# amirkdv/biseqt

Measured on AMD Instinct MI355X. Metric: GCUPS (DP cell updates/s) banded local align, higher is better.
Workload: dtype i16

## Files before the change

biseqt_amd/batch.py:

```python
import ctypes as C

import numpy as np

from . import _pwlib as W
from .sequence import Sequence

RESULT_DTYPE = np.dtype([('score', '<f8'), ('opt_i', '<i4'), ('opt_j', '<i4'),
                         ('origin_idx', '<i4'), ('mutant_idx', '<i4'),
                         ('tx_len', '<i4'), ('status', '<i4')])
assert RESULT_DTYPE.itemsize == 32
SUMMARY_DTYPE = np.dtype([(f, '<i4') for f in ('n_match', 'n_subst', 'n_ins', 'n_del', 'n_gaps', 'first_match', 'last_match',
                                               'head_origin', 'head_mutant', 'tail_origin', 'tail_mutant', 'flags')])
assert SUMMARY_DTYPE.itemsize == 48
CIGAR_EXTENDED, CIGAR_CLASSIC = W.PW_CIGAR_EXTENDED, W.PW_CIGAR_CLASSIC
CIGAR_OPS = 'MIDNSHP=X'
_CIGAR_FORMS = {'extended': CIGAR_EXTENDED, 'classic': CIGAR_CLASSIC}
SITE_DTYPE = np.dtype([('depth', '<u4'), ('call', 'u1'), ('ref', 'u1'), ('flags', '<u2')])
assert SITE_DTYPE.itemsize == 8
POLISH_STATS_DTYPE = np.dtype([(f, '<u4') for f in ('kept', 'substituted', 'deleted', 'inserted')])
assert POLISH_STATS_DTYPE.itemsize == 16
_SIDES = {'origin': W.PW_SIDE_ORIGIN, 'mutant': W.PW_SIDE_MUTANT, 'both': W.PW_SIDE_BOTH}
_CIGAR_LETTERS = ({'M': '=', 'S': 'X', 'I': 'I', 'D': 'D'}, {'M': 'M', 'S': 'M', 'I': 'I', 'D': 'D'})


# ... 604 lines not shown
        if sides not in _SIDES:
            raise ValueError("sides is 'origin', 'mutant' or 'both', not %r" % (sides,))

        def per_pair(a, dtype, what):
            if a is None:
                return None
            a = np.ascontiguousarray(a, dtype).reshape(-1)
            if len(a) != self.n:
                raise ValueError('%s has %d entries for %d pairs' % (what, len(a), self.n))
            return a
        c, mc = per_pair(col0, np.int64, 'col0'), per_pair(mutant_col0, np.int64, 'mutant_col0')
        rv = per_pair(None if reverse is None else np.asarray(reverse) != 0, np.uint8, 'reverse')
        comp = None
        if rv is not None and rv.any():
            if sides == 'origin':
                raise ValueError("reverse applies to the mutant side: sides is 'mutant' or 'both'")
            if complement is None:
                raise ValueError('reversed pairs need a complement table')
            comp = np.ascontiguousarray(complement, np.uint8).reshape(-1)
        if not isinstance(pileup, Pileup) or not pileup.handle:
            raise ValueError('pileup must be an open Pileup')
        if sides == 'origin' and mc is None and rv is None and complement is None and not pileup.ins_slots:
            self._ck(self.lib.pw_batch_pileup_add(self.handle, pileup.handle, None if c is None else c.ctypes.data, int(arena_first), stream),
                     'pw_batch_pileup_add')
            return

        def ptr(a):
            return None if a is None else a.ctypes.data
        self._ck(self.lib.pw_batch_pileup_add_sides(self.handle, pileup.handle, _SIDES[sides], ptr(c), ptr(mc), ptr(rv), ptr(comp),
                                                    0 if comp is None else len(comp), int(arena_first), stream),
                 'pw_batch_pileup_add_sides')

    def scores_plane(self, k):
        X, Y = self.lens[k]
        dmin, dmax, _ = self.band(k)
        nd, pitch = dmax - dmin + 1, min(X, Y) + 1
        out = np.zeros(nd * pitch, np.float64)
        self._ck(self.lib.pw_batch_scores(self.handle, k, out.ctypes.data_as(C.POINTER(C.c_double)), out.size),
                 'pw_batch_scores')
        return out.reshape(nd, pitch)

    def masks(self, k):
        out = np.zeros(max(int(self.lib.pw_batch_pair_cells(self.handle, k)), 1), np.uint8)
        self._ck(self.lib.pw_batch_masks(self.handle, k, out.ctypes.data_as(C.POINTER(C.c_uint8)), out.size),
                 'pw_batch_masks')
        return out

    def results_device(self):
        return DeviceBuffer(self.lib.pw_batch_results_device(self.handle), 32 * self.n, self)

    def transcripts_device(self):
        return DeviceBuffer(self.lib.pw_batch_transcripts_device(self.handle),
                            self.lib.pw_batch_transcripts_bytes(self.handle), self)

    def fill_ms(self):
        return float(self.lib.pw_batch_fill_ms(self.handle))

    def trace_ms(self):
        return float(self.lib.pw_batch_trace_ms(self.handle))


def align_batch(pairs, **kw):
    with BatchAligner(pairs, **kw) as b:
        res = b.run()
        return res, b.transcripts(res)


def summary_dict(rec):
    return {f: int(rec[f]) for f in SUMMARY_DTYPE.names}


def summarize_transcripts(transcripts, device=0):
    if isinstance(transcripts, tuple) and len(transcripts) == 2 and isinstance(transcripts[0], np.ndarray):
        buf = np.ascontiguousarray(transcripts[0], np.uint8)
        off = np.ascontiguousarray(transcripts[1], np.uint64)
        assert off.ndim == 1 and off.size >= 1 and int(off[-1]) <= buf.size
    else:
        raw = [(t or '').encode('ascii') for t in transcripts]
        off = np.zeros(len(raw) + 1, np.uint64)
        if raw:
            off[1:] = np.cumsum([len(r) for r in raw])
        buf = np.frombuffer(b''.join(raw), np.uint8)
    n = off.size - 1
    out = np.zeros(max(n, 1), SUMMARY_DTYPE)
    if W.load().pw_tx_summarize_packed(device, buf.ctypes.data if buf.size else None, off.ctypes.data, n, out.ctypes.data) != 0:
        raise RuntimeError('pw_tx_summarize_packed failed: ' + W.last_error())
    return out[:n]


def _packed_transcripts(transcripts):
    if isinstance(transcripts, tuple) and len(transcripts) == 2 and isinstance(transcripts[0], np.ndarray):
        buf = np.ascontiguousarray(transcripts[0], np.uint8)
        off = np.ascontiguousarray(transcripts[1], np.uint64)
        assert off.ndim == 1 and off.size >= 1 and int(off[-1]) <= buf.size
        return buf, off
    raw = [(t or '').encode('ascii') for t in transcripts]
    off = np.zeros(len(raw) + 1, np.uint64)
    if raw:
        off[1:] = np.cumsum([len(r) for r in raw])
    return np.frombuffer(b''.join(raw), np.uint8), off


def cigars_of_transcripts(transcripts, form='extended', device=0):
    f = _cigar_form(form)
    buf, off = _packed_transcripts(transcripts)
    n = off.size - 1
    lib = W.load()
    roff = np.zeros(n + 1, np.uint64)
    ops = buf.ctypes.data if buf.size else None
    runs = np.zeros(max(int(off[-1]) - int(off[0]), 1), np.uint32)
    if lib.pw_tx_cigar_packed(device, ops, off.ctypes.data, n, f, runs.ctypes.data, runs.size, roff.ctypes.data) != 0:
        raise RuntimeError('pw_tx_cigar_packed failed: ' + W.last_error())
    return runs[:int(roff[-1])].copy(), roff


def cigar_strings(runs, offsets):
    runs, offsets = np.asarray(runs, np.uint32), np.asarray(offsets, np.int64)
    lens, ops = (runs >> 4).tolist(), (runs & 15).tolist()
    return [''.join('%d%s' % (lens[r], CIGAR_OPS[ops[r]]) for r in range(int(offsets[k]), int(offsets[k + 1])))
            for k in range(len(offsets) - 1)]


def cigar_of_transcript(tx, form='extended'):
    letters = _CIGAR_LETTERS[_cigar_form(form)]
    out, cur, n = [], None, 0
    for op in tx or '':
        if op not in letters:
            raise ValueError('transcript op %r is none of M, S, I, D' % (op,))
        if letters[op] == cur:
            n += 1
            continue
        if cur is not None:
            out.append('%d%s' % (n, cur))
        cur, n = letters[op], 1
    if cur is not None:
        out.append('%d%s' % (n, cur))
    return ''.join(out)


def transcript_of_cigar(s):
    import re
    if not re.fullmatch(r'(?:[0-9]+[A-Za-z=])*', s):
        raise ValueError('not a CIGAR string: %r' % (s,))
    back = {'=': 'M', 'X': 'S', 'I': 'I', 'D': 'D'}
    out = []
    for n, op in re.findall(r'([0-9]+)([A-Za-z=])', s):
        if op not in back:
            raise ValueError('CIGAR op %r has no transcript letter (only the extended form =, X, I, D has)' % (op,))
        out.append(back[op] * int(n))
    return ''.join(out)


def plan_only(shapes, alnmode=W.STD_MODE, alntype=W.GLOBAL, alphabet_len=4, subst_scores=None, match_score=1, mismatch_score=0,
              go_score=0, ge_score=0, flags=0, ramp_free=False, stamp_group=False):
    lib = W.load()
    L = alphabet_len
    if subst_scores is None:
        subst_scores = [[match_score if i == j else mismatch_score for i in range(L)] for j in range(L)]
    S = np.ascontiguousarray(np.asarray(subst_scores, dtype=np.float64).reshape(L, L))
    sc = W.pw_scoring(alnmode, alntype, L, S.ctypes.data_as(C.POINTER(C.c_double)), float(go_score), float(ge_score))
    pairs = (W.pw_pair * max(len(shapes), 1))()
    off = 0
    for k, sh in enumerate(shapes):
        X, Y = int(sh[0]), int(sh[1])
        dmin, dmax = (int(sh[2]), int(sh[3])) if len(sh) > 2 else (0, 0)
        oo = off
        off += (X + 15) // 16 * 16 + 16
        mo = off
        off += (Y + 15) // 16 * 16 + 16
        pairs[k] = W.pw_pair(oo, mo, X, Y, dmin, dmax)
    name = C.create_string_buffer(128)
    info = (C.c_int32 * 8)()
    if lib.pw_plan_only(C.byref(sc), len(shapes), pairs, max(off, 16), flags, name, 128, info) != 0:
        raise RuntimeError('pw_plan_only failed: ' + W.last_error())
    out = dict(kernel=name.value.decode(), score_dtype='f64' if info[0] else 'i32', scale_shift=info[1], one_wavefront=info[2],
                workgroup=info[3], tiled=info[4], strips=info[5], packed_rule=info[6], matrix=bool(info[7] & 1))
    if ramp_free:
        out['ramp_free'] = bool(info[7] & 2)
    if stamp_group:
        out['stamp_group'] = 4 if info[7] & 4 else 1
    return out
```

biseqt_amd/csrc/build.py:

```python
import concurrent.futures
import os
import shutil
import subprocess
import sys

HERE = os.path.dirname(os.path.abspath(__file__))
ROOT = os.path.dirname(os.path.dirname(HERE))
OUT_DIR = os.path.join(os.path.dirname(HERE), 'pwlib')
OBJ_DIR = os.path.join(HERE, os.environ.get('PW_OBJ_DIR', '_build'))
SO = os.path.join(OUT_DIR, os.environ.get('PW_SO_NAME', 'pwlib.so'))
HIPCC = os.environ.get('HIPCC', '/opt/rocm/bin/hipcc')
ARCH = 'gfx950'
COMMON = ['--offload-arch=' + ARCH, '-O3', '-std=c++17', '-fPIC', '-ffp-contract=off', '-Wall',
          '-Wno-unused-function'] + os.environ.get('PW_EXTRA_CXXFLAGS', '').split()
BKS = (2, 4, 8, 16, 32)
PACKED_BKS = (4, 8, 12, 16, 20, 24, 28, 32)
PACKED_RULES = (0, 1, 2, 3, 4, 5)
PACKED_MAT_RULES = (0, 1, 2, 3)
FILL16_WAVES = {
    (8, 0, 0): (5, 0), (8, 3, 0): (5, 0),
    (16, 0, 0): (3, 0), (16, 3, 0): (3, 0),
    (8, 0, 1): (3, 0), (8, 3, 1): (3, 0),
}
for _e in filter(None, os.environ.get('PW_FILL16_WAVES_OVERRIDE', '').split(';')):
    _k, _v = _e.split('=')
    FILL16_WAVES[tuple(int(x) for x in _k.split(','))] = tuple(int(x) for x in _v.split(','))
FILL16_UNR = {}
for _e in filter(None, os.environ.get('PW_FILL16_UNR_OVERRIDE', '').split(';')):
    _k, _v = _e.split('=')
    FILL16_UNR[tuple(int(x) for x in _k.split(','))] = int(_v)
TYPES = (('i32', 'int32_t'), ('f64', 'double'))
F64_FLAGS = {'f64': ['-fno-honor-nans'] + os.environ.get('PW_F64_EXTRA_CXXFLAGS', '').split()}
FILL_EXTRA = {('f64', 8): ['-mllvm', '-amdgpu-sched-strategy=max-ilp']}
HASHED_OBJECTS = ('pw_fill16_bk8_r3_mat.o', 'pw_fill16g_bk8_r3_mat.o', 'pw_fill16_bk8_r3.o', 'pw_fill16_bk8_r0.o', 'pw_fill_i32_bk8.o', 'pw_fill_f64_bk8.o', 'pw_strip.o')
HEADERS = ['pw_types.h', 'pw_wave.h', 'pw_strip.h', 'pw_plan.h', 'pw_model.h', 'pw_launch.h', 'pw_device.h', 'pw_hip_host.h']


def _jobs():
    jobs = []
    for tn, t in TYPES:
        for bk in BKS:
            obj = os.path.join(OBJ_DIR, 'pw_fill_%s_bk%d.o' % (tn, bk))
            cmd = [HIPCC] + COMMON + F64_FLAGS.get(tn, []) + FILL_EXTRA.get((tn, bk), []) + ['-DPW_T=' + t, '-DPW_TNAME=' + tn, '-DPW_BK=%d' % bk, '-c',
                                      os.path.join(HERE, 'pw_fill_tu.hip'), '-o', obj]
            jobs.append((obj, cmd, [os.path.join(HERE, 'pw_fill_tu.hip')]))
    for tn, t in TYPES:
        obj = os.path.join(OBJ_DIR, 'pw_fill_mw_%s.o' % tn)
        cmd = [HIPCC] + COMMON + F64_FLAGS.get(tn, []) + ['-DPW_T=' + t, '-DPW_TNAME=' + tn, '-c', os.path.join(HERE, 'pw_fill_mw_tu.hip'), '-o', obj]
        jobs.append((obj, cmd, [os.path.join(HERE, 'pw_fill_mw_tu.hip')]))
    for tn, t in TYPES:
        obj = os.path.join(OBJ_DIR, 'pw_fill_tile_%s.o' % tn)
        cmd = [HIPCC] + COMMON + F64_FLAGS.get(tn, []) + ['-DPW_T=' + t, '-DPW_TNAME=' + tn, '-c', os.path.join(HERE, 'pw_fill_tile_tu.hip'), '-o', obj]
        jobs.append((obj, cmd, [os.path.join(HERE, 'pw_fill_tile_tu.hip')]))
    for bk, rule, mat in [(bk, r, 0) for r in PACKED_RULES for bk in PACKED_BKS] + [(bk, r, 1) for r in PACKED_MAT_RULES for bk in PACKED_BKS]:
        obj = os.path.join(OBJ_DIR, 'pw_fill16_bk%d_r%d%s.o' % (bk, rule, '_mat' if mat else ''))
        occ, occ_seg = FILL16_WAVES.get((bk, rule, mat), (0, 0)) if os.environ.get('PW_FILL16_OCCUPANCY', '1') != '0' else (0, 0)
        cmd = [HIPCC] + COMMON + ['-mllvm', '-amdgpu-sched-strategy=max-ilp', '-DPW_BK=%d' % bk, '-DPW_RULE=%d' % rule, '-DPW_MAT=%d' % mat,
                                  '-DPW_FILL16_WAVES=%d' % occ, '-DPW_FILL16_WAVES_SEG=%d' % occ_seg] + \
              (['-DPW_FILL16_UNR=%d' % FILL16_UNR[(bk, rule, mat)]] if (bk, rule, mat) in FILL16_UNR else []) + ['-c',
               os.path.join(HERE, 'pw_fill16_tu.hip'), '-o', obj]
        jobs.append((obj, cmd, [os.path.join(HERE, 'pw_fill16_tu.hip')]))
    obj = os.path.join(OBJ_DIR, 'pw_fill16g_bk8_r3_mat.o')
    occ, occ_seg = FILL16_WAVES.get((8, 3, 1), (0, 0)) if os.environ.get('PW_FILL16_OCCUPANCY', '1') != '0' else (0, 0)
    jobs.append((obj, [HIPCC] + COMMON + ['-mllvm', '-amdgpu-sched-strategy=max-ilp', '-DPW_FILL16_WAVES=%d' % occ,
                                          '-DPW_FILL16_WAVES_SEG=%d' % occ_seg, '-c', os.path.join(HERE, 'pw_fill16g_tu.hip'), '-o', obj],
                 [os.path.join(HERE, 'pw_fill16g_tu.hip')]))
    obj = os.path.join(OBJ_DIR, 'pw_trace.o')
    jobs.append((obj, [HIPCC] + COMMON + ['-c', os.path.join(HERE, 'pw_trace.hip'), '-o', obj],
                 [os.path.join(HERE, 'pw_trace.hip')]))
    obj = os.path.join(OBJ_DIR, 'pw_txsum.o')
    jobs.append((obj, [HIPCC] + COMMON + ['-c', os.path.join(HERE, 'pw_txsum.hip'), '-o', obj],
                 [os.path.join(HERE, 'pw_txsum.hip'), os.path.join(ROOT, 'include', 'pw_txsum.h'), os.path.join(ROOT, 'include', 'pw_batch.h')]))
    obj = os.path.join(OBJ_DIR, 'pw_cigar.o')
    jobs.append((obj, [HIPCC] + COMMON + ['-c', os.path.join(HERE, 'pw_cigar.hip'), '-o', obj],
                 [os.path.join(HERE, 'pw_cigar.hip'), os.path.join(ROOT, 'include', 'pw_cigar.h'), os.path.join(ROOT, 'include', 'pw_batch.h')]))
    obj = os.path.join(OBJ_DIR, 'pw_pileup.o')
    jobs.append((obj, [HIPCC] + COMMON + ['-c', os.path.join(HERE, 'pw_pileup.hip'), '-o', obj],
                 [os.path.join(HERE, 'pw_pileup.hip'), os.path.join(ROOT, 'include', 'pw_pileup.h'), os.path.join(ROOT, 'include', 'pw_batch.h')]))
    obj = os.path.join(OBJ_DIR, 'pw_polish.o')
    jobs.append((obj, [HIPCC] + COMMON + ['-Wno-unused-parameter', '-c', os.path.join(HERE, 'pw_polish.hip'), '-o', obj],
                 [os.path.join(HERE, 'pw_polish.hip'), os.path.join(ROOT, 'include', 'pw_polish.h'), os.path.join(ROOT, 'include', 'pw_pileup.h'),
                  os.path.join(ROOT, 'include', 'pw_batch.h')]))
    obj = os.path.join(OBJ_DIR, 'pw_graph.o')
    jobs.append((obj, [HIPCC] + COMMON + ['-Wno-unused-parameter', '-c', os.path.join(HERE, 'pw_graph.hip'), '-o', obj],
                 [os.path.join(HERE, 'pw_graph.hip'), os.path.join(HERE, 'pw_graph_launch.h'), os.path.join(ROOT, 'include', 'pw_graph.h'),
                  os.path.join(ROOT, 'include', 'pw_txsum.h'), os.path.join(ROOT, 'include', 'pw_batch.h')]))
    obj = os.path.join(OBJ_DIR, 'pw_consensus.o')
    jobs.append((obj, [HIPCC] + COMMON + ['-Wno-unused-parameter', '-c', os.path.join(HERE, 'pw_consensus.hip'), '-o', obj],
                 [os.path.join(HERE, 'pw_consensus.hip'), os.path.join(HERE, 'pw_consensus_launch.h'), os.path.join(HERE, 'pw_graph_launch.h'),
                  os.path.join(ROOT, 'include', 'pw_consensus.h'), os.path.join(ROOT, 'include', 'pw_graph.h'),
                  os.path.join(ROOT, 'include', 'pw_batch.h')]))
    obj = os.path.join(OBJ_DIR, 'pw_strip.o')
    jobs.append((obj, [HIPCC] + COMMON + os.environ.get('PW_STRIP_CXXFLAGS', '').split() + ['-c', os.path.join(HERE, 'pw_strip.hip'), '-o', obj],
                 [os.path.join(HERE, 'pw_strip.hip')]))
    obj = os.path.join(OBJ_DIR, 'pw_seeds.o')
    jobs.append((obj, [HIPCC] + COMMON + ['-Wno-unused-parameter', '-c', os.path.join(HERE, 'pw_seeds.hip'), '-o', obj],
                 [os.path.join(HERE, 'pw_seeds.hip'), os.path.join(HERE, 'pw_seed_kernels.h'), os.path.join(HERE, 'pw_seed_host.h'), os.path.join(ROOT, 'include', 'pw_seeds.h')]))
    obj = os.path.join(OBJ_DIR, 'pw_mseeds.o')
    jobs.append((obj, [HIPCC] + COMMON + ['-Wno-unused-parameter', '-c', os.path.join(HERE, 'pw_mseeds.hip'), '-o', obj],
                 [os.path.join(HERE, 'pw_mseeds.hip'), os.path.join(HERE, 'pw_seed_kernels.h'), os.path.join(HERE, 'pw_seed_host.h'), os.path.join(ROOT, 'include', 'pw_mseeds.h')]))
    obj = os.path.join(OBJ_DIR, 'pw_qseeds.o')
    jobs.append((obj, [HIPCC] + COMMON + ['-Wno-unused-parameter', '-c', os.path.join(HERE, 'pw_qseeds.hip'), '-o', obj],
                 [os.path.join(HERE, 'pw_qseeds.hip'), os.path.join(HERE, 'pw_seed_kernels.h'), os.path.join(HERE, 'pw_seed_host.h'), os.path.join(HERE, 'pw_complement.h'),
                  os.path.join(ROOT, 'include', 'pw_qseeds.h')]))
    obj = os.path.join(OBJ_DIR, 'pw_overlap.o')
    jobs.append((obj, [HIPCC] + COMMON + ['-Wno-unused-parameter', '-c', os.path.join(HERE, 'pw_overlap.hip'), '-o', obj],
                 [os.path.join(HERE, 'pw_overlap.hip'), os.path.join(HERE, 'pw_complement.h'), os.path.join(HERE, 'pw_kmer_encode.h'), os.path.join(HERE, 'pw_minimizer.h'),
                  os.path.join(ROOT, 'include', 'pw_overlap.h')]))
    obj = os.path.join(OBJ_DIR, 'pw_kmers.o')
    jobs.append((obj, [HIPCC] + COMMON + ['-Wno-unused-parameter', '-c', os.path.join(HERE, 'pw_kmers.hip'), '-o', obj],
                 [os.path.join(HERE, 'pw_kmers.hip'), os.path.join(HERE, 'pw_complement.h'), os.path.join(HERE, 'pw_kmer_encode.h'), os.path.join(HERE, 'pw_minimizer.h'),
                  os.path.join(ROOT, 'include', 'pw_kmers.h'), os.path.join(ROOT, 'include', 'pw_overlap.h')]))
    obj = os.path.join(OBJ_DIR, 'pwlib_api.o')
    jobs.append((obj, [HIPCC] + COMMON + ['-x', 'hip', '-c', os.path.join(HERE, 'pwlib_api.cpp'), '-o', obj],
                 [os.path.join(HERE, 'pwlib_api.cpp'), os.path.join(HERE, 'pw_model.h'), os.path.join(ROOT, 'include', 'pwlib.h'),
                  os.path.join(ROOT, 'include', 'pw_batch.h'), os.path.join(ROOT, 'include', 'pw_txsum.h'),
                  os.path.join(ROOT, 'include', 'pw_cigar.h'), os.path.join(ROOT, 'include', 'pw_pileup.h'),
                  os.path.join(ROOT, 'include', 'pw_polish.h'), os.path.join(ROOT, 'include', 'pw_graph.h'),
                  os.path.join(HERE, 'pw_graph_launch.h'), os.path.join(HERE, 'pw_complement.h'),
                  os.path.join(ROOT, 'include', 'pw_consensus.h'), os.path.join(HERE, 'pw_consensus_launch.h')]))
    return jobs


def _cmd_text(cmd):
    return ' '.join(cmd) + '\n'


def _stale(target, deps, cmd=None):
    if not os.path.exists(target):
        return True
    t = os.path.getmtime(target)
    if any(os.path.getmtime(d) > t for d in deps):
        return True
    if cmd is not None:
        try:
            with open(target + '.cmd') as f:
                return f.read() != _cmd_text(cmd)
        except OSError:
            return True
    return False


def build(force=False, verbose=True):
    os.makedirs(OBJ_DIR, exist_ok=True)
    os.makedirs(OUT_DIR, exist_ok=True)
    hdrs = [os.path.join(HERE, h) for h in HEADERS]
    jobs = _jobs()
    todo = [(o, c) for (o, c, deps) in jobs if force or _stale(o, deps + hdrs, c)]

    def run(job):
        obj, cmd = job
        if os.path.exists(obj + '.cmd'):
            os.remove(obj + '.cmd')
        r = subprocess.run(cmd, stdout=subprocess.PIPE, stderr=subprocess.STDOUT, universal_newlines=True)
        if r.returncode == 0:
            with open(obj + '.cmd', 'w') as f:
                f.write(_cmd_text(cmd))
        return obj, r.returncode, r.stdout

    workers = max(1, min(len(todo), (os.cpu_count() or 4)))
    if todo:
        if verbose:
            print('[build] compiling %d objects for %s with %d workers' % (len(todo), ARCH, workers))
        with concurrent.futures.ThreadPoolExecutor(workers) as ex:
            for obj, rc, out in ex.map(run, todo):
                if rc != 0:
                    raise RuntimeError('hipcc failed for %s:\n%s' % (obj, out))
                if verbose and out.strip():
                    print(out)
    objs = [o for (o, _, _) in jobs]
    strip_obj = os.path.join(OBJ_DIR, 'pw_strip.o')
    if force or any(o == strip_obj for o, _ in todo) or not os.path.exists(SO):
        from . import codeobj
        bad = codeobj.strip_kernel_violations(strip_obj)
        if bad:
            os.remove(strip_obj)
            raise RuntimeError('pw_strip.o breaks the invariants its inline asm relies on:\n  ' + '\n  '.join(bad))
    if force or todo or _stale(SO, objs):
        cmd = [HIPCC, '--offload-arch=' + ARCH, '-shared', '-fPIC'] + objs + ['-o', SO]
        r = subprocess.run(cmd, stdout=subprocess.PIPE, stderr=subprocess.STDOUT, universal_newlines=True)
        if r.returncode != 0:
            raise RuntimeError('link failed:\n' + r.stdout)
        if verbose:
            print('[build] linked', SO)
    shutil.copyfile(os.path.join(ROOT, 'include', 'pwlib.h'), os.path.join(OUT_DIR, 'pwlib.h'))
    hashes = os.path.join(OUT_DIR, 'kernel_hashes.json' if os.path.basename(SO) == 'pwlib.so' else os.path.basename(SO) + '.hashes.json')
    if force or todo or not os.path.exists(hashes):
        from . import codeobj
        import json
        fp = {}
        for obj in HASHED_OBJECTS:
            fp.update(codeobj.kernel_fingerprints(os.path.join(OBJ_DIR, obj)))
        with open(hashes, 'w') as f:
            json.dump(fp, f, indent=1, sort_keys=True)
    return SO


if __name__ == '__main__':
    build(force='--force' in sys.argv)
```

biseqt_amd/csrc/pw_device.h:

```cpp
#ifndef PW_DEVICE_H
#define PW_DEVICE_H

#include <hip/hip_runtime.h>
#include <stdint.h>

#define PW_FN __device__ __forceinline__
#include "pw_wave.h"
#include "pw_launch.h"

namespace pw {

PW_FN uint32_t dev_shl1_in(uint32_t m, bool flag) {
  const uint64_t mask = __builtin_amdgcn_ballot_w64(flag);
  uint32_t r;
  uint64_t cout;
  asm("v_addc_co_u32 %0, %1, %2, %2, %3" : "=v"(r), "=s"(cout) : "v"(m), "s"(mask));
  return r;
}

template <typename T, bool ALWAYS_LDS> PW_FN T dev_tab_read(const T* tab, uint32_t handle, uint32_t off, bool in_lds) {
  typedef __attribute__((address_space(3))) const T lds_T;
  if (ALWAYS_LDS || in_lds) return *(lds_T*)(uintptr_t)(handle + off);
  return *(const T*)((const char*)tab + off);
}
PW_FN uint32_t dev_lds_handle(const void* p) {
  return (uint32_t)(uintptr_t)(__attribute__((address_space(3))) const char*)p;
}

PW_FN uint32_t dev_const_dword(const uint8_t* base, int idx) {
  typedef const __attribute__((address_space(4))) uint32_t c_u32;
  return ((c_u32*)base)[idx];
}

typedef uint64_t FeedDwords __attribute__((aligned(4)));
PW_FN uint64_t dev_const_dword2(const uint8_t* base, uint32_t byte_off) {
  typedef const __attribute__((address_space(4))) uint8_t c_u8;
  typedef const __attribute__((address_space(4))) FeedDwords c_fd;
  return *(c_fd*)((c_u8*)base + byte_off + 4u);
}

struct DevFeed {
  PW_FN static uint64_t const_dword2(const uint8_t* base, uint32_t byte_off) { return dev_const_dword2(base, byte_off); }
};

struct DevP : DevFeed {
  PW_FN static uint32_t const_dword(const uint8_t* base, int idx) { return dev_const_dword(base, idx); }
  template <typename T, bool A> PW_FN static T tab_read(const T* tab, uint32_t h, uint32_t off, bool in_lds) { return dev_tab_read<T, A>(tab, h, off, in_lds); }
  PW_FN static uint32_t shl1_in(uint32_t m, bool flag) { return dev_shl1_in(m, flag); }
  PW_FN static int lane() { return (int)(threadIdx.x & 63u); }
  PW_FN static int32_t shr1(int32_t v, int32_t old) {
    return __builtin_amdgcn_update_dpp(old, v, 0x138 , 0xf, 0xf, false);
  }
  PW_FN static int32_t shl1(int32_t v, int32_t old) {
    return __builtin_amdgcn_update_dpp(old, v, 0x130 , 0xf, 0xf, false);
  }
  PW_FN static int32_t shr1z(int32_t v) { return __builtin_amdgcn_update_dpp(0, v, 0x138 , 0xf, 0xf, true); }
  PW_FN static int32_t shl1z(int32_t v) { return __builtin_amdgcn_update_dpp(0, v, 0x130 , 0xf, 0xf, true); }
  PW_FN static int32_t shfl_xor(int32_t v, int m) { return __shfl_xor(v, m, 64); }
  PW_FN static int32_t uniform(int32_t v) { return __builtin_amdgcn_readfirstlane(v); }
  PW_FN static int nlanes() { return 64; }
  PW_FN static int nwaves() { return 1; }
  PW_FN static int32_t wave_bcast(int32_t v, int) { return v; }
  PW_FN static int lane0() { return 0; }
  PW_FN static bool central() { return true; }
  static constexpr bool kVirtualLanes = false;
  static constexpr bool kBatchedShifts = false;
};

template <int N, int MAXW> PW_FN void wg_shift_right(int32_t* v, const int32_t* old, int phase) {
  __shared__ int32_t edge[2][MAXW][N];
  const int w = (int)(threadIdx.x >> 6), l = (int)(threadIdx.x & 63u);
  int32_t r[N];
#pragma unroll
  for (int i = 0; i < N; i++) r[i] = __builtin_amdgcn_update_dpp(old[i], v[i], 0x138 , 0xf, 0xf, false);
  if (l == 63) {
#pragma unroll
    for (int i = 0; i < N; i++) edge[phase][w][i] = v[i];
  }
  asm volatile("s_waitcnt lgkmcnt(0)\n\ts_barrier" ::: "memory");
  if (l == 0 && w > 0) {
#pragma unroll
    for (int i = 0; i < N; i++) r[i] = edge[phase][w - 1][i];
  }
#pragma unroll
  for (int i = 0; i < N; i++) v[i] = r[i];
}
template <int N, int MAXW> PW_FN void wg_shift_left(int32_t* v, const int32_t* old, int phase) {
  __shared__ int32_t edge[2][MAXW][N];
  const int w = (int)(threadIdx.x >> 6), l = (int)(threadIdx.x & 63u), nw = (int)(blockDim.x >> 6);
  int32_t r[N];
#pragma unroll
  for (int i = 0; i < N; i++) r[i] = __builtin_amdgcn_update_dpp(old[i], v[i], 0x130 , 0xf, 0xf, false);
  if (l == 0) {
#pragma unroll
    for (int i = 0; i < N; i++) edge[phase][w][i] = v[i];
  }
  asm volatile("s_waitcnt lgkmcnt(0)\n\ts_barrier" ::: "memory");
  if (l == 63 && w + 1 < nw) {
#pragma unroll
    for (int i = 0; i < N; i++) r[i] = edge[phase][w + 1][i];
  }
#pragma unroll
  for (int i = 0; i < N; i++) v[i] = r[i];
}

struct DevPM : DevFeed {
  PW_FN static uint32_t const_dword(const uint8_t* base, int idx) { return dev_const_dword(base, idx); }
  template <typename T, bool A> PW_FN static T tab_read(const T* tab, uint32_t h, uint32_t off, bool in_lds) { return dev_tab_read<T, A>(tab, h, off, in_lds); }
  PW_FN static uint32_t shl1_in(uint32_t m, bool flag) { return dev_shl1_in(m, flag); }
  PW_FN static int lane() { return (int)threadIdx.x; }
  PW_FN static int lane0() { return 0; }
  PW_FN static bool central() { return true; }
  static constexpr bool kVirtualLanes = false;
  static constexpr bool kBatchedShifts = true;
  template <int N> PW_FN static void shrv(int32_t* v, const int32_t* old, int phase) { wg_shift_right<N, 16>(v, old, phase); }
  template <int N> PW_FN static void shlv(int32_t* v, const int32_t* old, int phase) { wg_shift_left<N, 16>(v, old, phase); }
  PW_FN static int nlanes() { return (int)blockDim.x; }
  PW_FN static int nwaves() { return (int)(blockDim.x >> 6); }
  PW_FN static int32_t shr1(int32_t v, int32_t old) {
    __shared__ int32_t edge[16];
    const int w = (int)(threadIdx.x >> 6), l = (int)(threadIdx.x & 63u);
    int32_t r = __builtin_amdgcn_update_dpp(old, v, 0x138 , 0xf, 0xf, false);
    if (l == 63) edge[w] = v;
    __syncthreads();
    if (l == 0 && w > 0) r = edge[w - 1];
    __syncthreads();
    return r;
  }
  PW_FN static int32_t shl1(int32_t v, int32_t old) {
    __shared__ int32_t edge[16];
    const int w = (int)(threadIdx.x >> 6), l = (int)(threadIdx.x & 63u);
    int32_t r = __builtin_amdgcn_update_dpp(old, v, 0x130 , 0xf, 0xf, false);
    if (l == 0) edge[w] = v;
    __syncthreads();
    if (l == 63 && w + 1 < (int)(blockDim.x >> 6)) r = edge[w + 1];
    __syncthreads();
    return r;
  }
  PW_FN static int32_t shfl_xor(int32_t v, int m) { return __shfl_xor(v, m, 64); }
  PW_FN static int32_t uniform(int32_t v) { return __builtin_amdgcn_readfirstlane(v); }
  PW_FN static int32_t wave_bcast(int32_t v, int w) {
    __shared__ int32_t slot[16];
    if ((threadIdx.x & 63u) == 0) slot[threadIdx.x >> 6] = v;
    __syncthreads();
    const int32_t r = slot[w];
    __syncthreads();
    return r;
  }
};

constexpr int kMaxLdsL = 32;

#ifndef PW_FILL_ATTR
#define PW_FILL_ATTR
#endif
template <typename T, int BK, bool BANY, bool TRACK, bool GENERIC>
__global__ __launch_bounds__(64) PW_FILL_ATTR void k_fill(const FillParams<T> a) {
  constexpr bool TAB = true;
  __shared__ T sub_lds[TAB ? kMaxLdsL * kMaxLdsL : 1];
  const T* tab = a.subst;
  if (TAB) {
    if (a.L <= kMaxLdsL) {
      for (int i = (int)threadIdx.x; i < a.L * a.L; i += 64) sub_lds[i] = a.subst[i];
      __syncthreads();
      tab = sub_lds;
    }
  }
  const int slot = (int)blockIdx.x;
  const int pair = a.order ? a.order[slot] : slot;
  const PairDesc pd = a.pairs[pair];
  WaveFill<DevP, T, BK, BANY, TRACK, GENERIC> w(a, pd, tab);
  w.tab_handle = dev_lds_handle(sub_lds); w.tab_in_lds = tab == sub_lds;
  w.pair_slot = pair;
  w.run();
}

#ifndef PW_FILL16_WAVES
#define PW_FILL16_WAVES 0
#endif
#ifndef PW_FILL16_WAVES_SEG
#define PW_FILL16_WAVES_SEG 0
#endif
template <int BK, bool SEG, int RULE> struct Fill16Occupancy {
  static constexpr unsigned w = SEG ? PW_FILL16_WAVES_SEG : PW_FILL16_WAVES;
  static constexpr unsigned lo = w ? w : 1, hi = w ? w : 8;
};
template <int BK, bool SEG, int RULE, bool MAT = false>
__global__ __launch_bounds__(64) PW_FILL_ATTR
__attribute__((amdgpu_waves_per_eu(Fill16Occupancy<BK, SEG, RULE>::lo, Fill16Occupancy<BK, SEG, RULE>::hi)))
void k_fill16(const FillParams<int32_t> a) {
  const WaveDesc wd = a.waves[blockIdx.x];
  WaveFill16<DevP, BK, SEG, RULE, MAT> w(a, wd);
  w.run();
}

template <int BK, bool SEG, int RULE, bool MAT = false>
__global__ __launch_bounds__(64) PW_FILL_ATTR
__attribute__((amdgpu_waves_per_eu(Fill16Occupancy<BK, SEG, RULE>::lo, Fill16Occupancy<BK, SEG, RULE>::hi)))
void k_fill16g(const FillParams<int32_t> a) {
  const WaveDesc wd = a.waves[blockIdx.x];
  WaveFill16<DevP, BK, SEG, RULE, MAT, 4> w(a, wd);
  w.run();
}

template <int BK, int RULE, bool MAT = false>
__global__ __launch_bounds__(512) void k_fill16_mw(const FillParams<int32_t> a) {
  const WaveDesc wd = a.waves[blockIdx.x];
  WaveFill16<DevPM, BK, false, RULE, MAT> w(a, wd);
  w.run();
}

constexpr int kTileLanes = PW_TILE_LANES, kTileGhost = PW_TILE_GHOST, kTileCentral = kTileLanes - 2 * kTileGhost;
struct DevPT : DevFeed {
  PW_FN static uint32_t const_dword(const uint8_t* base, int idx) { return dev_const_dword(base, idx); }
  template <typename T, bool A> PW_FN static T tab_read(const T* tab, uint32_t h, uint32_t off, bool in_lds) { return dev_tab_read<T, A>(tab, h, off, in_lds); }
  PW_FN static uint32_t shl1_in(uint32_t m, bool flag) { return dev_shl1_in(m, flag); }
  PW_FN static int tile() {
#ifdef PW_TILE_NO_XCD_REMAP
    return (int)blockIdx.x;
#else
    return (int)(blockIdx.x & 7u) * (int)(gridDim.x >> 3) + (int)(blockIdx.x >> 3);
#endif
  }
  PW_FN static int lane0() { return tile() * kTileCentral - kTileGhost; }
  PW_FN static int lane() { return lane0() + (int)threadIdx.x; }
  PW_FN static int nlanes() { return lane0() + kTileLanes; }
  PW_FN static int nwaves() { return kTileLanes / 64; }
  PW_FN static bool central() { return (int)threadIdx.x >= kTileGhost && (int)threadIdx.x < kTileLanes - kTileGhost; }
  static constexpr bool kVirtualLanes = true;
  static constexpr bool kBatchedShifts = true;
  template <int N> PW_FN static void shrv(int32_t* v, const int32_t* old, int phase) { wg_shift_right<N, kTileLanes / 64>(v, old, phase); }
  template <int N> PW_FN static void shlv(int32_t* v, const int32_t* old, int phase) { wg_shift_left<N, kTileLanes / 64>(v, old, phase); }
  PW_FN static void wg_max4(int (&v)[4]) {
    __shared__ int red[4];
    if (threadIdx.x < 4) red[threadIdx.x] = -0x7fffffff;
    __syncthreads();
#pragma unroll
    for (int i = 0; i < 4; i++) atomicMax(&red[i], v[i]);
    __syncthreads();
#pragma unroll
    for (int i = 0; i < 4; i++) v[i] = red[i];
  }
  PW_FN static int32_t shr1(int32_t v, int32_t old) {
    __shared__ int32_t edge[kTileLanes / 64];
    const int w = (int)(threadIdx.x >> 6), l = (int)(threadIdx.x & 63u);
    int32_t r = __builtin_amdgcn_update_dpp(old, v, 0x138 , 0xf, 0xf, false);
    if (l == 63) edge[w] = v;
    __syncthreads();
    if (l == 0 && w > 0) r = edge[w - 1];
    __syncthreads();
    return r;
  }
  PW_FN static int32_t shl1(int32_t v, int32_t old) {
    __shared__ int32_t edge[kTileLanes / 64];
    const int w = (int)(threadIdx.x >> 6), l = (int)(threadIdx.x & 63u);
    int32_t r = __builtin_amdgcn_update_dpp(old, v, 0x130 , 0xf, 0xf, false);
    if (l == 0) edge[w] = v;
    __syncthreads();
    if (l == 63 && w + 1 < kTileLanes / 64) r = edge[w + 1];
    __syncthreads();
    return r;
  }
  PW_FN static int32_t shfl_xor(int32_t v, int m) { return __shfl_xor(v, m, 64); }
  PW_FN static int32_t uniform(int32_t v) { return __builtin_amdgcn_readfirstlane(v); }
  PW_FN static int32_t wave_bcast(int32_t v, int) { return v; }
};

constexpr int kTileBK = PW_TILE_BK;
static_assert(kTileBK == kTileBKHost && kTileCentral == kTileCentralLanes && kTileBlocks * 16 <= kTileGhost * kTileBK,
              "tile geometry: host and device must agree, and a time block must fit the ghost zone");

template <typename T, bool BANY, bool TRACK, bool GENERIC>
__global__ __launch_bounds__(kTileLanes) void k_fill_tile(const FillParams<T> a, const int pair) {
  constexpr bool TAB = true;
  __shared__ T sub_lds[TAB ? kMaxLdsL * kMaxLdsL : 1];
  const T* tab = a.subst;
  if (TAB) {
    if (a.L <= kMaxLdsL) {
      for (int i = (int)threadIdx.x; i < a.L * a.L; i += (int)blockDim.x) sub_lds[i] = a.subst[i];
      __syncthreads();
      tab = sub_lds;
    }
  }
  const PairDesc pd = a.pairs[pair];
  WaveFill<DevPT, T, kTileBK, BANY, TRACK, GENERIC> w(a, pd, tab);
  w.tab_handle = dev_lds_handle(sub_lds); w.tab_in_lds = tab == sub_lds;
  w.pair_slot = pair;
  w.run_tile();
}

template <typename T>
__global__ __launch_bounds__(256) void k_tile_finish(const FillParams<T> a, const int pair) {
  using Tr = ScoreTraits<T>;
  __shared__ T s_s[256]; __shared__ unsigned long long s_k[256]; __shared__ int s_x[256], s_y[256], s_h[256];
  const PairDesc pd = a.pairs[pair];
  const int X = pd.X, Y = pd.Y, endrule = a.endrule, pitch = a.st_pitch;
  T cs = Tr::neg(); unsigned long long ck = ~0ull; int cx = -1, cy = -1, have = 0;
  for (int dd = (int)threadIdx.x; dd < pd.ndiag; dd += 256) {
    const int d = pd.dmin + dd;
    const bool ends_right = d < X - Y;
    const int lx = ends_right ? d + Y : X, ly = ends_right ? Y : X - d;
    T s; unsigned long long k; int x, y; bool ok = true;
    if (endrule == END_CORNER) { ok = d == X - Y; s = a.st_in[dd]; k = 0; x = X; y = Y; }
    else if (endrule == END_STD_OVERLAP) { s = a.st_in[dd]; x = lx; y = ly; k = ends_right ? (unsigned)lx : (unsigned)(X + ly); }
    else if (endrule == END_BANDED_OVERLAP) { s = a.st_in[dd]; x = lx; y = ly; k = (unsigned)dd; }
    else {
      const int tfirst = (d < 0 ? -d : d) - pd.s0;
      const int aa = ((int)a.st_in[4 * pitch + dd] - tfirst) >> 1;
      s = a.st_in[3 * pitch + dd]; x = aa + (d > 0 ? d : 0); y = aa - (d < 0 ? d : 0);
      if (endrule == END_STD_LOCAL) k = (unsigned long long)(unsigned)x * (unsigned long long)(unsigned)(Y + 1) + (unsigned)y;
      else k = ((unsigned long long)(unsigned)dd << 32) | (unsigned)aa;
    }
    if (ok && (!have || s > cs || (s == cs && k < ck))) { cs = s; ck = k; cx = x; cy = y; have = 1; }
  }
  s_s[threadIdx.x] = cs; s_k[threadIdx.x] = ck; s_x[threadIdx.x] = cx; s_y[threadIdx.x] = cy; s_h[threadIdx.x] = have;
  __syncthreads();
  for (int off = 128; off >= 1; off >>= 1) {
    if ((int)threadIdx.x < off) {
      const int o = (int)threadIdx.x + off;
      if (s_h[o] && (!s_h[threadIdx.x] || s_s[o] > s_s[threadIdx.x] || (s_s[o] == s_s[threadIdx.x] && s_k[o] < s_k[threadIdx.x]))) {
        s_s[threadIdx.x] = s_s[o]; s_k[threadIdx.x] = s_k[o]; s_x[threadIdx.x] = s_x[o]; s_y[threadIdx.x] = s_y[o]; s_h[threadIdx.x] = 1;
      }
    }
    __syncthreads();
  }
  if (threadIdx.x == 0) {
    Result r;
    r.score = (double)s_s[0] * a.score_mul;
    r.opt_i = a.banded ? s_x[0] - s_y[0] - pd.dmin : s_x[0];
    r.opt_j = a.banded ? (s_x[0] < s_y[0] ? s_x[0] : s_y[0]) : s_y[0];
    r.origin_idx = 0; r.mutant_idx = 0; r.tx_len = 0; r.status = 0;
    if (!s_h[0] || (endrule == END_STD_LOCAL && !(s_s[0] > T(0)))) { r.opt_i = -1; r.opt_j = -1; r.score = 0.0; }
    a.results[pair] = r;
  }
}

template <typename T>
hipError_t launch_tile_T(const FillParams<T>& a, int variant, int pair, int ntiles, hipStream_t st) {
  const dim3 grid((unsigned)((ntiles + 7) / 8 * 8)), block(kTileLanes);
  switch (variant) {
    case VAR_FAST_ANY_TRACK: hipLaunchKernelGGL((k_fill_tile<T, true, true, false>), grid, block, 0, st, a, pair); break;
    case VAR_FAST_TRACK: hipLaunchKernelGGL((k_fill_tile<T, false, true, false>), grid, block, 0, st, a, pair); break;
    case VAR_FAST: hipLaunchKernelGGL((k_fill_tile<T, false, false, false>), grid, block, 0, st, a, pair); break;
    case VAR_GENERIC: hipLaunchKernelGGL((k_fill_tile<T, false, true, true>), grid, block, 0, st, a, pair); break;
    default: return hipErrorInvalidValue;
  }
  return hipGetLastError();
}
template <typename T>
hipError_t launch_tile_finish_T(const FillParams<T>& a, int pair, hipStream_t st) {
  hipLaunchKernelGGL((k_tile_finish<T>), dim3(1), dim3(256), 0, st, a, pair);
  return hipGetLastError();
}

// ... 50 lines not shown
```

biseqt_amd/csrc/pw_launch.h:

```cpp
#ifndef PW_LAUNCH_H
#define PW_LAUNCH_H

#include <hip/hip_runtime_api.h>

#include "pw_plan.h"
#include "pw_types.h"

namespace pw {

hipError_t launch_fill(const FillParams<int32_t>& a, int variant, int bk, int nblocks, hipStream_t st);
hipError_t launch_fill(const FillParams<double>& a, int variant, int bk, int nblocks, hipStream_t st);
hipError_t launch_fill16(const FillParams<int32_t>& a, int bk, int seg, int rule, int mat, int nwaves, hipStream_t st);
hipError_t launch_fill16_mw(const FillParams<int32_t>& a, int bk, int rule, int mat, int nw, int npairs, hipStream_t st);
hipError_t launch_fill16g(const FillParams<int32_t>& a, int nwaves, hipStream_t st);
hipError_t launch_fill_mw(const FillParams<int32_t>& a, int variant, int bk, int nw, int nblocks, hipStream_t st);
hipError_t launch_fill_mw(const FillParams<double>& a, int variant, int bk, int nw, int nblocks, hipStream_t st);
hipError_t launch_tile(const FillParams<int32_t>& a, int variant, int pair, int ntiles, hipStream_t st);
hipError_t launch_tile(const FillParams<double>& a, int variant, int pair, int ntiles, hipStream_t st);
hipError_t launch_tile_finish(const FillParams<int32_t>& a, int pair, hipStream_t st);
hipError_t launch_tile_finish(const FillParams<double>& a, int pair, hipStream_t st);
hipError_t launch_trace(const TraceParams& p, hipStream_t st);
hipError_t launch_tx_pack(const PairDesc* pairs, const Result* results, const uint8_t* slots, int n, uint64_t* offsets,
                          uint8_t* packed, hipStream_t st);
hipError_t launch_tx_summary(const PairDesc* pairs, const Result* results, const uint8_t* slots, int n, void* out, hipStream_t st);
hipError_t launch_tx_summary_packed(const uint8_t* ops, const uint64_t* offsets, int n, void* out, hipStream_t st);
hipError_t launch_cigar_count(const PairDesc* pairs, const Result* results, const uint8_t* slots, int n, int form, uint64_t* offsets,
                              hipStream_t st);
hipError_t launch_cigar_write(const PairDesc* pairs, const Result* results, const uint8_t* slots, int n, int form, const uint64_t* offsets,
                              uint32_t* runs, hipStream_t st);
hipError_t launch_cigar_count_packed(const uint8_t* ops, const uint64_t* offsets, int n, int form, uint64_t* run_offsets, hipStream_t st);
hipError_t launch_cigar_write_packed(const uint8_t* ops, const uint64_t* offsets, int n, int form, const uint64_t* run_offsets, uint32_t* runs,
                                     hipStream_t st);
hipError_t launch_pileup_add(const PairDesc* pairs, const Result* results, const uint8_t* slots, const uint8_t* arena, int n,
                             const int64_t* col0, int64_t arena_first, uint32_t* counts, int64_t n_cols, int L, hipStream_t st);
hipError_t launch_pileup_call(const uint32_t* counts, const uint8_t* ref, int64_t n_cols, int L, uint32_t min_depth, void* sites,
                              hipStream_t st);
struct PolishComplement { uint32_t w[8]; };
}
struct DeviceBuffer;
namespace pw {
hipError_t launch_polish_add(const PairDesc* pairs, const Result* results, const uint8_t* slots, const uint8_t* arena, int n, int sides,
                             const int64_t* ocol0, const int64_t* mcol0, const uint8_t* reversed, const PolishComplement& comp,
                             int64_t arena_first, uint32_t* counts, uint32_t* ins, int64_t n_cols, int L, int J, hipStream_t st);
hipError_t launch_polish_letters(uint32_t* counts, const uint8_t* letters, int64_t lo, int64_t hi, int L, uint32_t weight, hipStream_t st);
hipError_t launch_polish_count(const uint32_t* counts, const uint32_t* ins, const uint8_t* letters, const int64_t* roff, const int32_t* rlen,
                               int64_t n, int L, int J, uint32_t min_depth, uint64_t* lens, uint64_t* offsets, void* stats, DeviceBuffer& tmp,
                               hipStream_t st);
hipError_t launch_polish_write(const uint32_t* counts, const uint32_t* ins, const uint8_t* letters, const int64_t* roff, const int32_t* rlen,
                               int64_t n, int L, int J, uint32_t min_depth, const uint64_t* offsets, uint8_t* out, hipStream_t st);
struct StripParams;
struct StripTraceParams;
hipError_t launch_strip_fill(const StripParams& a, bool track, bool byte_rows, const uint32_t* ctl_init, int nworkers, int lds_bytes,
                             hipStream_t st);
hipError_t launch_strip_trace(const StripTraceParams& p, hipStream_t st);
hipError_t launch_xcc_census(uint32_t* d_seen8, hipStream_t st);
hipError_t launch_table_rowmajor(const void* plane, bool f64, int X, int Y, int pitch, double mul, double* out, hipStream_t st);

}
#endif
```

biseqt_amd/csrc/pw_plan.h:

```cpp
#ifndef PW_PLAN_H
#define PW_PLAN_H

#include <math.h>
#include <stdint.h>
#include <stdlib.h>

#include <algorithm>

#include "pw_model.h"
#include "pw_types.h"

namespace pw {

struct Plan {
  int rc;
  int clamped;
  int dmin, dmax;
  int num_rows;
  int64_t cells;
  int ndiag;
  int s0, nblocks, steady_b0, steady_b1;
  int brule, endrule;
};

// ... 18 lines not shown
  if (mode == STD_MODE) {
    *brule = (type == LOCAL || type == END_ANCHORED) ? BRULE_ANY
             : (type == OVERLAP || type == END_ANCHORED_OVERLAP) ? BRULE_EDGE : BRULE_ORIGIN;
    *endrule = (type == GLOBAL || type == END_ANCHORED || type == END_ANCHORED_OVERLAP) ? END_CORNER
               : (type == OVERLAP || type == START_ANCHORED_OVERLAP) ? END_STD_OVERLAP : END_STD_LOCAL;
  } else {
    *brule = type == B_LOCAL ? BRULE_ANY : type == B_OVERLAP ? BRULE_EDGE : BRULE_ORIGIN;
    *endrule = type == B_GLOBAL ? END_CORNER : type == B_OVERLAP ? END_BANDED_OVERLAP : END_BANDED_LOCAL;
  }
}

static inline Plan plan_problem(int mode, int type, int X, int Y, int dmin_in, int dmax_in) {
  Plan p;
  p.rc = 0; p.clamped = 0; p.cells = 0; p.ndiag = 0;
  p.s0 = 0; p.nblocks = 0; p.steady_b0 = 0; p.steady_b1 = 0;
  plan_rules(mode, type, &p.brule, &p.endrule);
  if (mode == STD_MODE) {
    p.dmin = -Y; p.dmax = X; p.num_rows = X + 1;
    p.cells = (int64_t)(X + 1) * (int64_t)(Y + 1);
  } else {
    int dmin = dmin_in, dmax = dmax_in;
    if (dmax > X || dmin < -Y) {
      dmax = dmax > X ? X : dmax;
      dmin = dmin < -Y ? -Y : dmin;
      p.clamped = 1;
    }
    p.dmin = dmin; p.dmax = dmax;
    const int dend = X - Y;
    if (type == B_GLOBAL && (dend > dmax || dend < dmin || (int64_t)dmax * dmin > 0)) { p.rc = -1; return p; }
    p.num_rows = 1 + dmax - dmin;
    if (p.num_rows < 0) { p.rc = -1; return p; }
    if (p.num_rows == 0) { p.ndiag = 0; return p; }
    p.cells = plan_band_cells(X, Y, dmin, dmax);
  }
  p.ndiag = 1 + p.dmax - p.dmin;
  const int amin = p.dmin > 0 ? p.dmin : (p.dmax < 0 ? -p.dmax : 0);
  int s_last = 0, tf_max = 0, tl_min = 0x7fffffff;
  p.s0 = amin - (((amin - p.dmin) % 2 + 2) % 2);
  const int cand[4] = {p.dmin, p.dmax, 0, X - Y};
  for (int k = 0; k < 4; k++) {
    const int d = cand[k];
    if (d < p.dmin || d > p.dmax) continue;
    const int ad = d < 0 ? -d : d;
    const int tl = ad + 2 * (plan_len(X, Y, d) - 1);
    if (tl > s_last) s_last = tl;
    if (ad - p.s0 > tf_max) tf_max = ad - p.s0;
    if (tl - p.s0 < tl_min) tl_min = tl - p.s0;
  }
  const int nsteps = s_last - p.s0 + 1;
  p.nblocks = (nsteps + 15) / 16;
  p.steady_b0 = tf_max / 16 + 1;
  p.steady_b1 = (tl_min + 1) / 16;
  if (p.steady_b1 > p.nblocks) p.steady_b1 = p.nblocks;
  if (p.steady_b1 < p.steady_b0) p.steady_b1 = p.steady_b0;
  return p;
}


enum { VAR_FAST_ANY_TRACK = 0,
       VAR_FAST_TRACK = 1,
       VAR_FAST = 2,
       VAR_GENERIC = 3,
       VAR_FAST16 = 4 };

static const int kSupportedBK[] = {2, 4, 8, 16, 32};
static const int kNumSupportedBK = 5;
static const int kNarrowMwBK[] = {4, 8, 16}, kWideMwBK[] = {8, 16, 32};
static const int kPackedBK[] = {4, 8, 12, 16, 20, 24, 28, 32};
static const int kNumPackedBK = 8;
static const int kMaxWavesPerPair = 8;
#ifndef PW_TILE_LANES
#define PW_TILE_LANES 256
#endif
#ifndef PW_TILE_BK
#define PW_TILE_BK 2
#endif
#ifndef PW_TILE_GHOST
#define PW_TILE_GHOST 64
#endif
#ifndef PW_TILE_BLOCKS
#define PW_TILE_BLOCKS (PW_TILE_GHOST * PW_TILE_BK / 16)
#endif
static const int kTileBKHost = PW_TILE_BK, kTileCentralLanes = PW_TILE_LANES - 2 * PW_TILE_GHOST, kTileBlocks = PW_TILE_BLOCKS;

static inline int narrowest_bk(int ndiag, const int* bk, int n, int waves) {
  for (int i = 0; i < n; i++) if ((int64_t)64 * waves * bk[i] >= ndiag) return bk[i];
  return 0;
}

static inline bool plan_integral(double v) { return v == floor(v) && fabs(v) < 1e9; }

struct ScoreSummary {
  bool finite;
  bool integral;
  bool simple;
  int scale_shift;
  double mt, mm;
  double smin, smax;
  double maxabs;
};

static inline ScoreSummary summarise_scores(int L, const double* subst, double go, double ge, bool allow_dyadic) {
  ScoreSummary s{};
  s.finite = true; s.simple = true;
  s.integral = plan_integral(go) && plan_integral(ge);
  s.maxabs = std::max(fabs(go), std::max(fabs(ge), fabs(go + ge)));
  const double mt0 = subst[0], mm0 = L > 1 ? subst[1] : subst[0];
  for (int i = 0; i < L * L; i++) {
    const double v = subst[i];
    if (!(v == v) || fabs(v) > 1e300) { s.finite = false; return s; }
    s.integral = s.integral && plan_integral(v);
    s.maxabs = std::max(s.maxabs, fabs(v));
    if (v != (i / L == i % L ? mt0 : mm0)) s.simple = false;
  }
  if (!s.integral && allow_dyadic && s.maxabs < 1e6) {
    for (int sh = 1; sh <= 10 && !s.scale_shift; sh++) {
      const double f = (double)(1 << sh);
      bool ok = plan_integral(go * f) && plan_integral(ge * f);
      for (int i = 0; ok && i < L * L; i++) ok = plan_integral(subst[i] * f);
      if (ok) s.scale_shift = sh;
    }
    if (s.scale_shift) { s.integral = true; s.maxabs *= (double)(1 << s.scale_shift); }
  }
  const double f = (double)(1 << s.scale_shift);
  s.mt = mt0 * f; s.mm = mm0 * f;
  s.smin = s.smax = s.mt;
  for (int i = 0; i < L * L; i++) { s.smax = std::max(s.smax, subst[i] * f); s.smin = std::min(s.smin, subst[i] * f); }
  if (s.simple) { s.smax = std::max(s.mt, s.mm); s.smin = std::min(s.mt, s.mm); }
  return s;
}

static inline double floor_gap_step(double go, double ge) { return std::max(0.0, -(ge + std::min(go, 0.0))); }
static inline bool reaches_reference_floor(int brule, bool one_diagonal, double gap_step, double smin, int64_t maxspan) {
  const double h = one_diagonal ? std::max(gap_step, -smin) : gap_step;
  return brule != BRULE_ANY && (double)maxspan * h >= 2147483647.0;
}

struct PlanKnobs {
  bool no_dyadic = false;
  int latency_mode = -1;
  bool no_packed_mat = false;
  bool no_packed_anchored = false;
  bool no_packed_overlap = false;
  bool no_packed_mw = false;
  bool no_strip = false;
  bool no_small_strip = false;
  bool strip_no_byte_rows = false;
  bool no_small_tiled = false;
  bool mw_wide_lanes = false;
  int simple_as_matrix = -1;
  bool no_scaled16 = false;
  bool ramp_blocks = false;
  bool stamp_group1 = false;
  bool packed_bk_forced = false;
  int packed_bk = 0;
  bool packed_bk_seg = false;
};

static inline int packed_rule(int brule, int endrule) {
  const bool local_end = endrule == END_STD_LOCAL || endrule == END_BANDED_LOCAL;
  const bool overlap_end = endrule == END_BANDED_OVERLAP || endrule == END_STD_OVERLAP;
  if (brule == BRULE_ANY) return local_end ? 0 : endrule == END_CORNER ? 4 : -1;
  if (brule == BRULE_ORIGIN) return endrule == END_STD_LOCAL ? 5 : endrule == END_STD_OVERLAP ? 1 : endrule == END_CORNER ? 2 : -1;
  if (brule == BRULE_EDGE) return overlap_end || endrule == END_CORNER ? 1 : -1;
  return -1;
}

static inline bool packed_matrix_bytes_ok(const ScoreSummary& s, int L, bool x4) {
  return L >= 2 && L <= 4 && s.integral && s.smin <= 0 && (x4 ? 4 : 1) * (s.smax - s.smin) <= 127;
}

static inline void packed_matrix_rows(const double* subst, int L, bool x4, uint32_t rows[4], int32_t* bias) {
  const int scale = x4 ? 4 : 1;
  double smin = subst[0];
  for (int i = 0; i < L * L; i++) smin = std::min(smin, subst[i]);
  for (int o = 0; o < 4; o++) {
    uint32_t row = 0;
    for (int m = 0; m < 4; m++)
      if (o < L && m < L) row |= (uint32_t)(scale * (int)(subst[(size_t)o * L + m] - smin)) << (8 * m);
    rows[o] = row;
  }
  *bias = scale * (int)(-smin);
}

struct PackedAdmission {
  int rule = -1;
  bool force_matrix = false;
  bool matrix_ok = false;
  bool x4 = false;
  bool x4_matrix = false;
};

static inline PackedAdmission admit_packed(int rule, const ScoreSummary& s, int L, double go, double ge, int64_t maxmin,
                                           int maxnd, int64_t maxspan, const PlanKnobs& kn) {
  PackedAdmission a;
  const bool bytes = !kn.no_packed_mat && packed_matrix_bytes_ok(s, L, false);
  if (rule < 0 || (!s.simple && (rule > 2 || !bytes))) return a;
  if (s.simple && s.mm > 0) {
    if (rule > 2 || !bytes) return a;
    a.force_matrix = true;
  }
  if (rule >= 4 && kn.no_packed_anchored) return a;
  const double best = (double)maxmin * std::max(0.0, s.smax);
  bool fits;
  if (rule == 0 || rule == 4) fits = best <= 8000;
  else {
    const double lowest = (double)maxmin * std::max(0.0, -s.smin) + fabs(go) + fabs(ge) * (maxnd + 2);
    fits = lowest <= 23000 && !kn.no_packed_overlap;
    fits = fits && best <= (rule == 5 ? 8000 : 30000);
  }
  if (!fits || s.maxabs > 100 || maxspan >= 32000 || go > 0 || ge > 0) return a;
  a.rule = rule;
  a.matrix_ok = s.simple && rule <= 2 && bytes;
  a.x4 = rule == 0 && best <= 2047 && !kn.no_scaled16;
  a.x4_matrix = packed_matrix_bytes_ok(s, L, true);
  return a;
}

static inline bool ramp_free(int rule, bool matrix, double go, double ge, double smin, const PlanKnobs& kn) {
  return (rule == 0 || rule == 3) && matrix && !kn.ramp_blocks && ge < 0 && ge + go < 0 && smin < 0;
}

static inline int stamp_group(int rule, bool matrix, int bk, bool seg, int nw, bool ramp_free_on, const PlanKnobs& kn) {
  return (rule == 3 && matrix && bk == 8 && !seg && nw == 1 && ramp_free_on && !kn.stamp_group1) ? 4 : 1;
}

struct PackedLayout { int bk = 0, nl = 0, seg = 0, nw = 1; };

static inline PackedLayout packed_workgroup_layout(int maxnd) {
  PackedLayout l;
  l.bk = narrowest_bk(maxnd, kPackedBK, kNumPackedBK, kMaxWavesPerPair);
  if (l.bk) { l.nw = (maxnd + 64 * l.bk - 1) / (64 * l.bk); l.nl = 64 * l.nw; }
  return l;
}

static inline PackedLayout packed_lane_layout(int maxnd, int64_t sumnd, int nsolv, bool latency_mode, bool strips_win,
                                              const PlanKnobs& kn, const PlanModel& model) {
  const bool forced = kn.packed_bk_forced;
  const double meannd = (double)sumnd / nsolv;
  double cost1 = 1e300, costp = 1e300; int bk1 = 0, bkp = 0, nlp = 0;
  for (int i = 0; i < kNumPackedBK; i++) {
    const int bk = kPackedBK[i];
    if (forced && kn.packed_bk != bk) continue;
    const int nl = (maxnd + bk - 1) / bk;
    if (nl > 64) continue;
    if (!bk1) {
      bk1 = bk;
      cost1 = model.one_pair_discount * model.seg_slot_cost[i] * last_round_factor((double)nsolv) / (meannd / (64.0 * bk));
    }
    const int ppw = 64 / nl;
    const int64_t nwv = ((int64_t)nsolv + ppw - 1) / ppw;
    const bool enough = forced || nwv >= 1024;
    const double cp = model.seg_slot_cost[i] * last_round_factor((double)nwv) / ((double)ppw * meannd / (64.0 * bk));
    if (ppw >= 2 && enough && cp < costp - 1e-9) { costp = cp; bkp = bk; nlp = nl; }
  }
  const bool want_seg = bkp && (!bk1 || costp < 0.95 * cost1 || (forced && kn.packed_bk_seg));
  const int ppw1 = bk1 ? std::max(1, 64 / ((maxnd + bk1 - 1) / bk1)) : 1;
  PackedLayout l;
  if ((latency_mode || nsolv < 1024 * ppw1) && bk1 && !forced) {
    l.bk = bk1; l.nl = (maxnd + bk1 - 1) / bk1; l.seg = 64 / l.nl >= 2 ? 1 : 0;
  }
  else if (want_seg) { l.bk = bkp; l.nl = nlp; l.seg = 1; }
  else if (bk1) { l.bk = bk1; l.nl = (maxnd + bk1 - 1) / bk1; }
  if (latency_mode && l.bk >= 16 && !l.seg) {
    l = PackedLayout();
    if (!strips_win && !forced && !kn.no_packed_mw) l = packed_workgroup_layout(maxnd);
    if (l.nw <= 1) l = PackedLayout();
  }
  return l;
}

static inline bool packed_matrix_form(const PackedAdmission& adm, const PackedLayout& l, bool simple, const PlanKnobs& kn) {
  const bool measured = !l.seg && l.nw <= 1 && (((l.bk == 8 || l.bk == 16) && adm.rule == 0) || (l.bk == 32 && adm.rule == 2));
  return !simple || adm.force_matrix || (adm.matrix_ok && (kn.simple_as_matrix > 0 || (kn.simple_as_matrix < 0 && measured)));
}

enum { PAIR_WAVES = 0, PAIR_TILED, PAIR_STRIPS };
struct PairLayout { int kind = PAIR_WAVES, bk = 0, nl = 64, nw = 1; };
struct PairRules {
  bool strips;
  bool all_strips;
  bool few_strips;
  bool all_tiled;
  bool few_tiled;
  bool latency_mode, f64, wide_lanes;
  int packed_bk, packed_nl;
};

static inline PairLayout pair_layout(int ndiag, int X, const PairRules& r) {
  PairLayout l;
  if (r.strips && (r.all_strips || ndiag > 2048 * kMaxWavesPerPair || (r.few_strips && X >= 127))) { l.kind = PAIR_STRIPS; return l; }
  if (r.packed_bk) { l.bk = r.packed_bk; l.nl = r.packed_nl; return l; }
  if (r.all_tiled || ndiag > 2048 * kMaxWavesPerPair || (r.few_tiled && ndiag > 1024)) {
    l.kind = PAIR_TILED; l.bk = kTileBKHost; l.nl = (ndiag + l.bk - 1) / l.bk;
    return l;
  }
  l.bk = narrowest_bk(ndiag, kSupportedBK, kNumSupportedBK, 1);
  if (l.bk == 0) {
    if (r.latency_mode || !r.wide_lanes) l.bk = narrowest_bk(ndiag, kWideMwBK, 3, kMaxWavesPerPair);
    if (l.bk == 0) l.bk = 32;
  } else if ((r.latency_mode && l.bk >= 16) || (r.f64 && l.bk >= 32)) {
    if (const int bk = narrowest_bk(ndiag, kNarrowMwBK, 3, kMaxWavesPerPair)) l.bk = bk;
  } else {
    return l;
  }
  l.nw = (ndiag + 64 * l.bk - 1) / (64 * l.bk);
  l.nl = 64 * l.nw;
  return l;
}

}
#endif
```

biseqt_amd/csrc/pw_trace.hip:

```cpp
#include "pw_device.h"

#include <stdlib.h>

namespace pw {

__global__ __launch_bounds__(64) void k_trace(const TraceParams p, const int walkers) {
  __shared__ uint32_t win[64][WIN_WORDS + 1];
  const int pair = (int)blockIdx.x * walkers + (int)threadIdx.x;
  if ((int)threadIdx.x < walkers && pair < p.npairs) trace_walk(p, pair, win[threadIdx.x]);
}

__device__ inline uint32_t bytes_equal(uint32_t w, uint32_t c4) {
  const uint32_t v = w ^ c4;
  const uint32_t t = (v & 0x7f7f7f7fu) + 0x7f7f7f7fu;
  return ~(t | v | 0x7f7f7f7fu);
}
__global__ __launch_bounds__(64) void k_trace_fixup(const TraceParams p) {
  const int pair = (int)blockIdx.x;
  const PairDesc& pd = p.pairs[pair];
  if (!pd.solvable) return;
  const Result r = p.results[pair];
  if (!(r.status & ST_TRACED) || r.tx_len <= 0) return;
  const uint8_t* oseq = p.arena + pd.o_off;
  const uint8_t* mseq = p.arena + pd.m_off;
// ... 18 lines not shown
    }
    const int tail0 = head + 4 * nwords;
    if (tail0 + lane < s0) { nI += tx[tail0 + lane] == 'I'; nD += tx[tail0 + lane] == 'D'; }
#pragma unroll
    for (int off = 32; off >= 1; off >>= 1) { nI += __shfl_xor(nI, off, 64); nD += __shfl_xor(nD, off, 64); }
    x += s0 - nI; y += s0 - nD;
  }
  for (int k0 = s0; k0 < s1; k0 += 64) {
    const int k = k0 + lane;
    const uint8_t ch = k < s1 ? tx[k] : (uint8_t)0;
    const bool isx = ch == 'X';
    const unsigned long long bo = __ballot(isx || ch == 'D'), bm = __ballot(isx || ch == 'I');
    if (isx) {
      const int mx = x + __popcll(bo & below), my = y + __popcll(bm & below);
      tx[k] = (oseq[mx] == mseq[my]) ? 'M' : 'S';
    }
    x += __popcll(bo); y += __popcll(bm);
  }
}

__global__ __launch_bounds__(1024) void k_tx_offsets(const Result* __restrict__ results, int n, unsigned long long* __restrict__ offsets) {
  __shared__ unsigned long long part[1024];
  const int t = (int)threadIdx.x;
  const int per = (n + 1023) / 1024;
  const int k0 = t * per, k1 = k0 + per < n ? k0 + per : n;
  unsigned long long s = 0;
  for (int k = k0; k < k1; k++) { const int len = results[k].tx_len; s += len > 0 ? (unsigned long long)len : 0ull; }
  part[t] = s;
  __syncthreads();
  for (int off = 1; off < 1024; off <<= 1) {
    const unsigned long long v = t >= off ? part[t - off] : 0ull;
    __syncthreads();
    part[t] += v;
    __syncthreads();
  }
  unsigned long long run = t > 0 ? part[t - 1] : 0ull;
  for (int k = k0; k < k1; k++) {
    offsets[k] = run;
    const int len = results[k].tx_len;
    run += len > 0 ? (unsigned long long)len : 0ull;
  }
  if (t == 1023) offsets[n] = part[1023];
}
__global__ __launch_bounds__(64) void k_tx_pack(const PairDesc* __restrict__ pairs, const Result* __restrict__ results,
                                                const uint8_t* __restrict__ slots, const unsigned long long* __restrict__ offsets,
                                                uint8_t* __restrict__ packed) {
  const int pair = (int)blockIdx.x;
  const int len = results[pair].tx_len;
  if (len <= 0) return;
  const PairDesc& pd = pairs[pair];
  const uint8_t* src = slots + pd.tx_off + pd.tx_cap - len;
  uint8_t* dst = packed + offsets[pair];
  const int lane = (int)threadIdx.x;
  const int head = (int)((4u - (uint32_t)((uintptr_t)dst & 3u)) & 3u);
  if (lane < head && lane < len) dst[lane] = src[lane];
  const int nwords = len > head ? (len - head) >> 2 : 0;
  for (int q = lane; q < nwords; q += 64) {
    const uint8_t* sp = src + head + 4 * q;
    PackedU32 v = *(const PackedU32*)sp;
    *(uint32_t*)(dst + head + 4 * q) = v.v;
  }
  const int tail0 = head + 4 * nwords;
  if (tail0 + lane < len) dst[tail0 + lane] = src[tail0 + lane];
}
hipError_t launch_tx_pack(const PairDesc* pairs, const Result* results, const uint8_t* slots, int n, uint64_t* offsets,
                          uint8_t* packed, hipStream_t st) {
  hipLaunchKernelGGL(k_tx_offsets, dim3(1), dim3(1024), 0, st, results, n, (unsigned long long*)offsets);
  hipError_t e = hipGetLastError();
  if (e != hipSuccess || n <= 0) return e;
  hipLaunchKernelGGL(k_tx_pack, dim3((unsigned)n), dim3(64), 0, st, pairs, results, slots, (const unsigned long long*)offsets, packed);
  return hipGetLastError();
}

template <typename T>
__global__ __launch_bounds__(256) void k_table_rowmajor(const T* __restrict__ plane, int X, int Y, int pitch, double mul, double* __restrict__ out) {
  const int64_t c = (int64_t)blockIdx.x * 256 + threadIdx.x;
  if (c >= (int64_t)(X + 1) * (Y + 1)) return;
  const int x = (int)(c / (Y + 1)), y = (int)(c - (int64_t)x * (Y + 1));
  out[c] = (double)plane[(int64_t)(x - y + Y) * pitch + (x < y ? x : y)] * mul;
}
hipError_t launch_table_rowmajor(const void* plane, bool f64, int X, int Y, int pitch, double mul, double* out, hipStream_t st) {
  const int64_t n = (int64_t)(X + 1) * (Y + 1);
  const dim3 grid((unsigned)((n + 255) / 256)), blk(256);
  if (f64) hipLaunchKernelGGL((k_table_rowmajor<double>), grid, blk, 0, st, (const double*)plane, X, Y, pitch, mul, out);
  else hipLaunchKernelGGL((k_table_rowmajor<int32_t>), grid, blk, 0, st, (const int32_t*)plane, X, Y, pitch, mul, out);
  return hipGetLastError();
}

hipError_t launch_trace(const TraceParams& p, hipStream_t st) {
  if (p.npairs <= 0) return hipSuccess;
  static int walkers = 0;
  if (walkers == 0) {
    const char* e = getenv("PWLIB_WALKERS_PER_WAVE");
    walkers = e ? atoi(e) : 64;
    if (walkers < 1 || walkers > 64) walkers = 64;
  }
  hipLaunchKernelGGL(k_trace, dim3((unsigned)((p.npairs + walkers - 1) / walkers)), dim3(64), 0, st, p, walkers);
  hipError_t e = hipGetLastError();
  if (e != hipSuccess) return e;
  hipLaunchKernelGGL(k_trace_fixup, dim3((unsigned)p.npairs, (unsigned)(p.fix_segments > 0 ? p.fix_segments : 1)), dim3(64), 0, st, p);
  return hipGetLastError();
}

#define PW_DECL(TN, T) \
  hipError_t launch_fill_##TN##_bk2(const FillParams<T>&, int, int, hipStream_t);  \
  hipError_t launch_fill_##TN##_bk4(const FillParams<T>&, int, int, hipStream_t);  \
  hipError_t launch_fill_##TN##_bk8(const FillParams<T>&, int, int, hipStream_t);  \
  hipError_t launch_fill_##TN##_bk16(const FillParams<T>&, int, int, hipStream_t); \
  hipError_t launch_fill_##TN##_bk32(const FillParams<T>&, int, int, hipStream_t);
PW_DECL(i32, int32_t)
PW_DECL(f64, double)
#undef PW_DECL
#define PW_BKS(M, R, MT) M(4, R, MT) M(8, R, MT) M(12, R, MT) M(16, R, MT) M(20, R, MT) M(24, R, MT) M(28, R, MT) M(32, R, MT)
#define PW_ALL16(M) PW_BKS(M, 0, 0) PW_BKS(M, 1, 0) PW_BKS(M, 2, 0) PW_BKS(M, 3, 0) PW_BKS(M, 4, 0) PW_BKS(M, 5, 0) \
                    PW_BKS(M, 0, 1) PW_BKS(M, 1, 1) PW_BKS(M, 2, 1) PW_BKS(M, 3, 1)
#define PW_DECL16(BK, R, MT) hipError_t launch_fill16_bk##BK##_r##R##_m##MT(const FillParams<int32_t>&, int, int, hipStream_t); \
  hipError_t launch_fill16mw_bk##BK##_r##R##_m##MT(const FillParams<int32_t>&, int, int, hipStream_t);
PW_ALL16(PW_DECL16)
#undef PW_DECL16

hipError_t launch_tile_i32(const FillParams<int32_t>&, int, int, int, hipStream_t);
hipError_t launch_tile_f64(const FillParams<double>&, int, int, int, hipStream_t);
hipError_t launch_tile_finish_i32(const FillParams<int32_t>&, int, hipStream_t);
hipError_t launch_tile_finish_f64(const FillParams<double>&, int, hipStream_t);
hipError_t launch_tile(const FillParams<int32_t>& a, int variant, int pair, int ntiles, hipStream_t st) { return launch_tile_i32(a, variant, pair, ntiles, st); }
hipError_t launch_tile(const FillParams<double>& a, int variant, int pair, int ntiles, hipStream_t st) { return launch_tile_f64(a, variant, pair, ntiles, st); }
hipError_t launch_tile_finish(const FillParams<int32_t>& a, int pair, hipStream_t st) { return launch_tile_finish_i32(a, pair, st); }
hipError_t launch_tile_finish(const FillParams<double>& a, int pair, hipStream_t st) { return launch_tile_finish_f64(a, pair, st); }

hipError_t launch_fill_mw_i32(const FillParams<int32_t>&, int, int, int, int, hipStream_t);
hipError_t launch_fill_mw_f64(const FillParams<double>&, int, int, int, int, hipStream_t);
hipError_t launch_fill_mw(const FillParams<int32_t>& a, int variant, int bk, int nw, int nblocks, hipStream_t st) {
  return launch_fill_mw_i32(a, variant, bk, nw, nblocks, st);
}
hipError_t launch_fill_mw(const FillParams<double>& a, int variant, int bk, int nw, int nblocks, hipStream_t st) {
  return launch_fill_mw_f64(a, variant, bk, nw, nblocks, st);
}

hipError_t launch_fill16(const FillParams<int32_t>& a, int bk, int seg, int rule, int mat, int nwaves, hipStream_t st) {
#define PW_CASE16(BK, R, MT) case ((BK) * 8 + (R)) * 2 + (MT): return launch_fill16_bk##BK##_r##R##_m##MT(a, seg, nwaves, st);
  switch ((bk * 8 + rule) * 2 + (mat ? 1 : 0)) {
    PW_ALL16(PW_CASE16)
    default: return hipErrorInvalidValue;
  }
#undef PW_CASE16
}

hipError_t launch_fill16g_bk8_r3_m1(const FillParams<int32_t>&, int, hipStream_t);
hipError_t launch_fill16g(const FillParams<int32_t>& a, int nwaves, hipStream_t st) {
  if (!a.ramp_free) return hipErrorInvalidValue;
  return launch_fill16g_bk8_r3_m1(a, nwaves, st);
}

hipError_t launch_fill16_mw(const FillParams<int32_t>& a, int bk, int rule, int mat, int nw, int npairs, hipStream_t st) {
#define PW_CASE16(BK, R, MT) case ((BK) * 8 + (R)) * 2 + (MT): return launch_fill16mw_bk##BK##_r##R##_m##MT(a, nw, npairs, st);
  switch ((bk * 8 + rule) * 2 + (mat ? 1 : 0)) {
    PW_ALL16(PW_CASE16)
    default: return hipErrorInvalidValue;
  }
#undef PW_CASE16
}

hipError_t launch_fill(const FillParams<int32_t>& a, int variant, int bk, int nblocks, hipStream_t st) {
  switch (bk) {
    case 2: return launch_fill_i32_bk2(a, variant, nblocks, st);
    case 4: return launch_fill_i32_bk4(a, variant, nblocks, st);
    case 8: return launch_fill_i32_bk8(a, variant, nblocks, st);
    case 16: return launch_fill_i32_bk16(a, variant, nblocks, st);
    case 32: return launch_fill_i32_bk32(a, variant, nblocks, st);
    default: return hipErrorInvalidValue;
  }
}
hipError_t launch_fill(const FillParams<double>& a, int variant, int bk, int nblocks, hipStream_t st) {
  switch (bk) {
    case 2: return launch_fill_f64_bk2(a, variant, nblocks, st);
    case 4: return launch_fill_f64_bk4(a, variant, nblocks, st);
    case 8: return launch_fill_f64_bk8(a, variant, nblocks, st);
    case 16: return launch_fill_f64_bk16(a, variant, nblocks, st);
    case 32: return launch_fill_f64_bk32(a, variant, nblocks, st);
    default: return hipErrorInvalidValue;
  }
}

}
```

biseqt_amd/csrc/pw_wave.h:

```cpp
#ifndef PW_WAVE_H
#define PW_WAVE_H

#ifndef PW_FN
#error "PW_FN must be defined by the includer"
#endif

#include "pw_types.h"
#if !defined(__HIPCC__)
#include <stdlib.h>
#endif

namespace pw {

template <typename T> struct ScoreTraits;
template <> struct ScoreTraits<int32_t> {
  static constexpr bool is_int = true;
  PW_FN static int32_t neg() { return -(1 << 28); }
  PW_FN static int32_t zero_blk() { return 0; }
  PW_FN static int32_t max2(int32_t a, int32_t b) { return a > b ? a : b; }
  PW_FN static int32_t gap_offer(bool kept, int32_t go, int32_t A) { return kept ? A : A + go; }
};
template <> struct ScoreTraits<double> {
  static constexpr bool is_int = false;
  PW_FN static double neg() { return -1.0e300; }
// ... 448 lines not shown
#pragma unroll
    for (int off = 32; off >= 1; off >>= 1) {
      const T os = xshfl_xor<P>(cs, off);
      const uint64_t ok_ = xshfl_xor<P>(ck, off);
      const int ox = P::shfl_xor(cx, off), oy = P::shfl_xor(cy, off), oh = P::shfl_xor(hv, off);
      const bool take = oh && (!hv || os > cs || (os == cs && ok_ < ck));
      if (take) { cs = os; ck = ok_; cx = ox; cy = oy; hv = 1; }
    }
    if (P::nwaves() > 1) {
      T bs = cs; uint64_t bk_ = ck; int bx = cx, by = cy, bh = 0;
      for (int wv = 0; wv < P::nwaves(); wv++) {
        const T os = xwave_bcast<P>(cs, wv);
        const uint64_t ok_ = xwave_bcast<P>(ck, wv);
        const int ox = P::wave_bcast(cx, wv), oy = P::wave_bcast(cy, wv), oh = P::wave_bcast(hv, wv);
        const bool take = oh && (!bh || os > bs || (os == bs && ok_ < bk_));
        if (take) { bs = os; bk_ = ok_; bx = ox; by = oy; bh = 1; }
      }
      cs = bs; ck = bk_; cx = bx; cy = by; hv = bh;
    }
    if (lane == 0) {
      Result r;
      r.score = (double)cs * a.score_mul;
      r.opt_i = a.banded ? cx - cy - pd.dmin : cx;
      r.opt_j = a.banded ? (cx < cy ? cx : cy) : cy;
      r.origin_idx = 0; r.mutant_idx = 0; r.tx_len = 0; r.status = 0;
      if (!hv || (endrule == END_STD_LOCAL && !(cs > T(0)))) { r.opt_i = -1; r.opt_j = -1; r.score = 0.0; }
      a.results[pair_slot] = r;
    }
  }
  int pair_slot;
};

struct __attribute__((aligned(8))) U4 { uint32_t x, y, z, w; };
struct __attribute__((packed)) PackedU64 { uint64_t v; };
struct __attribute__((packed)) PackedU32 { uint32_t v; };

namespace pk {
#if defined(__HIP_DEVICE_COMPILE__)
typedef short s2_t __attribute__((ext_vector_type(2)));
typedef unsigned short u2_t __attribute__((ext_vector_type(2)));
PW_FN s2_t as_s2(uint32_t v) { return __builtin_bit_cast(s2_t, v); }
PW_FN u2_t as_u2(uint32_t v) { return __builtin_bit_cast(u2_t, v); }
PW_FN uint32_t add(uint32_t a, uint32_t b) { return __builtin_bit_cast(uint32_t, (u2_t)(as_u2(a) + as_u2(b))); }
PW_FN uint32_t sub(uint32_t a, uint32_t b) { return __builtin_bit_cast(uint32_t, (u2_t)(as_u2(a) - as_u2(b))); }
PW_FN uint32_t add32(uint32_t a, uint32_t b) { return a + b; }
PW_FN uint32_t subsat(uint32_t a, uint32_t b) { return __builtin_bit_cast(uint32_t, __builtin_elementwise_sub_sat(as_u2(a), as_u2(b))); }
PW_FN uint32_t max(uint32_t a, uint32_t b) { return __builtin_bit_cast(uint32_t, __builtin_elementwise_max(as_s2(a), as_s2(b))); }
PW_FN uint32_t minu(uint32_t a, uint32_t b) { return __builtin_bit_cast(uint32_t, __builtin_elementwise_min(as_u2(a), as_u2(b))); }
PW_FN uint32_t maxu(uint32_t a, uint32_t b) { return __builtin_bit_cast(uint32_t, __builtin_elementwise_max(as_u2(a), as_u2(b))); }
PW_FN uint32_t shru(uint32_t a, uint32_t sh) { return __builtin_bit_cast(uint32_t, (u2_t)(as_u2(a) >> as_u2(sh))); }
PW_FN uint32_t mad(uint32_t a, uint32_t b, uint32_t c) { return __builtin_bit_cast(uint32_t, (u2_t)(as_u2(a) * as_u2(b) + as_u2(c))); }
PW_FN uint32_t mins(uint32_t a, uint32_t b) { return __builtin_bit_cast(uint32_t, __builtin_elementwise_min(as_s2(a), as_s2(b))); }
PW_FN uint32_t align16(uint32_t hi, uint32_t lo) { return __builtin_amdgcn_alignbit(hi, lo, 16); }
PW_FN uint32_t sign(uint32_t a, uint32_t sh15) { return __builtin_bit_cast(uint32_t, (s2_t)(as_s2(a) >> as_s2(sh15))); }
PW_FN uint32_t opaque(uint32_t v) { asm volatile("" : "+v"(v)); return v; }
PW_FN uint32_t opaque_su(uint32_t v) { asm volatile("" : "+s"(v)); return v; }
PW_FN uint8_t* opaque_s(uint8_t* v) { asm volatile("" : "+s"(v)); return v; }
PW_FN uint32_t copy_su(uint32_t src, uint32_t& pass) {
  uint32_t d;
  asm volatile("s_mov_b32 %0, %2" : "=&s"(d), "+s"(pass) : "s"(src));
  return d;
}
PW_FN void store_global(uint8_t* base, uint32_t off, const U4& v) {
  typedef __attribute__((address_space(1))) uint8_t gbyte_t;
  typedef __attribute__((address_space(1))) U4 gu4_t;
  *(gu4_t*)((gbyte_t*)base + off) = v;
}
PW_FN uint32_t perm(uint32_t a, uint32_t b, uint32_t sel) { return __builtin_amdgcn_perm(a, b, sel); }
#else
PW_FN uint32_t mk(uint32_t lo, uint32_t hi) { return (lo & 0xffffu) | (hi << 16); }
PW_FN int32_t sl(uint32_t v) { return (int16_t)(v & 0xffffu); }
PW_FN int32_t sh(uint32_t v) { return (int16_t)(v >> 16); }
PW_FN uint32_t add(uint32_t a, uint32_t b) { return mk((a & 0xffffu) + (b & 0xffffu), (a >> 16) + (b >> 16)); }
PW_FN uint32_t sub(uint32_t a, uint32_t b) { return mk((a & 0xffffu) - (b & 0xffffu), (a >> 16) - (b >> 16)); }
#if !defined(__HIPCC__)
inline unsigned& add32_breaches() { static unsigned n = 0; return n; }
PW_FN uint32_t add32(uint32_t a, uint32_t b) {
  if ((a & 0xffffu) >= 0xff80u || (a >> 16) >= 0xff80u) add32_breaches()++;
  return a + b;
}
#else
PW_FN uint32_t add32(uint32_t a, uint32_t b) { return a + b; }
#endif
PW_FN uint32_t subsat(uint32_t a, uint32_t b) {
  const uint32_t al = a & 0xffffu, bl = b & 0xffffu, ah = a >> 16, bh = b >> 16;
  return mk(al > bl ? al - bl : 0u, ah > bh ? ah - bh : 0u);
}
PW_FN uint32_t max(uint32_t a, uint32_t b) { return mk((uint32_t)(sl(a) > sl(b) ? sl(a) : sl(b)), (uint32_t)(sh(a) > sh(b) ? sh(a) : sh(b))); }
PW_FN uint32_t minu(uint32_t a, uint32_t b) {
  const uint32_t al = a & 0xffffu, bl = b & 0xffffu, ah = a >> 16, bh = b >> 16;
  return mk(al < bl ? al : bl, ah < bh ? ah : bh);
}
PW_FN uint32_t mad(uint32_t a, uint32_t b, uint32_t c) {
  return mk((uint32_t)(sl(a) * sl(b) + sl(c)), (uint32_t)(sh(a) * sh(b) + sh(c)));
}
PW_FN uint32_t maxu(uint32_t a, uint32_t b) {
  const uint32_t al = a & 0xffffu, bl = b & 0xffffu, ah = a >> 16, bh = b >> 16;
  return mk(al > bl ? al : bl, ah > bh ? ah : bh);
}
PW_FN uint32_t shru(uint32_t a, uint32_t sh) { return mk((a & 0xffffu) >> (sh & 0xfu), (a >> 16) >> ((sh >> 16) & 0xfu)); }
PW_FN uint32_t mins(uint32_t a, uint32_t b) { return mk((uint32_t)(sl(a) < sl(b) ? sl(a) : sl(b)), (uint32_t)(sh(a) < sh(b) ? sh(a) : sh(b))); }
PW_FN uint32_t align16(uint32_t hi, uint32_t lo) { return (lo >> 16) | (hi << 16); }
PW_FN uint32_t sign(uint32_t a, uint32_t) { return mk(sl(a) < 0 ? 0xffffu : 0u, sh(a) < 0 ? 0xffffu : 0u); }
PW_FN uint32_t opaque(uint32_t v) { return v; }
PW_FN uint32_t opaque_su(uint32_t v) { return v; }
PW_FN uint8_t* opaque_s(uint8_t* v) { return v; }
PW_FN uint32_t copy_su(uint32_t src, uint32_t&) { return src; }
PW_FN void store_global(uint8_t* base, uint32_t off, const U4& v) { *(U4*)(base + off) = v; }
PW_FN uint32_t perm(uint32_t a, uint32_t b, uint32_t sel) {
  const uint64_t in = ((uint64_t)a << 32) | b;
  uint32_t r = 0;
  for (int i = 0; i < 4; i++) {
    const uint32_t c = (sel >> (8 * i)) & 0xffu;
    uint32_t v;
    if (c >= 13) v = 0xffu;
    else if (c == 12) v = 0u;
    else if (c >= 8) v = ((in >> (8 * (2 * (c - 8) + 1) + 7)) & 1u) ? 0xffu : 0u;
    else v = (uint32_t)(in >> (8 * c)) & 0xffu;
    r |= v << (8 * i);
  }
  return r;
}
#endif
PW_FN uint32_t both(int32_t v) { return ((uint32_t)v & 0xffffu) | ((uint32_t)v << 16); }
PW_FN uint32_t pack(int32_t lo, int32_t hi) { return ((uint32_t)lo & 0xffffu) | ((uint32_t)hi << 16); }
PW_FN int32_t lo_s(uint32_t v) { return (int32_t)(int16_t)(v & 0xffffu); }
PW_FN int32_t hi_s(uint32_t v) { return (int32_t)(int16_t)(v >> 16); }
}
#if !defined(__HIPCC__)
extern "C" __attribute__((used, visibility("default"))) inline unsigned pw_pk_add32_breaches(int reset) {
  const unsigned n = pk::add32_breaches();
  if (reset) pk::add32_breaches() = 0;
  return n;
}
namespace pk {
inline unsigned* ramp_block_counts() { static unsigned n[4] = {0, 0, 0, 0}; return n; }
inline int& ramp_free_emu() { static int v = -1; return v; }
}
extern "C" __attribute__((used, visibility("default"))) inline void pw_ramp_block_counts(unsigned* out, int reset) {
  for (int i = 0; i < 4; i++) { out[i] = pk::ramp_block_counts()[i]; if (reset) pk::ramp_block_counts()[i] = 0; }
}
extern "C" __attribute__((used, visibility("default"))) inline void pw_emu_ramp_free(int v) { pk::ramp_free_emu() = v; }
namespace pk {
inline int& stamp_group_emu() { static int v = -1; return v; }
inline unsigned& group_stamps() { static unsigned n = 0; return n; }
}
extern "C" __attribute__((used, visibility("default"))) inline void pw_emu_stamp_group(int v) { pk::stamp_group_emu() = v; }
extern "C" __attribute__((used, visibility("default"))) inline unsigned pw_group_stamps(int reset) {
  const unsigned n = pk::group_stamps();
  if (reset) pk::group_stamps() = 0;
  return n;
}
namespace pk {
inline unsigned& feed_breaches() { static unsigned n = 0; return n; }
inline unsigned* feed_path_counts() { static unsigned n[4] = {0, 0, 0, 0}; return n; }
}
extern "C" __attribute__((used, visibility("default"))) inline unsigned pw_feed_breaches(int reset) {
  const unsigned n = pk::feed_breaches();
  if (reset) pk::feed_breaches() = 0;
  return n;
}
extern "C" __attribute__((used, visibility("default"))) inline void pw_feed_path_counts(unsigned* out, int reset) {
  for (int i = 0; i < 4; i++) { out[i] = pk::feed_path_counts()[i]; if (reset) pk::feed_path_counts()[i] = 0; }
}
#endif

template <class P, int BK, bool SEG, int RULE = 0, bool MAT = false, int GRP = 1>
struct WaveFill16 {
  static constexpr bool SC4 = RULE == 3;
  static constexpr int RL = SC4 ? 0 : RULE;
  static constexpr int SCL = SC4 ? 4 : 1;
  static constexpr bool ANYB = RL == 0 || RL == 4;
  static constexpr bool TRK = RL == 0 || RL == 5;
  static constexpr bool CAP = !TRK;
  static_assert(BK % 4 == 0, "packed layout needs an even number of cells per step");
  static constexpr int R = BK / 2;
  static constexpr int RH = R / 2;
#ifdef PW_FILL16_UNR
  static constexpr int UNR = PW_FILL16_UNR;
#else
  static constexpr int UNR = BK <= 8 ? 4 : (BK <= 16 ? 2 : 1);
#endif
  static constexpr int32_t NEG16 = ANYB ? -8192 : -24000;
  static constexpr uint32_t SENT_O = 0xfffeu, SENT_M = 0xffffu;
  static constexpr uint32_t MSEL = 0x0c00u, MOUT = 8u;
  static constexpr bool FIXSEL = MAT && RH == 2;
  PW_FN static uint32_t sel4_fed(int it) { return ((uint32_t)it >> 1) & 1u; }
  PW_FN static bool sel4_lo(int k, int p) { return (((k + 7 - p) >> 1) & 1) != 0; }
  using Base = WaveFill<P, int32_t, BK, true, true, false>;

  const FillParams<int32_t>& a;
  const WaveDesc wd;
  PairDesc pd;
  int li;
  bool valid, segfirst, seglast;
  int pair_slot;
  const uint8_t* oseq;
  const uint8_t* mseq;
  int X, Y, ndiag, owlast, mwlast, xfeed_o, yfeed_m;
  uint32_t fo_lo, fo_hi, fm_lo, fm_hi, fo_n0, fm_n0;
  uint64_t fo_n12, fm_n12;
  uint32_t fo_w, fm_w, fo_lim, fm_lim;

  uint32_t HE[RH], UE[RH], LE[RH], HO[RH], UO[RH], LO[RH];
  uint32_t bestE[RH], bestO[RH], btE[RH], btO[RH];
  uint32_t gebE[RH], gebO[RH];
  uint32_t clE[RH], clO[RH];
  uint32_t tfE[RH], tfO[RH], tlE[RH], tlO[RH];
  uint32_t accE[RH], accO[RH], acc2E[RH], acc2O[RH];
  uint32_t OW[RH], MW[RH];
  uint32_t ROW[MAT ? R : 1];
  uint32_t BIASV, MADJ;
  uint32_t MR0, MR1, MR2, MR3;
  uint32_t ONE, SH15, C2, C4, C16, NDELTA, MATCHV, GOV, GOVI, NEGV, LIMV;
  uint32_t kbE[RH], kbO[RH], C8, SEVEN;
  uint32_t up_prev;
  uint32_t left_next;
  int phase_l, phase_r;
  uint32_t mrow0, mrow_step, mspare, mgroup;
  static constexpr bool SPLIT = ANYB && MAT;
  static constexpr bool KEPT = SC4 && SPLIT;
  static constexpr bool SBASE = !SEG && SPLIT;
  static constexpr bool RAMPF = SPLIT && TRK;
  static constexpr bool GOK = SC4 && SPLIT && TRK && !SEG && BK == 8;
  static_assert(GRP == 1 || (GRP == 4 && GOK), "a stamp group of 4: rule 3, matrix form, one pair per wavefront, 8 per lane");
#if defined(__HIPCC__)
  PW_FN static constexpr bool grp4() { return GRP == 4; }
#else
  bool grp4_rt = false;
  PW_FN bool grp4() const { return grp4_rt; }
#endif
  uint32_t kgE[RH], kgO[RH];
  uint32_t POS[8];
  static constexpr bool FROWS = MAT && !SEG && UNR == 4 && BK <= 8;
  uint32_t frow[FROWS ? 8 : 1];
  bool rf;
  uint32_t flimx, flimy;
  uint32_t mrowb;
  uint8_t* mbase[BK / 4];

  PW_FN WaveFill16(const FillParams<int32_t>& a_, const WaveDesc& wd_) : a(a_), wd(wd_) {}

  template <int EK>
  PW_FN void cellpair(uint32_t& Hs, uint32_t& Us, uint32_t& Ls, uint32_t& bests, uint32_t& bts, uint32_t geb,
                      uint32_t tf, uint32_t tl, uint32_t& acc, uint32_t up, uint32_t left, uint32_t oc,
                      uint32_t mc, uint32_t tv, uint32_t clampL = 0, uint32_t och = 0, bool lo4 = false) {
    constexpr bool EDGE = EK != 0;
    uint32_t hM;
    constexpr bool FLOOR0 = MAT && ANYB && (EK & 1) == 0;
    if (MAT) {
      const uint32_t sub2 = lo4 ? pk::perm(oc, och, mc) : pk::perm(och, oc, mc);
      const uint32_t hb = ANYB ? pk::add32(Hs, sub2) : pk::add(Hs, sub2);
      hM = FLOOR0 ? pk::subsat(hb, BIASV) : pk::sub(hb, BIASV);
    } else {
      const uint32_t ne = pk::minu(oc ^ mc, ONE);
      hM = pk::add(Hs, pk::mad(ne, NDELTA, MATCHV));
    }
    uint32_t Hn = pk::max(pk::max(up, left), hM);
    uint32_t nB;
    if (ANYB) {
      if (EK & 1) Hn = pk::max(Hn, pk::sign(pk::sub(tv, tf), SH15) & NEGV);
      else if (!FLOOR0) Hn = pk::max(Hn, 0u);
      nB = KEPT ? pk::subsat(ONE, Hn) : pk::minu(Hn, ONE);
    } else {
      const uint32_t Bc = EDGE ? pk::mad(pk::minu(tv ^ tf, ONE), NEGV, 0u) : NEGV;
      Hn = pk::max(Hn, Bc);
      nB = pk::minu(Hn ^ Bc, ONE);
    }
    const uint32_t nD = KEPT ? pk::subsat(C2, Hn ^ up) : pk::minu(Hn ^ up, SC4 ? C2 : ONE);
    const uint32_t nI = KEPT ? pk::subsat(C4, Hn ^ left) : pk::minu(Hn ^ left, SC4 ? C4 : ONE);
    const uint32_t hg = pk::add(Hn, geb);
    Us = pk::mad(nD, GOV, hg);
    Ls = pk::mad(nI, GOVI, hg);
    if (!ANYB) Ls = pk::mins(Ls, clampL);
    if (SC4) acc = pk::mad(acc, C16, nB + nD + nI);
    else acc = pk::mad(acc, C16, pk::mad(nI, C4, pk::mad(nD, C2, nB)));
    if (TRK) {
    } else if (EK & 2) {
      const uint32_t e = pk::minu(tv ^ tl, ONE);
      bests = pk::mad(e, pk::sub(bests, Hn), Hn);
    }
    Hs = Hn;
  }

  PW_FN void stamp_best(uint32_t& bts, uint32_t kb, uint32_t kb0, uint32_t blk8) {
    const uint32_t ch = pk::minu((kb ^ kb0) & ~SEVEN, ONE);
    bts = pk::maxu(bts, pk::mad(ch, blk8, kb & SEVEN));
  }
  PW_FN void stamp_group(uint32_t g1) {
#if !defined(__HIPCC__)
    if (P::lane() == 0) pk::group_stamps()++;
#endif
    const uint32_t sv = pk::both((int32_t)(32u * g1));
#pragma unroll
    for (int p = 0; p < RH; p++) {
      const uint32_t chE = pk::minu((kbE[p] ^ kgE[p]) & 0xffe0ffe0u, ONE), chO = pk::minu((kbO[p] ^ kgO[p]) & 0xffe0ffe0u, ONE);
      btE[p] = pk::maxu(btE[p], pk::mad(chE, sv, kbE[p] & 0x001f001fu));
      btO[p] = pk::maxu(btO[p], pk::mad(chO, sv, kbO[p] & 0x001f001fu));
      kgE[p] = kbE[p]; kgO[p] = kbO[p];
    }
  }

  template <int EK>
  PW_FN void track_key(uint32_t& kb, uint32_t H, uint32_t tl, uint32_t tv, int k) {
    const uint32_t hk = (!ANYB || (EK & 1)) ? pk::max(H, 0u) : H;
    uint32_t key = grp4() ? pk::mad(hk, C8, POS[k]) : pk::mad(hk, SC4 ? C2 : C8, pk::both(7 - k));
    if (EK & 2) key &= ~pk::sign(pk::sub(tl, tv), SH15);
    kb = pk::maxu(kb, key);
  }

  template <int EK, int HALF>
  PW_FN void iteration16(int it, int k) {
    constexpr bool EDGE = EK != 0;
    const uint32_t tv0 = pk::both(2 * it), tv1 = pk::both(2 * it + 1);
    {
      uint32_t prev = up_prev;
      if (SEG) prev = segfirst ? NEGV : prev;
      const uint32_t up0 = pk::align16(UO[RH - 1], prev);
#pragma unroll
      for (int p = 0; p < RH; p++)
      {
        cellpair<EK>(HE[p], UE[p], LE[p], bestE[p], btE[p], gebE[p], tfE[p], tlE[p], HALF == 0 ? accE[p] : acc2E[p],
                     p == 0 ? up0 : UO[p == 0 ? 0 : p - 1], LO[p], MAT ? ROW[MAT ? p : 0] : OW[p], MW[p], tv0, clE[p],
                     MAT ? ROW[MAT ? p + RH : 0] : 0u, FIXSEL && sel4_lo(k, p));
        if (TRK) track_key<EK>(kbE[p], HE[p], tlE[p], tv0, k);
      }
    }
    {
      const int oi = xfeed_o + it;
      const uint32_t fb = Base::feed_byte(fo_lo, fo_hi, k);
      uint32_t feed = (!EDGE || (uint32_t)oi < (uint32_t)X) ? fb : SENT_O;
      if (MAT) feed = FROWS ? frow[FROWS ? k : 0] : row_of(fb);
      int32_t mv[2] = {(int32_t)(MAT ? ROW[0] : OW[0]), (int32_t)LE[0]};
      const int32_t mo[2] = {(int32_t)feed, (int32_t)left_next};
      xshlv<P, 2>(mv, mo, phase_l); phase_l ^= 1;
      uint32_t nxt = (uint32_t)mv[0];
      left_next = (uint32_t)mv[1];
      if (SEG) nxt = seglast ? feed : nxt;
      if (MAT) {
#pragma unroll
        for (int i = 0; i + 1 < (MAT ? R : 1); i++) ROW[i] = ROW[i + 1];
        ROW[MAT ? R - 1 : 0] = nxt;
      } else {
        const uint32_t last = pk::align16(nxt, OW[0]);
#pragma unroll
        for (int p = 0; p + 1 < RH; p++) OW[p] = OW[p + 1];
        OW[RH - 1] = last;
      }
    }
    {
      uint32_t nxt = left_next;
      if (SEG) nxt = seglast ? NEGV : nxt;
      const uint32_t leftl = pk::align16(nxt, LE[0]);
#pragma unroll
      for (int p = 0; p < RH; p++)
      {
        cellpair<EK>(HO[p], UO[p], LO[p], bestO[p], btO[p], gebO[p], tfO[p], tlO[p], HALF == 0 ? accO[p] : acc2O[p],
                     UE[p], p == RH - 1 ? leftl : LE[p == RH - 1 ? p : p + 1], MAT ? ROW[MAT ? p : 0] : OW[p], MW[p], tv1, clO[p],
                     MAT ? ROW[MAT ? p + RH : 0] : 0u, FIXSEL && sel4_lo(k, p));
        if (TRK) track_key<EK>(kbO[p], HO[p], tlO[p], tv1, k);
      }
    }
    {
      const int mi = yfeed_m + it;
      const uint32_t fbm = Base::feed_byte(fm_lo, fm_hi, k);
      const uint32_t feed = (MAT ? (MSEL | (fbm + 4u * (FIXSEL ? sel4_fed(k) : 1u)))
                                 : ((!EDGE || (uint32_t)mi < (uint32_t)Y) ? fbm : SENT_M)) << 16;
      int32_t mv[2] = {(int32_t)MW[RH - 1], (int32_t)UO[RH - 1]};
      const int32_t mo[2] = {(int32_t)feed, (int32_t)up_prev};
      xshrv<P, 2>(mv, mo, phase_r); phase_r ^= 1;
      uint32_t prv = (uint32_t)mv[0];
      up_prev = (uint32_t)mv[1];
      if (SEG) prv = segfirst ? feed : prv;
      uint32_t first = pk::align16(MW[RH - 1], prv);
      if (MAT && !FIXSEL) first += MADJ;
#pragma unroll
      for (int p = RH - 1; p > 0; p--) MW[p] = MW[p - 1];
      MW[0] = first;
    }
  }

  template <int EK>
  PW_FN void block16(int b) {
#if !defined(__HIPCC__)
    if (P::lane() == 0) pk::ramp_block_counts()[EK]++;
#endif
#pragma unroll
    for (int p = 0; p < RH; p++) { accE[p] = 0; accO[p] = 0; acc2E[p] = 0; acc2O[p] = 0; }
    uint32_t kb0E[RH], kb0O[RH];
    if (TRK && !grp4()) {
#pragma unroll
      for (int p = 0; p < RH; p++) { kb0E[p] = kbE[p]; kb0O[p] = kbO[p]; }
    }
#pragma clang loop unroll_count(UNR)
    for (int k = 0; k < 4; k++) iteration16<EK, 0>(8 * b + k, k);
#pragma clang loop unroll_count(UNR)
    for (int k = 4; k < 8; k++) iteration16<EK, 1>(8 * b + k, k);
    if (TRK && !grp4()) {
      const uint32_t blk8 = pk::both(8 * b + 8);
#pragma unroll
      for (int p = 0; p < RH; p++) {
        stamp_best(btE[p], kbE[p], kb0E[p], blk8);
        stamp_best(btO[p], kbO[p], kb0O[p], blk8);
      }
    }
    {
      uint32_t mwd[BK];
#pragma unroll
      for (int p = 0; p < RH; p++) {
        const uint32_t inv = KEPT ? 0u : 0x77777777u;
        const uint32_t kE = KEPT ? accE[p] : inv - accE[p], k2E = KEPT ? acc2E[p] : inv - acc2E[p];
        const uint32_t kO = KEPT ? accO[p] : inv - accO[p], k2O = KEPT ? acc2O[p] : inv - acc2O[p];
        mwd[2 * p] = pk::perm(kE, k2E, 0x05040100u);
        mwd[2 * p + R] = pk::perm(kE, k2E, 0x07060302u);
        mwd[2 * p + 1] = pk::perm(kO, k2O, 0x05040100u);
        mwd[2 * p + 1 + R] = pk::perm(kO, k2O, 0x07060302u);
      }
      if (!SBASE) {
        const uint32_t row = b < pd.nblocks ? mrow0 + (uint32_t)b * mrow_step : mspare;
        uint32_t* dst = a.masks + pd.mask_off;
#pragma unroll
        for (int g = 0; g < BK / 4; g++) {
          U4 v; v.x = mwd[4 * g]; v.y = mwd[4 * g + 1]; v.z = mwd[4 * g + 2]; v.w = mwd[4 * g + 3];
          *(U4*)(dst + (row + (uint32_t)g * mgroup)) = v;
        }
      } else {
#pragma unroll
        for (int g = 0; g < BK / 4; g++) {
          U4 v; v.x = mwd[4 * g]; v.y = mwd[4 * g + 1]; v.z = mwd[4 * g + 2]; v.w = mwd[4 * g + 3];
          pk::store_global(mbase[g], mrowb, v);
        }
        mrowb += 4u * mrow_step;
      }
    }
    if (TRK && grp4()) {
#pragma unroll
      for (int k = 0; k < 8; k++) POS[k] -= 0x00080008u;
      if ((b & 3) == 3) {
        stamp_group((uint32_t)(b >> 2) + 1u);
#pragma unroll
        for (int k = 0; k < 8; k++) POS[k] += 0x00200020u;
      }
    }
  }

  PW_FN static uint64_t dwords(uint32_t lo, uint32_t hi) { return ((uint64_t)hi << 32) | lo; }
  PW_FN static void feed_count(int which) {
#if !defined(__HIPCC__)
    if (P::lane() == 0) pk::feed_path_counts()[which]++;
#endif
  }
  PW_FN static uint32_t feed_dword(const uint8_t* base, int idx, int wlast) {
#if !defined(__HIPCC__)
    if (idx < 0 || idx > wlast) { pk::feed_breaches()++; return 0xa5a5a5a5u; }
#endif
    return P::const_dword(base, idx);
  }
  PW_FN static uint64_t feed_dword2(const uint8_t* base, uint32_t byte_off, int wlast) {
#if !defined(__HIPCC__)
    const int idx = (int)(byte_off + 4u) >> 2;
    if ((byte_off & 3u) != 0) pk::feed_breaches()++;
    return dwords(feed_dword(base, idx, wlast), feed_dword(base, idx + 1, wlast));
#else
    return P::const_dword2(base, byte_off);
#endif
  }
  PW_FN void feed_load3(const uint8_t* seq, int wlast, uint32_t fw, uint32_t& n0, uint64_t& n12) {
    const int w = (int)fw >> 2;
    n0 = feed_dword(seq, pw_clampi(w, 0, wlast), wlast);
    n12 = dwords(feed_dword(seq, pw_clampi(w + 1, 0, wlast), wlast), feed_dword(seq, pw_clampi(w + 2, 0, wlast), wlast));
  }
  PW_FN void feed_late(const uint8_t* seq, int wlast, uint32_t fw, uint32_t& n0, uint64_t& n12, int which) {
    const int w = (int)fw >> 2;
    feed_count(2 * which + 1);
    if (w >= wlast || w + 2 <= 0) { n0 = (uint32_t)(n12 >> 32); n12 = dwords(n0, n0); }
    else feed_load3(seq, wlast, fw, n0, n12);
  }
  PW_FN void feed_ahead(const uint8_t* seq, int wlast, uint32_t& fw, uint32_t flim, uint32_t& n0, uint64_t& n12, int which) {
    fw += 8u;
    if (fw < flim) {
      feed_count(2 * which);
      n0 = pk::copy_su((uint32_t)(n12 >> 32), fw);
      n12 = feed_dword2(seq, fw, wlast);
    }
  }
  template <bool FIRST = false>
  PW_FN void feed_issue(int b) {
    if (!SEG) {
      if (FIRST) {
        feed_load3(oseq, owlast, fo_w, fo_n0, fo_n12); feed_load3(mseq, mwlast, fm_w, fm_n0, fm_n12);
      } else {
        feed_ahead(oseq, owlast, fo_w, fo_lim, fo_n0, fo_n12, 0); feed_ahead(mseq, mwlast, fm_w, fm_lim, fm_n0, fm_n12, 1);
      }
      return;
    }
    const uint32_t* o32 = (const uint32_t*)oseq;
    const uint32_t* m32 = (const uint32_t*)mseq;
    const int wo = (xfeed_o + 8 * b) >> 2, wm = (yfeed_m + 8 * b) >> 2;
    fo_n0 = o32[pw_clampi(wo, 0, owlast)]; fo_n12 = dwords(o32[pw_clampi(wo + 1, 0, owlast)], o32[pw_clampi(wo + 2, 0, owlast)]);
    fm_n0 = m32[pw_clampi(wm, 0, mwlast)]; fm_n12 = dwords(m32[pw_clampi(wm + 1, 0, mwlast)], m32[pw_clampi(wm + 2, 0, mwlast)]);
  }
  PW_FN static int clamp08(int v) {
    if (SEG) return pw_clampi(v, 0, 8);
    const int r = (int)pk::opaque_su((uint32_t)(v > 0 ? v : 0));
    return r < 8 ? r : 8;
  }
  PW_FN static uint64_t inside_bytes(int i0, int n) {
    const int lo = clamp08(-i0), hi = clamp08(n - i0);
    const uint64_t below_hi = hi >= 8 ? ~(uint64_t)0 : (((uint64_t)1 << (8 * hi)) - 1);
    const uint64_t below_lo = lo >= 8 ? ~(uint64_t)0 : (((uint64_t)1 << (8 * lo)) - 1);
    return below_hi & ~below_lo;
  }
  template <bool RT = false>
  PW_FN void feed_commit(int b, bool edge) {
    const int ro = (xfeed_o + 8 * b) & 3, rm = (yfeed_m + 8 * b) & 3;
    if (!SEG) {
      const bool late_o = fo_w >= fo_lim, late_m = fm_w >= fm_lim;
      if (late_o | late_m) {
        if (late_o) feed_late(oseq, owlast, fo_w, fo_n0, fo_n12, 0);
        if (late_m) feed_late(mseq, mwlast, fm_w, fm_n0, fm_n12, 1);
      }
    }
    fo_lo = Base::funnel((uint32_t)fo_n12, fo_n0, ro); fo_hi = (uint32_t)(fo_n12 >> (8 * ro));
    fm_lo = Base::funnel((uint32_t)fm_n12, fm_n0, rm); fm_hi = (uint32_t)(fm_n12 >> (8 * rm));
    if (FROWS) {
#pragma unroll
      for (int k = 0; k < 8; k++) frow[k] = row_bits(fo_lo, fo_hi, k);
    }
    if (MAT && edge) {
      const uint64_t io = inside_bytes(xfeed_o + 8 * b, X), im = inside_bytes(yfeed_m + 8 * b, Y);
      const uint64_t m = (((((uint64_t)fm_hi) << 32) | fm_lo) & im) | ((0x0101010101010101ull * MOUT) & ~im);
      fm_lo = (uint32_t)m; fm_hi = (uint32_t)(m >> 32);
      if (FROWS) {
        const uint32_t io_lo = pk::opaque_su((uint32_t)io), io_hi = pk::opaque_su((uint32_t)(io >> 32));
#pragma unroll
        for (int k = 0; k < 8; k++) frow[k] = (((k < 4 ? io_lo : io_hi) >> (8 * (k & 3))) & 1u) ? frow[k] : 0u;
      } else {
        const uint64_t o = ((((uint64_t)fo_hi) << 32) | fo_lo) | ~io;
        fo_lo = (uint32_t)o; fo_hi = (uint32_t)(o >> 32);
      }
      if (!SEG && !RT) { if (!FROWS) fo_hi = pk::opaque_su(fo_hi); fm_hi = pk::opaque_su(fm_hi); }
    }
    if (MAT && !SEG && RT) { if (!FROWS) fo_hi = pk::opaque_su(fo_hi); fm_hi = pk::opaque_su(fm_hi); }
  }

  PW_FN int tfirst_of(int j) const {
    const int dd = li * BK + j, d = pd.dmin + dd;
    if (MAT && ANYB && valid && dd == ndiag) return 0;
    return (valid && dd < ndiag) ? (d < 0 ? -d : d) - pd.s0 : 32767;
  }
  PW_FN int tlast_of(int j) const {
    const int dd = li * BK + j, d = pd.dmin + dd;
    if (!valid || dd >= ndiag) return -1;
    const int len = 1 + (d > 0 ? 0 : d) + (X - d > Y ? Y : X - d);
    return (d < 0 ? -d : d) - pd.s0 + 2 * (len - 1);
  }
  PW_FN int tbegin_of(int j) const {
    const int dd = li * BK + j, d = pd.dmin + dd;
    if (!valid || dd >= ndiag) return 32767;
    if ((RL == 2 || RL == 5 || a.brule == BRULE_ORIGIN) && d != 0) return 32767;
    return (d < 0 ? -d : d) - pd.s0;
  }
  PW_FN uint32_t row_of(uint32_t l) const {
    uint32_t r = l == 3u ? MR3 : 0u;
    r = l == 2u ? MR2 : r;
    r = l == 1u ? MR1 : r;
    return l == 0u ? MR0 : r;
  }
  PW_FN uint32_t row_bits(uint32_t lo, uint32_t hi, int k) const {
    const uint32_t w = k < 4 ? lo : hi;
    const bool b0 = (w & (1u << (8 * (k & 3)))) != 0, b1 = (w & (2u << (8 * (k & 3)))) != 0;
    const uint32_t r01 = b0 ? MR1 : MR0, r23 = b0 ? MR3 : MR2;
    return b1 ? r23 : r01;
  }
  PW_FN uint32_t row_at(int i) const { return (uint32_t)i < (uint32_t)X ? row_of((uint32_t)oseq[i]) : 0u; }
  PW_FN uint32_t msel(int i, uint32_t plus4) const { return MSEL | (((uint32_t)i < (uint32_t)Y ? (uint32_t)mseq[i] : MOUT) + 4u * plus4); }
  PW_FN uint32_t letter_o(int i) const { return (uint32_t)i < (uint32_t)X ? (uint32_t)oseq[i] : SENT_O; }
  PW_FN uint32_t letter_m(int i) const { return (uint32_t)i < (uint32_t)Y ? (uint32_t)mseq[i] : SENT_M; }
  PW_FN int blocked(int j) const { return li * BK + j == ndiag ? NEG16 : 0; }
  PW_FN int start_of(int j) const { return (valid && li * BK + j <= ndiag) ? 0 : NEG16; }
  PW_FN bool ramp_free_on() const {
#if !defined(__HIPCC__)
    if (pk::ramp_free_emu() >= 0) {
      const char* knob = getenv("PWLIB_RAMP_BLOCKS");
      return pk::ramp_free_emu() != 0 && !(knob && atoi(knob) != 0);
    }
#endif
    return a.ramp_free != 0;
  }

  PW_FN void run() {
    const int lane = P::lane();
    const int nl = wd.nl;
    const int seg = lane / nl;
    li = lane - seg * nl;
    valid = seg < wd.count;
    segfirst = li == 0; seglast = li == nl - 1;
    const int slot = wd.first + ((SEG && valid) ? seg : 0);
    pair_slot = a.order ? a.order[slot] : slot;
    if (!SEG) pair_slot = P::uniform(pair_slot);
    pd = a.pairs[pair_slot];
    X = pd.X; Y = pd.Y; ndiag = pd.ndiag;
    oseq = a.arena + pd.o_off; mseq = a.arena + pd.m_off;
    owlast = (X > 0 ? X - 1 : 0) >> 2; mwlast = (Y > 0 ? Y - 1 : 0) >> 2;
    const int e = (pd.s0 + pd.dmin) >> 1;
    const int f = (pd.s0 - pd.dmin) >> 1;
    const int xbase = e + li * R, ybase = f - li * R;
    xfeed_o = e + nl * R - 1;
    yfeed_m = f;
    fo_w = (uint32_t)xfeed_o & ~3u; fm_w = (uint32_t)yfeed_m & ~3u;
    fo_lim = 4u * (uint32_t)(owlast > 1 ? owlast - 1 : 0); fm_lim = 4u * (uint32_t)(mwlast > 1 ? mwlast - 1 : 0);
    rf = RAMPF && (GRP == 4 || ramp_free_on());
#if !defined(__HIPCC__)
    grp4_rt = GRP == 4 || (GOK && rf && P::nwaves() == 1 && pk::stamp_group_emu() == 4);
#endif
    if (grp4()) {
#pragma unroll
      for (int k = 0; k < 8; k++) POS[k] = pk::opaque_su(pk::both(31 - k));
    }
    ONE =pk::opaque(0x00010001u); SH15 = pk::opaque(0x000f000fu);
    C2 = pk::opaque(0x00020002u); C4 = pk::opaque(0x00040004u); C16 = pk::opaque(0x00100010u);
    C8 = pk::opaque(0x00080008u); SEVEN = pk::opaque(0x00070007u);
    NEGV = pk::both(NEG16); LIMV = pk::both(-32767);
    NDELTA = pk::both(SCL * (a.mismatch - a.match)); MATCHV = pk::both(SCL * a.match);
    GOV = pk::both(KEPT ? -2 * a.go : (SC4 ? 2 * a.go : a.go)); GOVI = pk::both(KEPT ? -a.go : a.go);
    BIASV = pk::both(a.mat_bias); MADJ = 0x0003fffcu;
    MR0 = a.mat_rows[0]; MR1 = a.mat_rows[1]; MR2 = a.mat_rows[2]; MR3 = a.mat_rows[3];
    if (MAT) {
#pragma unroll
      for (int i = 0; i < (MAT ? R : 1); i++) ROW[i] = row_at(xbase + i - 1);
    }
#pragma unroll
    for (int p = 0; p < RH; p++) {
      const int e0 = 2 * p, e1 = 2 * p + R, o0 = 2 * p + 1, o1 = 2 * p + 1 + R;
      if (ANYB) {
        const int geo = SCL * a.ge + (KEPT ? SCL * a.go : 0);
        gebE[p] = pk::pack(geo + blocked(e0), geo + blocked(e1));
        gebO[p] = pk::pack(geo + blocked(o0), geo + blocked(o1));
        tfE[p] = pk::pack(tfirst_of(e0), tfirst_of(e1)); tfO[p] = pk::pack(tfirst_of(o0), tfirst_of(o1));
        clE[p] = clO[p] = 0;
      } else {
        gebE[p] = gebO[p] = pk::both(a.ge);
        clE[p] = pk::pack(blocked(e0) ? NEG16 : 32767, blocked(e1) ? NEG16 : 32767);
        clO[p] = pk::pack(blocked(o0) ? NEG16 : 32767, blocked(o1) ? NEG16 : 32767);
        tfE[p] = pk::pack(tbegin_of(e0), tbegin_of(e1)); tfO[p] = pk::pack(tbegin_of(o0), tbegin_of(o1));
      }
      tlE[p] = pk::pack(tlast_of(e0), tlast_of(e1)); tlO[p] = pk::pack(tlast_of(o0), tlast_of(o1));
      HE[p] = UE[p] = LE[p] = HO[p] = UO[p] = LO[p] = NEGV;
      if (RAMPF && rf) {
        HE[p] = pk::pack(start_of(e0), start_of(e1)); HO[p] = pk::pack(start_of(o0), start_of(o1));
      }
      up_prev = left_next = NEGV; phase_l = 0; phase_r = 0;
      bestE[p] = bestO[p] = NEGV;
      kbE[p] = kbO[p] = 0u; btE[p] = btO[p] = 0u; kgE[p] = kgO[p] = 0u;
      OW[p] = pk::pack((int32_t)letter_o(xbase + p - 1), (int32_t)letter_o(xbase + p + RH - 1));
      if (MAT) {
        const int yl = ybase - p - 1, yh = ybase - p - RH - 1;
        MW[p] = pk::pack((int32_t)msel(yl, FIXSEL ? sel4_fed(yl - f) : 0u), (int32_t)msel(yh, FIXSEL ? sel4_fed(yh - f) : 1u));
      }
      else MW[p] = pk::pack((int32_t)letter_m(ybase - p - 1), (int32_t)letter_m(ybase - p - RH - 1));
    }
    const int sb1 = CAP ? wd.steady_b1 - 1 : wd.steady_b1;
    mgroup = 4u * (uint32_t)pd.nl;
    mspare = (uint32_t)mask_word_index(BK, pd.nl, pd.nblocks, 0, 0);
    const bool mrow_ok = valid && li < pd.nl;
    mrow0 = mrow_ok ? (uint32_t)mask_word_index(BK, pd.nl, 0, li, 0) : mspare;
    mrow_step = mrow_ok ? (uint32_t)mask_word_index(BK, pd.nl, 1, 0, 0) : 0u;
    mrowb = 4u * mrow0;
    if (SBASE) {
#pragma unroll
      for (int g = 0; g < BK / 4; g++)
        mbase[g] = pk::opaque_s((uint8_t*)(a.masks + pd.mask_off) + (uint64_t)(4u * (uint32_t)g * mgroup));
    }
    feed_issue<true>(0);
    if constexpr (SPLIT) {
      const int nb = nblocks_run();
      const int b0 = wd.steady_b0 < nb ? (wd.steady_b0 > 0 ? wd.steady_b0 : 0) : nb;
      const int b1 = sb1 < nb ? sb1 : nb;
      const int r0 = (RAMPF && rf) ? 0 : b0, r1 = (RAMPF && rf) ? nb : b1;
      flimx = (uint32_t)(X > 7 ? X - 7 : 0); flimy = (uint32_t)(Y > 7 ? Y - 7 : 0);
      int b = 0;
      if (GRP != 4) {
        if (sb1 > wd.steady_b0) for (; b < r0; b++) blocks_step<1>(b);
        else for (; b < r0; b++) blocks_step<3>(b);
      }
      for (; b < r1; b++) blocks_step<0>(b);
      if (GRP != 4) for (; b < nb; b++) blocks_step<2>(b);
      if (grp4() && (nb & 3) != 0 && nb > 0) stamp_group((uint32_t)(nb >> 2) + 1u);
    } else {
      for (int b = 0, nb = nblocks_run(); b < nb; b++) {
        const bool steady = b >= wd.steady_b0 && b < sb1;
        feed_commit(b, !steady);
        if (b + 1 < nb) feed_issue(b + 1);
        if (steady) block16<0>(b);
        else if (!ANYB) block16<3>(b);
        else if (b >= wd.steady_b0) block16<2>(b);
        else if (sb1 > wd.steady_b0) block16<1>(b);
        else block16<3>(b);
      }
    }
    finish();
  }
  PW_FN int nblocks_run() const { return SBASE ? (wd.nblocks < pd.nblocks ? wd.nblocks : pd.nblocks) : wd.nblocks; }
  template <int EK>
  PW_FN void blocks_step(int b) {
    if constexpr (RAMPF && EK == 0)
      feed_commit<true>(b, rf & (((uint32_t)(xfeed_o + 8 * b) >= flimx) | ((uint32_t)(yfeed_m + 8 * b) >= flimy)));
    else feed_commit(b, EK != 0);
    if (b + 1 < nblocks_run()) feed_issue(b + 1);
    block16<EK>(b);
  }

  PW_FN void finish() {
    const int endrule = a.endrule;
    int32_t cs = -32768; uint64_t ck = ~(uint64_t)0; int cx = -1, cy = -1; bool have = false;
    uint32_t parked[4 * RH];
#pragma unroll
    for (int p = 0; p < RH; p++) {
      parked[4 * p] = TRK ? pk::opaque(kbE[p]) : bestE[p]; parked[4 * p + 1] = TRK ? pk::opaque(btE[p]) : 0u;
      parked[4 * p + 2] = TRK ? pk::opaque(kbO[p]) : bestO[p]; parked[4 * p + 3] = TRK ? pk::opaque(btO[p]) : 0u;
    }
#pragma unroll 1
    for (int q = 0; q < 2 * RH; q++) {
      const int p = q >> 1, odd = q & 1;
      const uint32_t bq = parked[4 * p + 2 * odd], tq = parked[4 * p + 2 * odd + 1];
#pragma unroll 1
      for (int h = 0; h < 2; h++) {
        const int j = 2 * p + odd + h * R;
        const int dd = li * BK + j, d = pd.dmin + dd;
        const int tfirst = (d < 0 ? -d : d) - pd.s0;
        int32_t s; int bt;
        if (TRK) {
          const uint32_t key = h ? (bq >> 16) : (bq & 0xffffu), stamp = h ? (tq >> 16) : (tq & 0xffffu);
          if (!grp4()) {
            s = (int32_t)(key >> 3);
            if (stamp < 8u) bt = ANYB ? (int)((uint32_t)tfirst & 0xffffu) : 0;
            else bt = 16 * ((int)(stamp >> 3) - 1) + 2 * (7 - (int)(stamp & 7u)) + odd;
          } else {
            s = (int32_t)(key >> 5);
            if (stamp < 32u) bt = ANYB ? (int)((uint32_t)tfirst & 0xffffu) : 0;
            else bt = 64 * ((int)(stamp >> 5) - 1) + 2 * (31 - (int)(stamp & 31u)) + odd;
          }
        } else {
          s = (h ? pk::hi_s(bq) : pk::lo_s(bq)) / SCL;
          bt = 0;
        }
        const int aa = (bt - tfirst) >> 1;
        int x = aa + (d > 0 ? d : 0), y = aa - (d < 0 ? d : 0);
        uint64_t k;
        bool ok = true;
        if (CAP) {
          const bool ends_right = d < X - Y;
          x = ends_right ? d + Y : X; y = ends_right ? Y : X - d;
          k = endrule == END_STD_OVERLAP ? (uint64_t)(uint32_t)(x < X ? x : X + y) : (uint64_t)(uint32_t)dd;
          if (RL == 2 || RL == 4 || endrule == END_CORNER) ok = d == X - Y;
        } else if (endrule == END_STD_LOCAL) k = (uint64_t)(uint32_t)x * (uint64_t)(uint32_t)(Y + 1) + (uint64_t)(uint32_t)y;
        else k = ((uint64_t)(uint32_t)dd << 32) | (uint64_t)(uint32_t)aa;
        const bool better = ok && valid && dd < ndiag && (!have || s > cs || (s == cs && k < ck));
        if (better) { cs = s; ck = k; cx = x; cy = y; have = true; }
      }
    }
    const int lane = P::lane();
    const int seg = lane / wd.nl;
    for (int sidx = 0; sidx < wd.count; sidx++) {
      int hv = (have && seg == sidx) ? 1 : 0;
      int32_t rs = cs; uint64_t rk = ck; int rx = cx, ry = cy;
#pragma unroll
      for (int off = 32; off >= 1; off >>= 1) {
        const int32_t os = P::shfl_xor(rs, off);
        const uint64_t ok_ = xshfl_xor<P>(rk, off);
        const int ox = P::shfl_xor(rx, off), oy = P::shfl_xor(ry, off), oh = P::shfl_xor(hv, off);
        const bool take = oh && (!hv || os > rs || (os == rs && ok_ < rk));
        if (take) { rs = os; rk = ok_; rx = ox; ry = oy; hv = 1; }
      }
      if (P::nwaves() > 1) {
        int32_t bs = rs; uint64_t bk_ = rk; int bx = rx, by = ry, bh = 0;
        for (int wv = 0; wv < P::nwaves(); wv++) {
          const int32_t os = P::wave_bcast(rs, wv);
          const uint64_t ok_ = xwave_bcast<P>(rk, wv);
          const int ox = P::wave_bcast(rx, wv), oy = P::wave_bcast(ry, wv), oh = P::wave_bcast(hv, wv);
          const bool take = oh && (!bh || os > bs || (os == bs && ok_ < bk_));
          if (take) { bs = os; bk_ = ok_; bx = ox; by = oy; bh = 1; }
        }
        rs = bs; rk = bk_; rx = bx; ry = by; hv = bh;
      }
      if (seg == sidx && li == 0) {
        Result r;
        r.score = (double)rs * a.score_mul;
        r.opt_i = a.banded ? rx - ry - pd.dmin : rx;
        r.opt_j = a.banded ? (rx < ry ? rx : ry) : ry;
        r.origin_idx = 0; r.mutant_idx = 0; r.tx_len = 0; r.status = 0;
        if (!hv || (endrule == END_STD_LOCAL && !(rs > 0))) { r.opt_i = -1; r.opt_j = -1; r.score = 0.0; }
        a.results[pair_slot] = r;
      }
    }
  }
};

PW_FN int pw_first_op(uint32_t mask) {
  return (mask & 1u) ? 0 : (mask & 2u) ? 1 : (mask & 4u) ? 2 : 3;
}


enum { WIN_B = 4, WIN_WORDS = WIN_B * 2 * 4 };

PW_FN void trace_walk(const TraceParams& p, int pair, uint32_t* win ) {
  const PairDesc pdv = p.pairs[pair];
  if (!pdv.solvable || pdv.layout != 0) return;
  Result r = p.results[pair];
  const int ei = p.ends ? p.ends[2 * pair] : r.opt_i;
  const int ej = p.ends ? p.ends[2 * pair + 1] : r.opt_j;
  if (ei < 0 || ej < 0) { r.tx_len = 0; r.status = 0; p.results[pair] = r; return; }
  const int dmin = pdv.dmin, s0 = pdv.s0, ndiag = pdv.ndiag, bk = pdv.bk, nl = pdv.nl, gosign = p.gosign;
  int x = ei, y = ej;
  if (p.banded) {
    const int d = ei + dmin;
    x = ej + (d > 0 ? d : 0); y = ej - (d > 0 ? 0 : d);
  }
  const uint32_t* __restrict__ plane = p.masks + pdv.mask_off;
  uint8_t* __restrict__ tx = p.transcripts + pdv.tx_off;
  const int lgG = bk < 4 ? 1 : 2;
  const int G = 1 << lgG;
  const int njg = bk >> lgG;
  const int ngroups = (ndiag + G - 1) >> lgG;
  int pos = pdv.tx_cap;
  int nms = 0, bad = 0;
  int prev = 3;
  bool done = false;
  while (!done) {
    const int dd0 = x - y - dmin, t0 = x + y - s0;
    if (x < 0 || y < 0 || x > pdv.X || y > pdv.Y || dd0 < 0 || dd0 >= ndiag) { bad = 1; break; }
    const int cb = t0 >> 4;
    const int ga = dd0 >> lgG;
    int gb = ((dd0 & (G - 1)) >= (G >> 1)) ? ga + 1 : ga - 1;
    gb = gb < 0 ? ga + 1 : (gb >= ngroups ? ga - 1 : gb);
    if (gb < 0) gb = ga;
#pragma unroll
    for (int s2 = 0; s2 < 2; s2++) {
      const int gg = s2 ? gb : ga;
      const int ln = gg / njg, jg = gg - ln * njg;
#pragma unroll
      for (int k = 0; k < WIN_B; k++) {
        const int bb = cb - k > 0 ? cb - k : 0;
        const U4 v = *(const U4*)(plane + ((uint64_t)((uint64_t)bb * njg + jg) * nl + ln) * G);
        uint32_t* wslot = win + (k * 2 + s2) * 4;
        wslot[0] = v.x; wslot[1] = v.y; wslot[2] = v.z; wslot[3] = v.w;
      }
    }
    while (true) {
      const int dd = x - y - dmin, t = x + y - s0;
      if (x < 0 || y < 0 || x > pdv.X || y > pdv.Y || dd < 0 || dd >= ndiag) { bad = 1; done = true; break; }
      const int gg = dd >> lgG, b = t >> 4, kb = cb - b;
      if ((gg != ga && gg != gb) || kb < 0 || kb >= WIN_B) break;
      const uint32_t w = win[(kb * 2 + (gg == ga ? 0 : 1)) * 4 + (dd & (G - 1))];
      const uint32_t pm = (w >> (4 * (7 - ((t & 15) >> 1)))) & 15u;
      int op;
      if (prev == 3 || gosign == 0) op = pw_first_op(pm);
      else if (gosign < 0) op = (pm & (1u << prev)) ? prev : pw_first_op(pm);
      else { const uint32_t others = pm & ~(1u << prev); op = others ? pw_first_op(others) : prev; }
      if (op == 0 || pos <= 0) { done = true; break; }
      tx[--pos] = op == 3 ? 'X' : (op == 1 ? 'D' : 'I');
      nms += (op == 3);
      x -= (op != 2); y -= (op != 1);
      prev = op;
      if (op == 3) {
        const int n = ((t & 15) >> 1) - 1;
        if (n >= 0 && pos >= 16) {
          const uint64_t v = (uint64_t)((w & 0x77777777u) >> (4 * (7 - n))) | ((uint64_t)1 << (4 * (n + 1)));
          int k = (int)(__builtin_ctzll(v) >> 2);
          const int lim = x < y ? x : y;
          k = k < lim ? k : lim;
          if (k > 0) {
            PackedU64 xs; xs.v = 0x5858585858585858ull;
            *(PackedU64*)(tx + pos - 8) = xs;
            pos -= k; nms += k; x -= k; y -= k;
          }
        }
      }
    }
  }
  r.origin_idx = x; r.mutant_idx = y;
  r.tx_len = pdv.tx_cap - pos;
  r.status = ST_TRACED | (r.tx_len == 0 ? ST_EMPTY : 0) | ((x + y + nms <= 0) ? ST_PANICK : 0) | (bad ? ST_BADPATH : 0);
  p.results[pair] = r;
}

PW_FN void trace_fixup_serial(const TraceParams& p, int pair) {
  const PairDesc& pd = p.pairs[pair];
  if (!pd.solvable) return;
  const Result r = p.results[pair];
  if (!(r.status & ST_TRACED) || r.tx_len <= 0) return;
  const uint8_t* oseq = p.arena + pd.o_off;
  const uint8_t* mseq = p.arena + pd.m_off;
  uint8_t* tx = p.transcripts + pd.tx_off + pd.tx_cap - r.tx_len;
  int x = r.origin_idx, y = r.mutant_idx;
  for (int k = 0; k < r.tx_len; k++) {
    const uint8_t ch = tx[k];
    if (ch == 'X') { tx[k] = (oseq[x] == mseq[y]) ? 'M' : 'S'; x++; y++; }
    else if (ch == 'D') x++;
    else y++;
  }
}

}
#endif
```

biseqt_amd/csrc/pwlib_api.cpp:

```cpp
#include <hip/hip_runtime.h>
#include <math.h>
#include <cmath>
#include <stdint.h>
#include <stdio.h>
#include <stdlib.h>
#include <string.h>

#include <algorithm>
#include <string>
#include <chrono>
#include <memory>
#include <mutex>
#include <thread>
#include <vector>
#include <unordered_set>

#include "../../include/pw_batch.h"
#include "../../include/pw_txsum.h"
#include "../../include/pw_cigar.h"
#include "../../include/pw_pileup.h"
#include "../../include/pw_polish.h"
#include "../../include/pw_graph.h"
#include "../../include/pw_consensus.h"
#include "pw_launch.h"
// ... 20 lines not shown
struct PoolEntry { void* p; size_t bytes; int device; };
std::mutex g_pool_mutex;
std::vector<PoolEntry> g_pool;
constexpr int kMaxDevices = 64;
size_t g_pool_held[kMaxDevices] = {0};
size_t g_pool_cap[kMaxDevices] = {0};

size_t pool_cap(int device) {
  if (device < 0 || device >= kMaxDevices) return 0;
  if (g_pool_cap[device] == 0) {
    const char* v = getenv("PWLIB_POOL_GB");
    size_t cap;
    if (v && *v) cap = (size_t)atoi(v) << 30;
    else {
      size_t fr = 0, tot = 0;
      cap = (hipMemGetInfo(&fr, &tot) == hipSuccess) ? tot / 4 : ((size_t)16 << 30);
    }
    g_pool_cap[device] = cap + 1;
  }
  return g_pool_cap[device] - 1;
}
size_t pool_room_now(int device, size_t held) {
  static const bool fixed = [] { const char* v = getenv("PWLIB_POOL_GB"); return v && *v; }();
  const size_t cap = pool_cap(device);
  if (fixed) return cap;
  size_t fr = 0, tot = 0;
  if (hipMemGetInfo(&fr, &tot) != hipSuccess) return cap;
  return std::min(cap, (fr + held) / 2);
}

void* pool_take(int device, size_t bytes, size_t* got) {
  std::lock_guard<std::mutex> lk(g_pool_mutex);
  int best = -1;
  for (int i = 0; i < (int)g_pool.size(); i++)
    if (g_pool[i].device == device && g_pool[i].bytes >= bytes && g_pool[i].bytes <= bytes + bytes / 4 + (1u << 20) &&
        (best < 0 || g_pool[i].bytes < g_pool[best].bytes)) best = i;
  if (best < 0) return nullptr;
  void* p = g_pool[best].p; *got = g_pool[best].bytes;
  if (device >= 0 && device < kMaxDevices) g_pool_held[device] -= g_pool[best].bytes;
  g_pool.erase(g_pool.begin() + best);
  return p;
}
void pool_give(int device, void* p, size_t bytes) {
  if (!p) return;
  if (device >= 0 && device < kMaxDevices && bytes >= (1u << 20)) {
    size_t held_now;
    { std::lock_guard<std::mutex> lk(g_pool_mutex); held_now = g_pool_held[device]; }
    const size_t cap = pool_room_now(device, held_now);
    std::lock_guard<std::mutex> lk(g_pool_mutex);
    if (g_pool_held[device] + bytes <= cap && g_pool.size() < 64) {
      g_pool.push_back(PoolEntry{p, bytes, device});
      g_pool_held[device] += bytes;
      return;
    }
  }
  (void)hipFree(p);
}
void pool_drop(int device ) {
  std::vector<PoolEntry> drop;
  {
    std::lock_guard<std::mutex> lk(g_pool_mutex);
    std::vector<PoolEntry> keep;
    for (auto& e : g_pool) (device < 0 || e.device == device ? drop : keep).push_back(e);
    g_pool.swap(keep);
    for (int d = 0; d < kMaxDevices; d++) if (device < 0 || d == device) g_pool_held[d] = 0;
  }
  int cur = 0;
  (void)hipGetDevice(&cur);
  for (auto& d : drop) { (void)hipSetDevice(d.device); (void)hipFree(d.p); }
  (void)hipSetDevice(cur);
}
hipError_t pool_alloc(int device, void** p, size_t bytes, size_t* got) {
  if (bytes >= (1u << 20)) {
    int lg = 0; while ((bytes >> (lg + 1)) != 0) lg++;
    const size_t step = (size_t)1 << (lg - 3);
    bytes = (bytes + step - 1) / step * step;
  }
  *p = pool_take(device, bytes, got);
  if (*p) return hipSuccess;
  *got = bytes;
  hipError_t e = hipMalloc(p, bytes);
  if (e != hipSuccess) {
    (void)hipGetLastError();
    pool_drop(device);
    e = hipMalloc(p, bytes);
  }
  return e;
}

template <typename T>
struct PoolBuffer {
  int device = -1;
  T* p = nullptr;
  size_t bytes = 0;
  PoolBuffer() = default;
  PoolBuffer(PoolBuffer&& o) noexcept : device(o.device), p(std::exchange(o.p, nullptr)), bytes(std::exchange(o.bytes, 0)) {}
  PoolBuffer& operator=(PoolBuffer&& o) noexcept { std::swap(device, o.device); std::swap(p, o.p); std::swap(bytes, o.bytes); return *this; }
  ~PoolBuffer() { pool_give(device, p, bytes); }
  hipError_t alloc(int dev, size_t want) {
    pool_give(device, std::exchange(p, nullptr), bytes);
    device = dev;
    void* q = nullptr;
    const hipError_t e = pool_alloc(dev, &q, want, &bytes);
    if (e == hipSuccess) p = (T*)q;
    return e;
  }
};

thread_local std::string g_err;

int fail(const std::string& msg) { g_err = msg; return -1; }

#define HIP_TRY(expr) PW_HIP_CHECK(fail, expr)

struct BkClass {
  int bk = 0;
  int nw = 1;
  std::vector<int32_t> order;
  DeviceArray<int32_t> d_order;
};

}

struct pw_batch {
  int device = 0;
  int32_t n = 0;
  uint32_t flags = 0;
  int mode = 0, type = 0, L = 0;
  double go = 0, ge = 0;
  std::vector<double> subst;
  bool simple = false, use_f64 = false;
  double plan_ms = 0;
  pw::PlanKnobs knobs;
  int scale_shift = 0;
  double score_mul = 1.0;
  int variant = 0, brule = 0, endrule = 0, gosign = 0;
  std::vector<pw_pair> pairs;
  std::vector<pw::Plan> plans;
  std::vector<pw::PairDesc> descs;
  std::vector<BkClass> classes;
  std::vector<pw::WaveDesc> waves;
  std::vector<int32_t> strips;
  std::vector<uint32_t> strip_ctl_init;
  PoolBuffer<uint64_t> d_fifo; size_t fifo_bytes = 0;
  DeviceArray<pw::StripBest> d_sbest;
  DeviceArray<uint32_t> d_ctl;
  std::vector<int32_t> tiled;
  DeviceBuffer d_state[2];
  int32_t st_pitch = 0;
  int packed_seg = 0, packed_rule = 0, packed_nw = 1;
  int packed_mat = 0;
  int ramp_free = 0;
  int stamp_group = 1;
  DeviceArray<pw::WaveDesc> d_waves;
  int64_t cells = 0, alg_bytes = 0;
  bool on_device = false;
  PoolBuffer<uint8_t> arena; uint64_t arena_bytes = 0;
  uint8_t* d_arena = nullptr;
  bool arena_shared = false;
  PoolBuffer<pw::PairDesc> d_pairs;
  PoolBuffer<uint32_t> d_masks; uint64_t mask_words = 0;
  DeviceBuffer d_hdump; uint64_t h_elems = 0;
  PoolBuffer<pw::Result> d_results;
  PoolBuffer<uint8_t> d_tx; uint64_t tx_bytes = 0;
  DeviceBuffer d_subst;
  DeviceArray<int32_t> d_ends;
  PoolBuffer<uint8_t> d_txpacked;
  DeviceArray<uint64_t> d_txoffsets;
  PoolBuffer<pw_tx_summary> d_summaries;
  uint64_t trace_seq = 0, summary_seq = 0;
  DeviceArray<uint64_t> d_cigoffsets;
  PoolBuffer<uint32_t> d_cigruns;
  uint64_t cigar_room = 0, cigar_total = 0, cigar_seq = 0;
  int cigar_form = -1;
  hipStream_t cigar_stream = nullptr;
  DeviceArray<int64_t> d_col0;
  std::vector<int64_t> h_col0;
  DeviceArray<int64_t> d_sides_col0;
  DeviceArray<uint8_t> d_reversed;
  std::vector<int64_t> h_sides_col0;
  std::vector<uint8_t> h_reversed;
  DeviceEvent ev_fill0, ev_fill1, ev_tr0, ev_tr1;
  bool fill_timed = false, trace_timed = false;
  std::vector<double> subst_in; double go_in = 0, ge_in = 0;
  std::vector<std::pair<int32_t, std::unique_ptr<pw_batch>>> repaired;
  std::vector<std::pair<hipStream_t, DeviceEvent>> done_events;
  bool traced = false, traced_from = false;
  std::vector<int32_t> last_ends;
  ~pw_batch();
};

pw_batch::~pw_batch() {
  repaired.clear();
  if (!on_device) return;
  (void)hipSetDevice(device);
  for (auto& se : done_events) (void)hipEventSynchronize(se.second.e);
}

namespace {

pw::PlanKnobs plan_knobs() {
  auto on = [](const char* name) { return env_int(name, 0) != 0; };
  pw::PlanKnobs k;
  k.no_dyadic = on("PWLIB_NO_DYADIC");
  k.latency_mode = env_int("PWLIB_LATENCY_MODE", -1);
  k.no_packed_mat = on("PWLIB_NO_PACKED_MAT");
  k.no_packed_anchored = on("PWLIB_NO_PACKED_ANCHORED");
  k.no_packed_overlap = on("PWLIB_NO_PACKED_OVERLAP");
  k.no_packed_mw = on("PWLIB_NO_PACKED_MW");
  k.no_strip = on("PWLIB_NO_STRIP");
  k.no_small_strip = on("PWLIB_NO_SMALL_STRIP");
  k.strip_no_byte_rows = on("PWLIB_STRIP_NO_BYTE_ROWS");
  k.no_small_tiled = on("PWLIB_NO_SMALL_TILED");
  k.mw_wide_lanes = on("PWLIB_MW_WIDE_LANES");
  k.simple_as_matrix = env_int("PWLIB_SIMPLE_AS_MATRIX", -1);
  k.no_scaled16 = on("PWLIB_NO_SCALED16");
  k.ramp_blocks = on("PWLIB_RAMP_BLOCKS");
  k.stamp_group1 = env_int("PWLIB_STAMP_GROUP", 0) == 1;
  const char* bk = getenv("PWLIB_PACKED_BK");
  if (bk && *bk) { k.packed_bk_forced = true; k.packed_bk = atoi(bk); k.packed_bk_seg = strchr(bk, 's') != nullptr; }
  return k;
}

int batch_inputs(pw_batch* b, bool plan_only, const pw_scoring* sc, int32_t n_pairs, const pw_pair* pairs, uint64_t arena_bytes,
                 uint32_t flags) {
  if (!sc || n_pairs < 0 || (n_pairs > 0 && !pairs) || (plan_only && !sc->subst))
    return fail(plan_only ? "pw_plan_only: bad arguments" : "pw_batch_create: bad arguments");
  if (sc->mode != pw::STD_MODE && sc->mode != pw::BANDED_MODE) return fail("unknown alignment mode");
  if (sc->type < 0 || sc->type > (sc->mode == pw::STD_MODE ? 6 : 2)) return fail("unknown alignment type");
  if (sc->alphabet_len < 1 || sc->alphabet_len > 256 || !sc->subst) return fail("alphabet_len must be 1..256 with a score matrix");
  b->n = n_pairs; b->flags = flags;
  b->mode = sc->mode; b->type = sc->type; b->L = sc->alphabet_len; b->go = sc->go; b->ge = sc->ge;
  b->subst.assign(sc->subst, sc->subst + (size_t)b->L * b->L);
  b->subst_in = b->subst; b->go_in = b->go; b->ge_in = b->ge;
  b->pairs.assign(pairs, pairs + n_pairs);
  b->arena_bytes = arena_bytes;
  return 0;
}

void plan_waves(pw_batch* b, const pw::PackedLayout& p16) {
  const int ppw = p16.seg ? 64 / p16.nl : 1;
  BkClass& c = b->classes[0];
  for (size_t i = 0; i < c.order.size(); i += ppw) {
    pw::WaveDesc wd;
    memset(&wd, 0, sizeof wd);
    wd.first = (int32_t)i; wd.count = (int32_t)std::min<size_t>(ppw, c.order.size() - i);
    wd.nl = (p16.seg || p16.nw > 1) ? p16.nl : 64;
    wd.nblocks = 0; wd.steady_b0 = 0; wd.steady_b1 = 0x7fffffff;
    for (int q = 0; q < wd.count; q++) {
      const pw::PairDesc& d = b->descs[c.order[i + q]];
      wd.nblocks = std::max(wd.nblocks, d.nblocks);
      wd.steady_b0 = std::max(wd.steady_b0, d.steady_b0);
      wd.steady_b1 = std::min(wd.steady_b1, d.steady_b1);
    }
    if (wd.steady_b1 < wd.steady_b0) wd.steady_b1 = wd.steady_b0;
    b->waves.push_back(wd);
  }
}

int batch_plan(pw_batch* b) {
  const double t_build0 = std::chrono::duration<double, std::milli>(std::chrono::steady_clock::now().time_since_epoch()).count();
  const int L = b->L;
  const pw::PlanKnobs& kn = b->knobs = plan_knobs();
  const pw::ScoreSummary sc = pw::summarise_scores(L, b->subst.data(), b->go, b->ge, !(b->flags & PW_FLAG_FORCE_F64) && !kn.no_dyadic);
  if (!sc.finite) return fail("substitution scores must be finite");
  b->simple = sc.simple;
  if (sc.scale_shift) {
    const double f = (double)(1 << sc.scale_shift);
    for (auto& v : b->subst) v *= f;
    b->go *= f; b->ge *= f;
    b->scale_shift = sc.scale_shift; b->score_mul = 1.0 / f;
  }
  pw::plan_rules(b->mode, b->type, &b->brule, &b->endrule);
  b->gosign = b->go < 0 ? -1 : (b->go > 0 ? 1 : 0);
  int64_t maxspan = 0, maxmin = 0; int maxnd = 0; int64_t sumnd = 0; int nsolv = 0;
  const pw::PlanModel& model = pw::kPlanModel;
  pw::BatchEstimates est;
  int min_x = 0x7fffffff;
  b->plans.resize(b->n); b->descs.resize(b->n);
  uint64_t mask_words = 0, h_elems = 0, tx_bytes = 0;
  for (int32_t k = 0; k < b->n; k++) {
    const pw_pair& p = b->pairs[k];
    if (p.origin_len < 0 || p.mutant_len < 0) return fail("negative sequence length");
    if (p.origin_off + (uint64_t)p.origin_len > b->arena_bytes || p.mutant_off + (uint64_t)p.mutant_len > b->arena_bytes)
      return fail("pair frame outside the arena");
    if ((int64_t)p.origin_len + p.mutant_len > (1 << 30)) return fail("sequences too long");
    if ((p.origin_off & 3) || (p.mutant_off & 3)) return fail("frames must start on a 4-byte boundary of the arena");
    pw::Plan pl = pw::plan_problem(b->mode, b->type, p.origin_len, p.mutant_len, p.dmin, p.dmax);
    b->plans[k] = pl;
    pw::PairDesc d;
    memset(&d, 0, sizeof d);
    d.o_off = p.origin_off; d.m_off = p.mutant_off;
    d.X = p.origin_len; d.Y = p.mutant_len;
    d.solvable = (pl.rc == 0 && pl.ndiag > 0) ? 1 : 0;
    d.tx_off = tx_bytes;
    d.tx_cap = p.origin_len + p.mutant_len + 1;
    tx_bytes += ((uint64_t)d.tx_cap + 15) / 16 * 16;
    if (d.solvable) {
      d.dmin = pl.dmin; d.ndiag = pl.ndiag; d.s0 = pl.s0; d.nblocks = pl.nblocks;
      d.steady_b0 = pl.steady_b0; d.steady_b1 = pl.steady_b1;
      d.h_pitch = std::min(p.origin_len, p.mutant_len) + 1;
      b->cells += pl.cells;
      b->alg_bytes += pl.cells / 2 + p.origin_len + p.mutant_len + 32;
      maxspan = std::max<int64_t>(maxspan, (int64_t)p.origin_len + p.mutant_len + 2);
      maxmin = std::max<int64_t>(maxmin, std::min(p.origin_len, p.mutant_len));
      maxnd = std::max(maxnd, pl.ndiag); sumnd += pl.ndiag; nsolv++;
      est.add_pair(model, (double)pl.nblocks * 16.0 , pl.ndiag);
      min_x = std::min(min_x, (int)p.origin_len);
      if (b->mode == pw::STD_MODE) est.add_std_pair(model, p.origin_len, p.mutant_len, pl.ndiag);
    }
    b->descs[k] = d;
  }
  {
    const double f = (double)(1 << sc.scale_shift);
    const double gstep = pw::floor_gap_step(b->go, b->ge) / f, smin = sc.smin / f;
    for (int32_t k = 0; k < b->n; k++) {
      const pw::PairDesc& d = b->descs[k];
      if (d.solvable && pw::reaches_reference_floor(b->brule, d.ndiag == 1 && b->mode == pw::BANDED_MODE, gstep, smin,
                                                    (int64_t)d.X + d.Y + 2))
        return fail("scores too low for this alignment type: (X + Y + 2) * (the most a gap step, or on a one-diagonal band a "
                    "substitution, can lower a score) must stay below INT_MAX, where the reference floors gap candidates and "
                    "end cells at -INT_MAX (not reproduced)");
    }
  }
  b->use_f64 = (b->flags & PW_FLAG_FORCE_F64) || !sc.integral || (double)maxspan * sc.maxabs >= (double)(1 << 27);
  const bool bany = b->brule == pw::BRULE_ANY;
  const bool track = b->endrule == pw::END_STD_LOCAL || b->endrule == pw::END_BANDED_LOCAL;
  if ((b->flags & (PW_FLAG_FORCE_GENERIC | PW_FLAG_DUMP_SCORES)) || b->go > 0 || L > 32) b->variant = pw::VAR_GENERIC;
  else if (bany) b->variant = pw::VAR_FAST_ANY_TRACK;
  else if (track) b->variant = pw::VAR_FAST_TRACK;
  else b->variant = pw::VAR_FAST;
  const bool latency_mode = kn.latency_mode >= 0 ? kn.latency_mode != 0 : nsolv <= 256;
  const bool strips_serve = b->mode == pw::STD_MODE && !kn.no_strip && !(b->flags & (PW_FLAG_DUMP_SCORES | PW_FLAG_NO_STRIP)) &&
                            (double)maxspan * sc.maxabs < (double)(1 << 25) &&
                            (sc.simple || (sc.integral && L <= 4 && sc.smax <= 127 && sc.smin >= -128 && !kn.strip_no_byte_rows));
  const bool strips_win = latency_mode && strips_serve && min_x >= 127 && !kn.no_small_strip && est.strips_beat_packed_workgroups(model);
  const int rule = b->variant == pw::VAR_GENERIC ? -1 : pw::packed_rule(b->brule, b->endrule);
  const pw::PackedAdmission adm = pw::admit_packed(rule, sc, L, b->go, b->ge, maxmin, maxnd, maxspan, kn);
  pw::PackedLayout p16;
  if (adm.rule >= 0 && !b->use_f64 && nsolv > 0 && !(b->flags & (PW_FLAG_NO_PACKED16 | PW_FLAG_FORCE_TILED | PW_FLAG_FORCE_STRIP))) {
    if (maxnd > 2048) {
      if (maxnd <= 64 * pw::kMaxWavesPerPair * 32 && !kn.no_packed_mw && !strips_win) p16 = pw::packed_workgroup_layout(maxnd);
    } else {
      p16 = pw::packed_lane_layout(maxnd, sumnd, nsolv, latency_mode, strips_win, kn, model);
    }
  }
  if (p16.bk) {
    b->variant = pw::VAR_FAST16;
    b->packed_seg = p16.seg; b->packed_nw = p16.nw;
    b->packed_mat = pw::packed_matrix_form(adm, p16, sc.simple, kn);
    b->packed_rule = adm.x4 && (!b->packed_mat || adm.x4_matrix) ? 3 : adm.rule;
    b->ramp_free = pw::ramp_free(b->packed_rule, b->packed_mat != 0, b->go, b->ge, sc.smin, kn);
    b->stamp_group = pw::stamp_group(b->packed_rule, b->packed_mat != 0, p16.bk, p16.seg != 0, p16.nw, b->ramp_free != 0, kn);
  }
  pw::PairRules pr;
  pr.strips = strips_serve && !b->use_f64 && b->variant != pw::VAR_GENERIC && b->variant != pw::VAR_FAST16 &&
              !(b->flags & PW_FLAG_FORCE_TILED);
  pr.all_strips = (b->flags & PW_FLAG_FORCE_STRIP) != 0;
  pr.few_strips = latency_mode && !kn.no_small_strip && est.strips_beat_workgroups(model);
  pr.all_tiled = (b->flags & PW_FLAG_FORCE_TILED) != 0;
  pr.few_tiled = latency_mode && !(b->flags & PW_FLAG_DUMP_SCORES) && !kn.no_small_tiled && est.tiles_beat_workgroups(model, b->use_f64);
  pr.latency_mode = latency_mode; pr.f64 = b->use_f64; pr.wide_lanes = kn.mw_wide_lanes;
  pr.packed_bk = p16.bk; pr.packed_nl = p16.nl;
  for (int32_t k = 0; k < b->n; k++) {
    pw::PairDesc& d = b->descs[k];
    if (!d.solvable) continue;
    const pw::PairLayout lay = pw::pair_layout(d.ndiag, d.X, pr);
    d.bk = lay.bk; d.nl = lay.nl;
    d.mask_off = mask_words;
    d.h_off = h_elems;
    if (lay.kind == pw::PAIR_STRIPS) {
      const int nstrips = pw::strip_count(d.X), nkq = pw::strip_nkq(d.Y);
      d.layout = 1;
      mask_words += (uint64_t)nstrips * nkq * 64 * 4;
      b->strips.push_back(k);
      b->fifo_bytes = std::max<size_t>(b->fifo_bytes, (size_t)nstrips * (size_t)pw::strip_fifo_pitch(d.Y) * sizeof(uint64_t));
      continue;
    }
    if (lay.kind == pw::PAIR_TILED && (b->flags & PW_FLAG_DUMP_SCORES)) return fail("the score plane is not available for tiled (very wide) tables");
    mask_words += (uint64_t)(d.nblocks + 1) * lay.nl * lay.bk;
    if (b->flags & PW_FLAG_DUMP_SCORES) h_elems += (uint64_t)d.ndiag * d.h_pitch;
    if (lay.kind == pw::PAIR_TILED) { b->tiled.push_back(k); b->st_pitch = std::max(b->st_pitch, (d.ndiag + 63) / 64 * 64); continue; }
    size_t ci = 0;
    for (; ci < b->classes.size(); ci++) if (b->classes[ci].bk == lay.bk && b->classes[ci].nw == lay.nw) break;
    if (ci == b->classes.size()) { b->classes.emplace_back(); b->classes.back().bk = lay.bk; b->classes.back().nw = lay.nw; }
    b->classes[ci].order.push_back(k);
  }
  for (auto& c : b->classes)
    std::stable_sort(c.order.begin(), c.order.end(), [&](int32_t x, int32_t y) {
      return b->descs[x].nblocks > b->descs[y].nblocks;
    });
  if (b->variant == pw::VAR_FAST16) plan_waves(b, p16);
  b->mask_words = mask_words; b->h_elems = h_elems; b->tx_bytes = tx_bytes;
  b->arena_shared = (b->flags & PW_FLAG_SHARED_ARENA) != 0;
  b->plan_ms = std::chrono::duration<double, std::milli>(std::chrono::steady_clock::now().time_since_epoch()).count() - t_build0;
  return 0;
}

int batch_alloc(pw_batch* b) {
  const int L = b->L;
  const uint64_t mask_words = b->mask_words, h_elems = b->h_elems, tx_bytes = b->tx_bytes;
  const bool tim = env_int("PWLIB_TIMING", 0) != 0;
  auto tnow = []() { return std::chrono::duration<double, std::milli>(std::chrono::steady_clock::now().time_since_epoch()).count(); };
  const double t_plan = tnow();
  const int dev = b->device;
  b->on_device = true;
  HIP_TRY(hipSetDevice(dev));
  if (!b->arena_shared) {
    HIP_TRY(b->arena.alloc(dev, b->arena_bytes + 16));
    b->d_arena = b->arena.p;
  }
  HIP_TRY(b->d_pairs.alloc(dev, sizeof(pw::PairDesc) * std::max<int32_t>(b->n, 1)));
  HIP_TRY(b->d_masks.alloc(dev, 4 * mask_words + 64));
  HIP_TRY(b->d_results.alloc(dev, sizeof(pw::Result) * std::max<int32_t>(b->n, 1)));
  HIP_TRY(b->d_tx.alloc(dev, std::max<uint64_t>(tx_bytes, 16)));
  const size_t esz = b->use_f64 ? 8 : 4;
  if (h_elems) HIP_TRY(b->d_hdump.ensure(esz * h_elems));
  HIP_TRY(b->d_subst.ensure(esz * (size_t)L * L));
  if (b->use_f64) {
    HIP_TRY(hipMemcpy(b->d_subst.p, b->subst.data(), 8 * (size_t)L * L, hipMemcpyHostToDevice));
  } else {
    std::vector<int32_t> si((size_t)L * L);
    for (size_t i = 0; i < si.size(); i++) si[i] = (int32_t)b->subst[i];
    HIP_TRY(hipMemcpy(b->d_subst.p, si.data(), 4 * si.size(), hipMemcpyHostToDevice));
  }
  if (b->n) HIP_TRY(hipMemcpy(b->d_pairs.p, b->descs.data(), sizeof(pw::PairDesc) * b->n, hipMemcpyHostToDevice));
  if (!b->strips.empty()) {
    int maxs = 0;
    for (int32_t k : b->strips) maxs = std::max(maxs, pw::strip_count(b->descs[k].X));
    HIP_TRY(b->d_fifo.alloc(dev, b->fifo_bytes));
    HIP_TRY(hipMemset(b->d_fifo.p, 0, b->fifo_bytes));
    HIP_TRY(b->d_sbest.ensure((size_t)maxs));
    HIP_TRY(b->d_ctl.ensure(b->strips.size() * 16));
  }
  if (!b->tiled.empty())
    for (DeviceBuffer& st : b->d_state) HIP_TRY(st.ensure((size_t)5 * b->st_pitch * sizeof(double)));
  if (!b->waves.empty() && upload(fail, b->d_waves, b->waves.data(), b->waves.size()) != 0) return -1;
  for (auto& c : b->classes)
    if (upload(fail, c.d_order, c.order.data(), c.order.size()) != 0) return -1;
  {
    std::vector<pw::Result> init(std::max<int32_t>(b->n, 1));
    for (auto& r : init) { r.score = 0; r.opt_i = r.opt_j = -1; r.origin_idx = r.mutant_idx = 0; r.tx_len = 0; r.status = 0; }
    HIP_TRY(hipMemcpy(b->d_results.p, init.data(), sizeof(pw::Result) * init.size(), hipMemcpyHostToDevice));
  }
  if (b->flags & PW_FLAG_PROFILE)
    for (DeviceEvent* ev : {&b->ev_fill0, &b->ev_fill1, &b->ev_tr0, &b->ev_tr1}) HIP_TRY(ev->create());
  if (tim && b->n > 1000) fprintf(stderr, "pwlib timing: batch of %d pairs: planning %.1f ms, device buffers + descriptors %.1f ms\n", b->n, b->plan_ms, tnow() - t_plan);
  return 0;
}

int mark_done(pw_batch* b, hipStream_t st) {
  for (auto& se : b->done_events)
    if (se.first == st) { HIP_TRY(hipEventRecord(se.second.e, st)); return 0; }
  DeviceEvent ev;
  HIP_TRY(hipEventCreateWithFlags(&ev.e, hipEventDisableTiming));
  b->done_events.emplace_back(st, std::move(ev));
  HIP_TRY(hipEventRecord(b->done_events.back().second.e, st));
  return 0;
}

std::atomic<uint32_t> g_strip_epoch{1};

int xcc_queues(int device, int32_t* xcc_queue) {
  static std::mutex mu;
  static int cached_n[kMaxDevices] = {0};
  static int32_t cached_map[kMaxDevices][8];
  std::lock_guard<std::mutex> lk(mu);
  if (device < 0 || device >= kMaxDevices) return 0;
  if (cached_n[device] == 0) {
    DeviceArray<uint32_t> d; uint32_t h[8] = {0};
    if (d.ensure(8) != hipSuccess || hipMemset(d.p, 0, sizeof h) != hipSuccess ||
        pw::launch_xcc_census(d.p, nullptr) != hipSuccess || hipMemcpy(h, d.p, sizeof h, hipMemcpyDeviceToHost) != hipSuccess)
      return 0;
    int n = 0;
    for (int i = 0; i < 8; i++) cached_map[device][i] = h[i] ? n++ : -1;
    cached_n[device] = n;
  }
  memcpy(xcc_queue, cached_map[device], sizeof cached_map[device]);
  return cached_n[device];
}

bool strip_byte_rows_ok(const pw_batch* b) {
  if (b->L > 4 || b->knobs.strip_no_byte_rows) return false;
  for (double v : b->subst) if (v != std::floor(v) || v < -128 || v > 127) return false;
  return true;
}

int launch_strip_fills(pw_batch* b, hipStream_t st) {
  static const int workers = std::max(1, env_int("PWLIB_STRIP_WAVES", 1024));
  static const int lds_kb = std::max(0, env_int("PWLIB_STRIP_LDS_KB", 0));
  size_t q = 0;
  if (b->strip_ctl_init.size() != 16 * b->strips.size()) b->strip_ctl_init.assign(16 * b->strips.size(), 0u);
  for (int32_t k : b->strips) {
    const pw::PairDesc& d = b->descs[k];
    pw::StripParams a;
    memset(&a, 0, sizeof a);
    a.arena = b->d_arena; a.o_off = d.o_off; a.m_off = d.m_off;
    a.fifo = b->d_fifo.p; a.masks = b->d_masks.p + d.mask_off; a.sbest = b->d_sbest.p;
    a.ctl = b->d_ctl.p + 16 * q++;
    a.result = b->d_results.p + k;
    a.X = d.X; a.Y = d.Y;
    a.nstrips = pw::strip_count(d.X); a.nkq = pw::strip_nkq(d.Y);
    a.fifo_pitch = pw::strip_fifo_pitch(d.Y);
    uint32_t e = g_strip_epoch.fetch_add(1) & 0xffffffu;
    if (e == 0) e = g_strip_epoch.fetch_add(1) & 0xffffffu;
    a.epoch = e;
    a.brule = b->brule; a.endrule = b->endrule;
    a.match = (int32_t)b->subst[0]; a.mismatch = (int32_t)(b->L > 1 ? b->subst[1] : b->subst[0]);
    a.go = (int32_t)b->go; a.ge = (int32_t)b->ge;
    a.score_mul = b->score_mul;
    a.spin_limit = env_int("PWLIB_STRIP_SPIN_LIMIT", 1 << 21);
    a.nq = xcc_queues(b->device, a.xcc_queue);
    if (a.nq <= 0) return fail("could not determine the XCDs of the device");
    a.run_len = std::max(1, env_int("PWLIB_STRIP_RUN", std::max(1, workers / a.nq)));
    const bool track = b->endrule != pw::END_CORNER;
    const char* trace = getenv("PWLIB_STRIP_TRACE");
    DeviceArray<uint64_t> stamps;
    if (trace && *trace && q == 1) {
      HIP_TRY(stamps.ensure((size_t)a.nstrips * 16));
      HIP_TRY(hipMemset(stamps.p, 0, stamps.bytes((size_t)a.nstrips * 16)));
      a.stamps = stamps.p;
    }
    const bool byte_rows = strip_byte_rows_ok(b);
    if (!byte_rows && !b->simple) return fail("internal: a substitution matrix on the strips needs their byte rows");
    uint32_t* ci = b->strip_ctl_init.data() + 16 * (q - 1);
    uint32_t rows[4] = {0u, 0u, 0u, 0u};
    if (byte_rows)
      for (int o = 0; o < 4; o++)
        for (int m = 0; m < 4; m++)
          if (o < b->L && m < b->L) rows[o] |= ((uint32_t)(int32_t)b->subst[(size_t)o * b->L + m] & 0xffu) << (8 * m);
    for (int z = 0; z < 16; z++) ci[z] = (z >= pw::kStripRows && z < pw::kStripRows + 4) ? rows[z - pw::kStripRows] : 0u;
    HIP_TRY(pw::launch_strip_fill(a, track, byte_rows, ci, workers, lds_kb << 10, st));
    if (stamps.p) {
      std::vector<uint64_t> h((size_t)a.nstrips * 16);
      HIP_TRY(hipStreamSynchronize(st));
      HIP_TRY(hipMemcpy(h.data(), stamps.p, stamps.bytes(h.size()), hipMemcpyDeviceToHost));
      if (FILE* f = fopen(trace, "wb")) { fwrite(h.data(), 8, h.size(), f); fclose(f); }
    }
  }
  return 0;
}

template <typename T>
pw::FillParams<T> fill_params(const pw_batch* b) {
  pw::FillParams<T> a;
  memset(&a, 0, sizeof a);
  a.pairs = b->d_pairs.p; a.arena = b->d_arena; a.masks = b->d_masks.p; a.results = b->d_results.p;
  a.npairs = b->n; a.L = b->L; a.brule = b->brule; a.endrule = b->endrule;
  a.banded = b->mode == pw::BANDED_MODE;
  a.match = (T)b->subst[0]; a.mismatch = (T)(b->L > 1 ? b->subst[1] : b->subst[0]);
  a.go = (T)b->go; a.ge = (T)b->ge;
  a.score_mul = b->score_mul;
  return a;
}

template <typename T>
int launch_all_fills(pw_batch* b, hipStream_t st) {
  pw::FillParams<T> a = fill_params<T>(b);
  a.hdump = b->d_hdump.as<T>(); a.subst = b->d_subst.as<const T>();
  for (auto& c : b->classes) {
    a.order = c.d_order.p;
    if (c.nw > 1) HIP_TRY(pw::launch_fill_mw(a, b->variant, c.bk, c.nw, (int)c.order.size(), st));
    else HIP_TRY(pw::launch_fill(a, b->variant, c.bk, (int)c.order.size(), st));
  }
  a.order = nullptr;
  a.st_pitch = b->st_pitch;
  for (int32_t k : b->tiled) {
    const pw::PairDesc& d = b->descs[k];
    const int ntiles = (d.nl + pw::kTileCentralLanes - 1) / pw::kTileCentralLanes;
    int cur = 0;
    for (int tb = 0; tb < d.nblocks; tb += pw::kTileBlocks) {
      a.tile_b0 = tb; a.tile_nb = std::min(pw::kTileBlocks, d.nblocks - tb);
      a.st_in = b->d_state[cur].as<const T>(); a.st_out = b->d_state[cur ^ 1].as<T>();
      HIP_TRY(pw::launch_tile(a, b->variant, (int)k, ntiles, st));
      cur ^= 1;
    }
    a.st_in = b->d_state[cur].as<const T>();
    HIP_TRY(pw::launch_tile_finish(a, (int)k, st));
  }
  return 0;
}

int launch_packed_fill(pw_batch* b, hipStream_t st) {
  pw::FillParams<int32_t> a = fill_params<int32_t>(b);
  a.order = b->classes[0].d_order.p; a.waves = b->d_waves.p;
  if (b->packed_mat) pw::packed_matrix_rows(b->subst.data(), b->L, b->packed_rule == 3, a.mat_rows, &a.mat_bias);
  a.ramp_free = b->ramp_free;
  if (b->packed_nw > 1) HIP_TRY(pw::launch_fill16_mw(a, b->classes[0].bk, b->packed_rule, b->packed_mat, b->packed_nw, (int)b->waves.size(), st));
  else if (b->stamp_group == 4) HIP_TRY(pw::launch_fill16g(a, (int)b->waves.size(), st));
  else HIP_TRY(pw::launch_fill16(a, b->classes[0].bk, b->packed_seg, b->packed_rule, b->packed_mat, (int)b->waves.size(), st));
  return 0;
}

}

extern "C" {

const char* pw_last_error(void) { return g_err.c_str(); }

void pw_pool_trim(void) { pool_drop(-1); }

int pw_device_memory(int device, uint64_t* free_bytes, uint64_t* total_bytes) {
  size_t fr = 0, tot = 0;
  HIP_TRY(hipSetDevice(device));
  HIP_TRY(hipMemGetInfo(&fr, &tot));
  if (free_bytes) *free_bytes = fr;
  if (total_bytes) *total_bytes = tot;
  return 0;
}

int pw_device_count(void) {
  int n = 0;
  if (hipGetDeviceCount(&n) != hipSuccess) return 0;
  return n;
}

pw_batch* pw_batch_create(int device, const pw_scoring* sc, int32_t n_pairs, const pw_pair* pairs,
                          uint64_t arena_bytes, uint32_t flags) {
  std::unique_ptr<pw_batch> b(new pw_batch());
  b->device = device;
  if (batch_inputs(b.get(), false, sc, n_pairs, pairs, arena_bytes, flags) != 0 || batch_plan(b.get()) != 0 ||
      batch_alloc(b.get()) != 0)
    return nullptr;
  return b.release();
}

void pw_batch_destroy(pw_batch* b) { delete b; }

int pw_plan_only(const pw_scoring* sc, int32_t n_pairs, const pw_pair* pairs, uint64_t arena_bytes, uint32_t flags,
                 char* kernel, int32_t kernel_cap, int32_t* info) {
  pw_batch b;
  b.device = -1;
  if (batch_inputs(&b, true, sc, n_pairs, pairs, arena_bytes, flags) != 0 || batch_plan(&b) != 0) return -1;
  if (kernel && kernel_cap > 0) { strncpy(kernel, pw_batch_kernel_name(&b), (size_t)kernel_cap - 1); kernel[kernel_cap - 1] = 0; }
  if (info) {
    int64_t one = 0, wg = 0;
    for (const auto& c : b.classes) (c.nw > 1 || (b.variant == pw::VAR_FAST16 && b.packed_nw > 1) ? wg : one) += (int64_t)c.order.size();
    info[0] = b.use_f64 ? 1 : 0; info[1] = b.scale_shift; info[2] = (int32_t)one; info[3] = (int32_t)wg;
    info[4] = (int32_t)b.tiled.size(); info[5] = (int32_t)b.strips.size();
    info[6] = b.variant == pw::VAR_FAST16 ? b.packed_rule : -1; info[7] = (b.packed_mat ? 1 : 0) | (b.ramp_free ? 2 : 0) | (b.stamp_group == 4 ? 4 : 0);
  }
  return 0;
}

int pw_batch_init_rc(const pw_batch* b, int32_t k) { return (k < 0 || k >= b->n) ? -1 : b->plans[k].rc; }

int pw_batch_band(const pw_batch* b, int32_t k, int32_t* dmin, int32_t* dmax, int32_t* num_rows) {
  if (k < 0 || k >= b->n) return -1;
  if (dmin) *dmin = b->plans[k].dmin;
  if (dmax) *dmax = b->plans[k].dmax;
  if (num_rows) *num_rows = b->plans[k].num_rows;
  return b->plans[k].clamped;
}

int64_t pw_batch_pair_cells(const pw_batch* b, int32_t k) { return (k < 0 || k >= b->n) ? -1 : b->plans[k].cells; }
int64_t pw_batch_cells(const pw_batch* b) { return b->cells; }
int64_t pw_batch_algorithmic_bytes(const pw_batch* b) { return b->alg_bytes; }
int pw_batch_score_type(const pw_batch* b) { return b->use_f64 ? 1 : 0; }

const char* pw_batch_kernel_name(const pw_batch* b) {
  static thread_local char name[96];
  int bk = 0, nw = 1; size_t most = 0;
  for (const auto& c : b->classes) if (c.order.size() > most) { most = c.order.size(); bk = c.bk; nw = c.nw; }
  if (b->classes.empty() && b->tiled.empty() && !b->strips.empty()) {
    snprintf(name, sizeof name, "k_fill_strip<%s> x row strips", b->endrule != pw::END_CORNER ? "true" : "false");
    return name;
  }
  if (b->classes.empty() && !b->tiled.empty()) { snprintf(name, sizeof name, "k_fill_tile<%s> x time blocks", b->use_f64 ? "double" : "int"); return name; }
  const char* t = b->use_f64 ? "double" : "int";
  if (nw > 1) { snprintf(name, sizeof name, "k_fill_mw<%s, %d, ...> x %d wavefronts", t, bk, nw); return name; }
  switch (b->variant) {
    case pw::VAR_FAST16:
      if (b->packed_nw > 1) snprintf(name, sizeof name, "k_fill16_mw<%d, %d> x %d wavefronts", bk, b->packed_rule, b->packed_nw);
      else if (b->packed_rule == 3) snprintf(name, sizeof name, "k_fill16<%d, %s> x4", bk, b->packed_seg ? "true" : "false");
      else if (b->packed_rule) snprintf(name, sizeof name, "k_fill16<%d, %s, %d>", bk, b->packed_seg ? "true" : "false", b->packed_rule);
      else snprintf(name, sizeof name, "k_fill16<%d, %s>", bk, b->packed_seg ? "true" : "false");
      if (b->packed_mat) strncat(name, " matrix", sizeof name - strlen(name) - 1);
      break;
    case pw::VAR_FAST_ANY_TRACK: snprintf(name, sizeof name, "k_fill<%s, %d, true, true, false>", t, bk); break;
    case pw::VAR_FAST_TRACK: snprintf(name, sizeof name, "k_fill<%s, %d, false, true, false>", t, bk); break;
    case pw::VAR_FAST: snprintf(name, sizeof name, "k_fill<%s, %d, false, false, false>", t, bk); break;
    default: snprintf(name, sizeof name, "k_fill<%s, %d, false, true, true>", t, bk); break;
  }
  return name;
}

void* pw_arena_upload(int device, const uint8_t* host, uint64_t bytes) {
  void* p = nullptr;
  if (hipSetDevice(device) != hipSuccess || hipMalloc(&p, bytes + 16) != hipSuccess) { (void)hipGetLastError(); fail("pw_arena_upload: allocation failed"); return nullptr; }
  if (hipMemset((uint8_t*)p + bytes, 0, 16) != hipSuccess || (bytes && hipMemcpy(p, host, bytes, hipMemcpyHostToDevice) != hipSuccess)) {
    (void)hipGetLastError(); (void)hipFree(p); fail("pw_arena_upload: copy failed"); return nullptr;
  }
  return p;
}
void pw_arena_free(int device, void* p) { if (p) { (void)hipSetDevice(device); (void)hipFree(p); } }
int pw_batch_share_arena(pw_batch* b, void* dev) {
  if (!b->arena_shared) return fail("pw_batch_share_arena: the batch was not created with PW_FLAG_SHARED_ARENA");
  if (!dev) return fail("pw_batch_share_arena: null arena");
  b->d_arena = (uint8_t*)dev;
  return 0;
}

int pw_batch_upload_arena(pw_batch* b, const uint8_t* host, uint64_t bytes) {
  if (b->arena_shared) return fail("the batch shares a caller-owned arena (PW_FLAG_SHARED_ARENA): nothing to upload");
  if (bytes > b->arena_bytes) return fail("arena upload larger than the arena");
  HIP_TRY(hipSetDevice(b->device));
  if (bytes) HIP_TRY(hipMemcpy(b->d_arena, host, bytes, hipMemcpyHostToDevice));
  return 0;
}

void* pw_batch_arena_device(pw_batch* b) { return b->d_arena; }

void* pw_host_alloc(uint64_t bytes) {
  void* p = nullptr;
  if (hipHostMalloc(&p, bytes ? bytes : 1, hipHostMallocDefault) != hipSuccess) { (void)hipGetLastError(); fail("hipHostMalloc failed"); return nullptr; }
  return p;
}
void pw_host_free(void* p) { if (p) (void)hipHostFree(p); }

int pw_batch_upload_arena_async(pw_batch* b, const uint8_t* host, uint64_t bytes, void* stream) {
  if (b->arena_shared) return fail("the batch shares a caller-owned arena (PW_FLAG_SHARED_ARENA): nothing to upload");
  if (bytes > b->arena_bytes) return fail("arena upload larger than the arena");
  HIP_TRY(hipSetDevice(b->device));
  if (bytes) HIP_TRY(hipMemcpyAsync(b->d_arena, host, bytes, hipMemcpyHostToDevice, (hipStream_t)stream));
  return mark_done(b, (hipStream_t)stream);
}
int pw_batch_results_async(pw_batch* b, pw_result* out, void* stream) {
  HIP_TRY(hipSetDevice(b->device));
  if (b->n) HIP_TRY(hipMemcpyAsync(out, b->d_results.p, sizeof(pw_result) * (size_t)b->n, hipMemcpyDeviceToHost, (hipStream_t)stream));
  return mark_done(b, (hipStream_t)stream);
}
int pw_batch_transcripts_async(pw_batch* b, uint8_t* out, void* stream) {
  HIP_TRY(hipSetDevice(b->device));
  if (b->tx_bytes) HIP_TRY(hipMemcpyAsync(out, b->d_tx.p, b->tx_bytes, hipMemcpyDeviceToHost, (hipStream_t)stream));
  return mark_done(b, (hipStream_t)stream);
}

int pw_batch_solve(pw_batch* b, void* stream) {
  hipStream_t st = (hipStream_t)stream;
  if (b->arena_shared && !b->d_arena) return fail("pw_batch_solve: the batch was created with PW_FLAG_SHARED_ARENA and has no arena yet");
  HIP_TRY(hipSetDevice(b->device));
  b->traced = false; b->traced_from = false;
  if (!b->repaired.empty()) {
    HIP_TRY(hipDeviceSynchronize());
    b->repaired.clear();
  }
  if (b->flags & PW_FLAG_PROFILE) HIP_TRY(hipEventRecord(b->ev_fill0.e, st));
  int rc = b->variant == pw::VAR_FAST16 ? launch_packed_fill(b, st)
           : b->use_f64 ? launch_all_fills<double>(b, st) : launch_all_fills<int32_t>(b, st);
  if (rc == 0 && !b->strips.empty()) rc = launch_strip_fills(b, st);
  if (rc != 0) return rc;
  if (b->flags & PW_FLAG_PROFILE) { HIP_TRY(hipEventRecord(b->ev_fill1.e, st)); b->fill_timed = true; }
  return mark_done(b, st);
}

static pw_batch* repaired_sub(pw_batch* b, int32_t k) {
  for (auto& r : b->repaired) if (r.first == k) return r.second.get();
  return nullptr;
}

static int replay_trace(pw_batch* b, int32_t k, pw_batch* sub, hipStream_t st) {
  if (b->traced_from) {
    const int32_t e[2] = {b->last_ends[2 * (size_t)k], b->last_ends[2 * (size_t)k + 1]};
    if (pw_batch_traceback_from(sub, e, st) != 0) return -1;
  } else if (pw_batch_traceback(sub, st) != 0) return -1;
  const pw::PairDesc& d = b->descs[k];
  HIP_TRY(hipMemcpyAsync(b->d_results.p + k, sub->d_results.p, sizeof(pw::Result), hipMemcpyDeviceToDevice, st));
  HIP_TRY(hipMemcpyAsync(b->d_tx.p + d.tx_off, sub->d_tx.p + sub->descs[0].tx_off, (size_t)d.tx_cap, hipMemcpyDeviceToDevice, st));
  return 0;
}

static int repair_strip_pair(pw_batch* b, int32_t k) {
  pw_scoring sc;
  sc.mode = b->mode; sc.type = b->type; sc.alphabet_len = b->L; sc.subst = b->subst_in.data(); sc.go = b->go_in; sc.ge = b->ge_in;
  const uint32_t keep = b->flags & (PW_FLAG_FORCE_F64 | PW_FLAG_FORCE_GENERIC | PW_FLAG_NO_PACKED16);
  std::unique_ptr<pw_batch> owned(pw_batch_create(b->device, &sc, 1, &b->pairs[k], b->arena_bytes,
                                                  keep | PW_FLAG_SHARED_ARENA | PW_FLAG_NO_STRIP));
  pw_batch* sub = owned.get();
  if (!sub) return -1;
  if (!sub->strips.empty()) return fail("internal: the replacement of a strip pair took the strips again");
  if (pw_batch_share_arena(sub, b->d_arena) != 0 || pw_batch_solve(sub, nullptr) != 0) return -1;
  b->repaired.emplace_back(k, std::move(owned));
  if (b->traced) { b->trace_seq++; if (replay_trace(b, k, sub, nullptr) != 0) return -1; }
  else HIP_TRY(hipMemcpyAsync(b->d_results.p + k, sub->d_results.p, sizeof(pw::Result), hipMemcpyDeviceToDevice, nullptr));
  HIP_TRY(hipStreamSynchronize(nullptr));
  static const bool verbose = env_int("PWLIB_TIMING", 0) != 0;
  if (verbose) fprintf(stderr, "pwlib: strip pipeline of pair %d abandoned; solved again on %s\n", (int)k, pw_batch_kernel_name(sub));
  return 0;
}

static int do_trace(pw_batch* b, const int32_t* d_ends, hipStream_t st) {
  pw::TraceParams p;
  memset(&p, 0, sizeof p);
// ... 1110 lines not shown
```

Baseline: 2937.

## Feed sequence letters to the grouped fill16 kernel through an LDS ring

Adds a new fill16l kernel variant, selected by default whenever the grouped stamp kernel would run, that stages origin rows and mutant codes into a double LDS ring buffer. The wave then reads per-step letters from LDS instead of issuing global feed loads and commits on every block. Each 8-block period restages the ring behind a workgroup barrier. This removes the per-block global feed path but adds LDS traffic, barriers and extra registers, which may affect occupancy.

```diff
diff --git a/biseqt_amd/batch.py b/biseqt_amd/batch.py
--- a/biseqt_amd/batch.py
+++ b/biseqt_amd/batch.py
@@ -780,7 +780,7 @@
 
 
 def plan_only(shapes, alnmode=W.STD_MODE, alntype=W.GLOBAL, alphabet_len=4, subst_scores=None, match_score=1, mismatch_score=0,
-              go_score=0, ge_score=0, flags=0, ramp_free=False, stamp_group=False):
+              go_score=0, ge_score=0, flags=0, ramp_free=False, stamp_group=False, lds_feed=False):
     lib = W.load()
     L = alphabet_len
     if subst_scores is None:
@@ -807,4 +807,6 @@
         out['ramp_free'] = bool(info[7] & 2)
     if stamp_group:
         out['stamp_group'] = 4 if info[7] & 4 else 1
+    if lds_feed:
+        out['lds_feed'] = bool(info[7] & 8)
     return out
diff --git a/biseqt_amd/csrc/build.py b/biseqt_amd/csrc/build.py
--- a/biseqt_amd/csrc/build.py
+++ b/biseqt_amd/csrc/build.py
@@ -32,7 +32,7 @@
 TYPES = (('i32', 'int32_t'), ('f64', 'double'))
 F64_FLAGS = {'f64': ['-fno-honor-nans'] + os.environ.get('PW_F64_EXTRA_CXXFLAGS', '').split()}
 FILL_EXTRA = {('f64', 8): ['-mllvm', '-amdgpu-sched-strategy=max-ilp']}
-HASHED_OBJECTS = ('pw_fill16_bk8_r3_mat.o', 'pw_fill16g_bk8_r3_mat.o', 'pw_fill16_bk8_r3.o', 'pw_fill16_bk8_r0.o', 'pw_fill_i32_bk8.o', 'pw_fill_f64_bk8.o', 'pw_strip.o')
+HASHED_OBJECTS = ('pw_fill16_bk8_r3_mat.o', 'pw_fill16g_bk8_r3_mat.o', 'pw_fill16l_bk8_r3_mat.o', 'pw_fill16_bk8_r3.o', 'pw_fill16_bk8_r0.o', 'pw_fill_i32_bk8.o', 'pw_fill_f64_bk8.o', 'pw_strip.o')
 HEADERS = ['pw_types.h', 'pw_wave.h', 'pw_strip.h', 'pw_plan.h', 'pw_model.h', 'pw_launch.h', 'pw_device.h', 'pw_hip_host.h']
 
 
@@ -65,6 +65,10 @@
     jobs.append((obj, [HIPCC] + COMMON + ['-mllvm', '-amdgpu-sched-strategy=max-ilp', '-DPW_FILL16_WAVES=%d' % occ,
                                           '-DPW_FILL16_WAVES_SEG=%d' % occ_seg, '-c', os.path.join(HERE, 'pw_fill16g_tu.hip'), '-o', obj],
                  [os.path.join(HERE, 'pw_fill16g_tu.hip')]))
+    obj = os.path.join(OBJ_DIR, 'pw_fill16l_bk8_r3_mat.o')
+    jobs.append((obj, [HIPCC] + COMMON + ['-mllvm', '-amdgpu-sched-strategy=max-ilp', '-DPW_FILL16_WAVES=%d' % occ,
+                                          '-DPW_FILL16_WAVES_SEG=%d' % occ_seg, '-c', os.path.join(HERE, 'pw_fill16l_tu.hip'), '-o', obj],
+                 [os.path.join(HERE, 'pw_fill16l_tu.hip')]))
     obj = os.path.join(OBJ_DIR, 'pw_trace.o')
     jobs.append((obj, [HIPCC] + COMMON + ['-c', os.path.join(HERE, 'pw_trace.hip'), '-o', obj],
                  [os.path.join(HERE, 'pw_trace.hip')]))
diff --git a/biseqt_amd/csrc/pw_device.h b/biseqt_amd/csrc/pw_device.h
--- a/biseqt_amd/csrc/pw_device.h
+++ b/biseqt_amd/csrc/pw_device.h
@@ -41,6 +41,10 @@
 
 struct DevFeed {
   PW_FN static uint64_t const_dword2(const uint8_t* base, uint32_t byte_off) { return dev_const_dword2(base, byte_off); }
+  PW_FN static uint32_t lds_read32(uint32_t addr) { return *(__attribute__((address_space(3))) const uint32_t*)(uintptr_t)addr; }
+  PW_FN static void lds_write32(uint32_t addr, uint32_t v) { *(__attribute__((address_space(3))) uint32_t*)(uintptr_t)addr = v; }
+  PW_FN static void lds_write16(uint32_t addr, uint32_t v) { *(__attribute__((address_space(3))) uint16_t*)(uintptr_t)addr = (uint16_t)v; }
+  PW_FN static void lds_sync() { __syncthreads(); }
 };
 
 struct DevP : DevFeed {
@@ -200,6 +204,18 @@
 void k_fill16g(const FillParams<int32_t> a) {
   const WaveDesc wd = a.waves[blockIdx.x];
   WaveFill16<DevP, BK, SEG, RULE, MAT, 4> w(a, wd);
+  w.run();
+}
+
+template <int BK, bool SEG, int RULE, bool MAT = false>
+__global__ __launch_bounds__(64) PW_FILL_ATTR
+__attribute__((amdgpu_waves_per_eu(Fill16Occupancy<BK, SEG, RULE>::lo, Fill16Occupancy<BK, SEG, RULE>::hi)))
+void k_fill16l(const FillParams<int32_t> a) {
+  using W = WaveFill16<DevP, BK, SEG, RULE, MAT, 4, true>;
+  __shared__ uint32_t ring[2 * W::kRingWords];
+  const WaveDesc wd = a.waves[blockIdx.x];
+  W w(a, wd);
+  w.ring_h = dev_lds_handle(ring);
   w.run();
 }
 
diff --git a/biseqt_amd/csrc/pw_fill16l_tu.hip b/biseqt_amd/csrc/pw_fill16l_tu.hip
--- /dev/null
+++ b/biseqt_amd/csrc/pw_fill16l_tu.hip
@@ -0,0 +1,8 @@
+#include "pw_device.h"
+
+namespace pw {
+hipError_t launch_fill16l_bk8_r3_m1(const FillParams<int32_t>& a, int nwaves, hipStream_t st) {
+  hipLaunchKernelGGL((k_fill16l<8, false, 3, true>), dim3((unsigned)nwaves), dim3(64), 0, st, a);
+  return hipGetLastError();
+}
+}
diff --git a/biseqt_amd/csrc/pw_launch.h b/biseqt_amd/csrc/pw_launch.h
--- a/biseqt_amd/csrc/pw_launch.h
+++ b/biseqt_amd/csrc/pw_launch.h
@@ -13,6 +13,7 @@
 hipError_t launch_fill16(const FillParams<int32_t>& a, int bk, int seg, int rule, int mat, int nwaves, hipStream_t st);
 hipError_t launch_fill16_mw(const FillParams<int32_t>& a, int bk, int rule, int mat, int nw, int npairs, hipStream_t st);
 hipError_t launch_fill16g(const FillParams<int32_t>& a, int nwaves, hipStream_t st);
+hipError_t launch_fill16l(const FillParams<int32_t>& a, int nwaves, hipStream_t st);
 hipError_t launch_fill_mw(const FillParams<int32_t>& a, int variant, int bk, int nw, int nblocks, hipStream_t st);
 hipError_t launch_fill_mw(const FillParams<double>& a, int variant, int bk, int nw, int nblocks, hipStream_t st);
 hipError_t launch_tile(const FillParams<int32_t>& a, int variant, int pair, int ntiles, hipStream_t st);
diff --git a/biseqt_amd/csrc/pw_plan.h b/biseqt_amd/csrc/pw_plan.h
--- a/biseqt_amd/csrc/pw_plan.h
+++ b/biseqt_amd/csrc/pw_plan.h
@@ -194,6 +194,7 @@
   bool no_scaled16 = false;
   bool ramp_blocks = false;
   bool stamp_group1 = false;
+  bool no_lds_feed = false;
   bool packed_bk_forced = false;
   int packed_bk = 0;
   bool packed_bk_seg = false;
@@ -266,6 +267,8 @@
 static inline int stamp_group(int rule, bool matrix, int bk, bool seg, int nw, bool ramp_free_on, const PlanKnobs& kn) {
   return (rule == 3 && matrix && bk == 8 && !seg && nw == 1 && ramp_free_on && !kn.stamp_group1) ? 4 : 1;
 }
+
+static inline bool lds_feed(int stamp_group_, const PlanKnobs& kn) { return stamp_group_ == 4 && !kn.no_lds_feed; }
 
 struct PackedLayout { int bk = 0, nl = 0, seg = 0, nw = 1; };
 
diff --git a/biseqt_amd/csrc/pw_trace.hip b/biseqt_amd/csrc/pw_trace.hip
--- a/biseqt_amd/csrc/pw_trace.hip
+++ b/biseqt_amd/csrc/pw_trace.hip
@@ -194,6 +194,12 @@
   return launch_fill16g_bk8_r3_m1(a, nwaves, st);
 }
 
+hipError_t launch_fill16l_bk8_r3_m1(const FillParams<int32_t>&, int, hipStream_t);
+hipError_t launch_fill16l(const FillParams<int32_t>& a, int nwaves, hipStream_t st) {
+  if (!a.ramp_free) return hipErrorInvalidValue;
+  return launch_fill16l_bk8_r3_m1(a, nwaves, st);
+}
+
 hipError_t launch_fill16_mw(const FillParams<int32_t>& a, int bk, int rule, int mat, int nw, int npairs, hipStream_t st) {
 #define PW_CASE16(BK, R, MT) case ((BK) * 8 + (R)) * 2 + (MT): return launch_fill16mw_bk##BK##_r##R##_m##MT(a, nw, npairs, st);
   switch ((bk * 8 + rule) * 2 + (mat ? 1 : 0)) {
diff --git a/biseqt_amd/csrc/pw_wave.h b/biseqt_amd/csrc/pw_wave.h
--- a/biseqt_amd/csrc/pw_wave.h
+++ b/biseqt_amd/csrc/pw_wave.h
@@ -624,6 +624,17 @@
   return n;
 }
 namespace pk {
+inline int& lds_feed_emu() { static int v = -1; return v; }
+inline unsigned& ring_restages() { static unsigned n = 0; return n; }
+inline uint32_t* emu_ring() { static uint32_t r[2 * 528]; return r; }
+}
+extern "C" __attribute__((used, visibility("default"))) inline void pw_emu_lds_feed(int v) { pk::lds_feed_emu() = v; }
+extern "C" __attribute__((used, visibility("default"))) inline unsigned pw_ring_restages(int reset) {
+  const unsigned n = pk::ring_restages();
+  if (reset) pk::ring_restages() = 0;
+  return n;
+}
+namespace pk {
 inline unsigned& feed_breaches() { static unsigned n = 0; return n; }
 inline unsigned* feed_path_counts() { static unsigned n[4] = {0, 0, 0, 0}; return n; }
 }
@@ -637,7 +648,7 @@
 }
 #endif
 
-template <class P, int BK, bool SEG, int RULE = 0, bool MAT = false, int GRP = 1>
+template <class P, int BK, bool SEG, int RULE = 0, bool MAT = false, int GRP = 1, bool LDSF = false>
 struct WaveFill16 {
   static constexpr bool SC4 = RULE == 3;
   static constexpr int RL = SC4 ? 0 : RULE;
@@ -704,6 +715,79 @@
 #endif
   uint32_t kgE[RH], kgO[RH];
   uint32_t POS[8];
+  static constexpr bool LOK = SPLIT && TRK && !SEG && BK == 8;
+  static_assert(!LDSF || (LOK && GRP == 4), "letters from LDS: the grouped kernel's form");
+  static constexpr int kRingRow = 132, kRingWords = 4 * kRingRow;
+#if defined(__HIPCC__)
+#define PW_IF_LDSF if constexpr (LDSF)
+#else
+  bool ldsf_rt = false;
+#define PW_IF_LDSF if (ldsf_rt)
+#endif
+  PW_FN uint32_t ring_read(int which, uint32_t base, int c) const {
+    const uint32_t w = (uint32_t)(which * kRingWords + (c & 3) * kRingRow + (c >> 2));
+#if defined(__HIPCC__)
+    return P::lds_read32(ring_h + base + 4u * w);
+#else
+    return pk::emu_ring()[w + (base >> 2)];
+#endif
+  }
+  PW_FN void ring_store(uint32_t w, uint32_t v, int half) {
+#if defined(__HIPCC__)
+    if (half < 0) P::lds_write32(ring_h + 4u * w, v);
+    else P::lds_write16(ring_h + 4u * w + 2u * (uint32_t)half, v);
+#else
+    uint32_t& d = pk::emu_ring()[w];
+    d = half < 0 ? v : (half == 0 ? ((d & 0xffff0000u) | (v & 0xffffu)) : ((d & 0xffffu) | (v << 16)));
+#endif
+  }
+  PW_FN void ring_put(int which, uint32_t u, uint32_t v, int half) {
+    const uint32_t s = u & 511u;
+    const uint32_t w = (uint32_t)(which * kRingWords) + (s & 3u) * (uint32_t)kRingRow + (s >> 2);
+    ring_store(w, v, half);
+    if ((s >> 2) < 4u) ring_store(w + 128u, v, half);
+  }
+  PW_FN static void ring_sync() {
+#if defined(__HIPCC__)
+    P::lds_sync();
+#else
+    (void)P::shr1z(0);
+#endif
+  }
+  PW_FN static uint32_t ring_letter(const uint8_t* seq, int idx, int n) {
+    const int c = pw_clampi(idx, 0, n > 0 ? n - 1 : 0);
+#if !defined(__HIPCC__)
+    if (c < 0 || c >= (n > 0 ? n : 1)) { pk::feed_breaches()++; return 0xa5u; }
+#endif
+    return (uint32_t)seq[c];
+  }
+  PW_FN void stage_issue(int u0) {
+    const int u = u0 + P::lane();
+    nx_o = ring_letter(oseq, fe + u, X); nx_m = ring_letter(mseq, ff - 256 + u, Y);
+  }
+  PW_FN void stage_commit(int u0) {
+#if !defined(__HIPCC__)
+    if (P::lane() == 0) pk::ring_restages()++;
+#endif
+    const int u = u0 + P::lane();
+    const uint32_t row = (uint32_t)(fe + u) < (uint32_t)X ? row_of(nx_o) : 0u;
+    const uint32_t code = MSEL | (((uint32_t)(ff - 256 + u) < (uint32_t)Y ? nx_m : MOUT) + 4u * sel4_fed(u));
+    ring_put(0, (uint32_t)u, row, -1);
+    ring_put(1, (uint32_t)u, code, 0);
+    ring_put(1, (uint32_t)u + 2u, code, 1);
+  }
+  PW_FN void ring_begin() {
+#pragma unroll 1
+    for (int c = 0; c < 6; c++) { stage_issue(64 * c); stage_commit(64 * c); }
+    ring_sync();
+    stage_issue(384);
+    ro = 4u * (uint32_t)li; rm = 4u * (uint32_t)(64 - li);
+  }
+  PW_FN void restage(int s) {
+    stage_commit(64 * s + 384);
+    ring_sync();
+    stage_issue(64 * s + 448);
+  }
   static constexpr bool FROWS = MAT && !SEG && UNR == 4 && BK <= 8;
   uint32_t frow[FROWS ? 8 : 1];
   bool rf;
@@ -798,7 +882,13 @@
         if (TRK) track_key<EK>(kbE[p], HE[p], tlE[p], tv0, k);
       }
     }
-    {
+    PW_IF_LDSF {
+      left_next = (uint32_t)P::shl1((int32_t)LE[0], (int32_t)left_next);
+      const uint32_t nxt = ring_read(0, ro, 3 + k);
+#pragma unroll
+      for (int i = 0; i + 1 < (MAT ? R : 1); i++) ROW[i] = ROW[i + 1];
+      ROW[MAT ? R - 1 : 0] = nxt;
+    } else {
       const int oi = xfeed_o + it;
       const uint32_t fb = Base::feed_byte(fo_lo, fo_hi, k);
       uint32_t feed = (!EDGE || (uint32_t)oi < (uint32_t)X) ? fb : SENT_O;
@@ -833,7 +923,13 @@
         if (TRK) track_key<EK>(kbO[p], HO[p], tlO[p], tv1, k);
       }
     }
-    {
+    PW_IF_LDSF {
+      up_prev = (uint32_t)P::shr1((int32_t)UO[RH - 1], (int32_t)up_prev);
+      const uint32_t first = ring_read(1, rm, k);
+#pragma unroll
+      for (int p = RH - 1; p > 0; p--) MW[p] = MW[p - 1];
+      MW[0] = first;
+    } else {
       const int mi = yfeed_m + it;
       const uint32_t fbm = Base::feed_byte(fm_lo, fm_hi, k);
       const uint32_t feed = (MAT ? (MSEL | (fbm + 4u * (FIXSEL ? sel4_fed(k) : 1u)))
@@ -912,8 +1008,12 @@
         stamp_group((uint32_t)(b >> 2) + 1u);
 #pragma unroll
         for (int k = 0; k < 8; k++) POS[k] += 0x00200020u;
-      }
-    }
+        PW_IF_LDSF { if ((b & 7) == 7) restage(b >> 3); }
+      }
+    } else PW_IF_LDSF {
+      if ((b & 7) == 7) restage(b >> 3);
+    }
+    PW_IF_LDSF { ro = (ro + 8u) & 511u; rm = (rm + 8u) & 511u; }
   }
 
   PW_FN static uint64_t dwords(uint32_t lo, uint32_t hi) { return ((uint64_t)hi << 32) | lo; }
@@ -1144,7 +1244,11 @@
       for (int g = 0; g < BK / 4; g++)
         mbase[g] = pk::opaque_s((uint8_t*)(a.masks + pd.mask_off) + (uint64_t)(4u * (uint32_t)g * mgroup));
     }
-    feed_issue<true>(0);
+#if !defined(__HIPCC__)
+    ldsf_rt = LOK && rf && P::nwaves() == 1 && pk::lds_feed_emu() == 1;
+#endif
+    PW_IF_LDSF { fe = e; ff = f; ring_begin(); }
+    else feed_issue<true>(0);
     if constexpr (SPLIT) {
       const int nb = nblocks_run();
       const int b0 = wd.steady_b0 < nb ? (wd.steady_b0 > 0 ? wd.steady_b0 : 0) : nb;
@@ -1176,10 +1280,13 @@
   PW_FN int nblocks_run() const { return SBASE ? (wd.nblocks < pd.nblocks ? wd.nblocks : pd.nblocks) : wd.nblocks; }
   template <int EK>
   PW_FN void blocks_step(int b) {
-    if constexpr (RAMPF && EK == 0)
-      feed_commit<true>(b, rf & (((uint32_t)(xfeed_o + 8 * b) >= flimx) | ((uint32_t)(yfeed_m + 8 * b) >= flimy)));
-    else feed_commit(b, EK != 0);
-    if (b + 1 < nblocks_run()) feed_issue(b + 1);
+    PW_IF_LDSF {
+    } else {
+      if constexpr (RAMPF && EK == 0)
+        feed_commit<true>(b, rf & (((uint32_t)(xfeed_o + 8 * b) >= flimx) | ((uint32_t)(yfeed_m + 8 * b) >= flimy)));
+      else feed_commit(b, EK != 0);
+      if (b + 1 < nblocks_run()) feed_issue(b + 1);
+    }
     block16<EK>(b);
   }
 
@@ -1267,7 +1374,12 @@
       }
     }
   }
+  uint32_t ring_h = 0;
+  uint32_t ro, rm;
+  uint32_t nx_o, nx_m;
+  int fe, ff;
 };
+#undef PW_IF_LDSF
 
 PW_FN int pw_first_op(uint32_t mask) {
   return (mask & 1u) ? 0 : (mask & 2u) ? 1 : (mask & 4u) ? 2 : 3;
diff --git a/biseqt_amd/csrc/pwlib_api.cpp b/biseqt_amd/csrc/pwlib_api.cpp
--- a/biseqt_amd/csrc/pwlib_api.cpp
+++ b/biseqt_amd/csrc/pwlib_api.cpp
@@ -196,6 +196,7 @@
   int packed_mat = 0;
   int ramp_free = 0;
   int stamp_group = 1;
+  int lds_feed = 0;
   DeviceArray<pw::WaveDesc> d_waves;
   int64_t cells = 0, alg_bytes = 0;
   bool on_device = false;
@@ -261,6 +262,7 @@
   k.no_scaled16 = on("PWLIB_NO_SCALED16");
   k.ramp_blocks = on("PWLIB_RAMP_BLOCKS");
   k.stamp_group1 = env_int("PWLIB_STAMP_GROUP", 0) == 1;
+  k.no_lds_feed = env_int("PWLIB_LDS_FEED", 1) == 0;
   const char* bk = getenv("PWLIB_PACKED_BK");
   if (bk && *bk) { k.packed_bk_forced = true; k.packed_bk = atoi(bk); k.packed_bk_seg = strchr(bk, 's') != nullptr; }
   return k;
@@ -396,6 +398,7 @@
     b->packed_rule = adm.x4 && (!b->packed_mat || adm.x4_matrix) ? 3 : adm.rule;
     b->ramp_free = pw::ramp_free(b->packed_rule, b->packed_mat != 0, b->go, b->ge, sc.smin, kn);
     b->stamp_group = pw::stamp_group(b->packed_rule, b->packed_mat != 0, p16.bk, p16.seg != 0, p16.nw, b->ramp_free != 0, kn);
+    b->lds_feed = pw::lds_feed(b->stamp_group, kn) ? 1 : 0;
   }
   pw::PairRules pr;
   pr.strips = strips_serve && !b->use_f64 && b->variant != pw::VAR_GENERIC && b->variant != pw::VAR_FAST16 &&
@@ -631,6 +634,7 @@
   if (b->packed_mat) pw::packed_matrix_rows(b->subst.data(), b->L, b->packed_rule == 3, a.mat_rows, &a.mat_bias);
   a.ramp_free = b->ramp_free;
   if (b->packed_nw > 1) HIP_TRY(pw::launch_fill16_mw(a, b->classes[0].bk, b->packed_rule, b->packed_mat, b->packed_nw, (int)b->waves.size(), st));
+  else if (b->lds_feed) HIP_TRY(pw::launch_fill16l(a, (int)b->waves.size(), st));
   else if (b->stamp_group == 4) HIP_TRY(pw::launch_fill16g(a, (int)b->waves.size(), st));
   else HIP_TRY(pw::launch_fill16(a, b->classes[0].bk, b->packed_seg, b->packed_rule, b->packed_mat, (int)b->waves.size(), st));
   return 0;
@@ -682,7 +686,7 @@
     for (const auto& c : b.classes) (c.nw > 1 || (b.variant == pw::VAR_FAST16 && b.packed_nw > 1) ? wg : one) += (int64_t)c.order.size();
     info[0] = b.use_f64 ? 1 : 0; info[1] = b.scale_shift; info[2] = (int32_t)one; info[3] = (int32_t)wg;
     info[4] = (int32_t)b.tiled.size(); info[5] = (int32_t)b.strips.size();
-    info[6] = b.variant == pw::VAR_FAST16 ? b.packed_rule : -1; info[7] = (b.packed_mat ? 1 : 0) | (b.ramp_free ? 2 : 0) | (b.stamp_group == 4 ? 4 : 0);
+    info[6] = b.variant == pw::VAR_FAST16 ? b.packed_rule : -1; info[7] = (b.packed_mat ? 1 : 0) | (b.ramp_free ? 2 : 0) | (b.stamp_group == 4 ? 4 : 0) | (b.lds_feed ? 8 : 0);
   }
   return 0;
 }
```

Measured after the change: 3093 (median of 6 runs). +5.3%, better.
